# mateomarin/two_towers

Hardware: AMD Instinct MI355X
Metric: training pairs/sec at global batch=8192, 1/2/4/8 GPUs; MRR@10 match (higher is better)
Workload: dtype bf16; 1 GPU; BASELINE configs[2]: EnhancedTwoTowerModel(300, 256), seq_len 64, batch 8192 per GPU, bf16, hard-negative mining k=5 + margin 0.2, dropout 0.1, Adam; global_batch=8192, seq_len=64, hidden=256, embedding_dim=300, parallelism=dp1, loss=hardneg_margin

## Files before the change

### include/tt_hip.h

```cpp
#ifndef TT_HIP_H
#define TT_HIP_H
#include <stdint.h>

#ifdef __cplusplus
extern "C" {
#endif

#define TT_OK 0
#define TT_EINVAL 1000
#define TT_DT_F32 0
#define TT_DT_BF16 1

const char* tt_version(void);
const char* tt_last_error(void);
int tt_set_option(const char* name, int value);
int tt_get_option(const char* name, int* value);

int tt_embed_gather(int dtype, const void* table, long vocab, int ep, const int32_t* ids, long n,
                    void* out, void* stream);

int tt_pack_rows(int dtype, const float* src, long n, int e, int ep, void* out, void* stream);
typedef struct {
  const float* src;
  const float* src2;
  void* dst;
  int rows, cols, dcols;
  long lds, ldd;
  int dst_bf16;
} tt_pack_job;
int tt_pack_multi(const tt_pack_job* jobs, int njobs, void* stream);

int tt_cast(int dtype, const float* x, long n, void* y, void* stream);

int tt_colsum(const float* x, long rows, int cols, long ld, float* out, int accumulate, void* stream);

typedef struct {
  const void* a[4];
  const void* b[4];
  void* c[4];
  const float* bias[4];
  int bshift[4];
  const void* a_hi[4];
  int a_split;
  uint32_t drop_row0;
} tt_gemm_batch;

int tt_gemm(int dtype, int out_dtype, int a_kouter, int b_kouter, int m, int n, int k,
            const tt_gemm_batch* batch, int nbatch, long lda, long ldb, long ldc, float alpha,
            int beta_accum, int relu, int seq_t, uint32_t drop_seed, float drop_p, int splits,
            float* splitk_ws, void* stream);
int tt_gemm_ct(int dtype, int out_dtype, int a_kouter, int b_kouter, int m, int n, int k,
               const tt_gemm_batch* batch, int nbatch, long lda, long ldb, long ldc, float alpha,
               int beta_accum, int relu, int seq_t, uint32_t drop_seed, float drop_p, int splits,
               float* splitk_ws, int c_trans, void* stream);
long tt_gemm_ws_size(int m, int n, int nbatch, int splits);
int tt_gemm_pick_splits(int m, int n, int k, int nbatch);
int tt_gemm_bres_form(int m, int n, int k, int nbatch, long lda, long ldc);
int tt_gemm_tall_form(int dtype, int out_dtype, int a_kouter, int b_kouter, int m, int n, int k, long lda,
                      long ldb, int splits, int extras);

typedef struct {
  const void* g;
  const void* whh;
  const float* bhn;
  void* y;
  void* x1;
  void* save;
  float* hstate;
  int dir;
  uint32_t drop_seed;
  int drop_col0;
  uint32_t drop_row0;
} tt_gru_fwd_rec;

int tt_gru_fwd(int dtype, const tt_gru_fwd_rec* recs, int nrec, int B, int T, int H, long ldg,
               long ldy, float drop_p, void* ws, long ws_bytes, void* stream);
int tt_gru_fwd_launches(int dtype, int T, int H);
long tt_gru_fwd_ws_size(int dtype, int nrec, int B, int T, int H, long ldg, long ldy);
int tt_gru_fwd_launches_for(int dtype, int nrec, int B, int T, int H, long ldg, long ldy);

typedef struct {
  const void* g; const void* whh; const float* bhn;
  void* y;
  void* hfinal;
  void* scratch;
  int dir;
} tt_gru_infer_rec;
int  tt_gru_fwd_infer(int dtype, const tt_gru_infer_rec* recs, int nrec, int B, int T, int H, long ldg,
                      long ldy, long ldf, void* ws, long ws_bytes, void* stream);
long tt_gru_infer_scratch_size(int dtype, int B, int T, int H, int final_only);

typedef struct {
  const void* save;
  const void* y;
  const void* dy;
  const float* dfinal;
  const void* whh;
  void* dgx;
  void* dgh;
  void* dhstate;
  float* dbias_part;
  int dir;
} tt_gru_bwd_rec;

int tt_gru_bwd(int dtype, const tt_gru_bwd_rec* recs, int nrec, int B, int T, int H, long ldy,
               long ldd, long ldf, void* stream);
int tt_gru_bwd_launches(int dtype, int T, int H);
int tt_gru_bwd_carry_on_chip(int dtype, int T, int H);
int tt_gru_bias_rows(int B);

typedef struct {
  const void* w1; const float* b1; const float* ln_g; const float* ln_b;
  const void* w2; const float* b2;
  const void* x;
  void* p1;
  float* mean;
  float* rstd;
  void* u;
  float* out;
} tt_head_fwd_io;

int tt_proj_head_fwd(int dtype, const tt_head_fwd_io* io, int ntower, int B, int h, float ln_eps,
                     void* stream);

typedef struct {
  const void* w1; const float* ln_g; const float* ln_b; const void* w2;
  const void* x; const void* p1; const float* mean; const float* rstd; const void* u;
  const float* dout;
  float* dx;
  float* dw1; float* db1; float* dg; float* dbeta; float* dw2; float* db2;
  void* ws;
} tt_head_bwd_io;

int tt_proj_head_bwd(int dtype, const tt_head_bwd_io* io, int ntower, int B, int h, float ln_eps,
                     void* stream);
long tt_proj_head_bwd_ws_size(int dtype, int B, int h);

typedef struct {
  const void* x;
  const void* w1; const float* b1; const float* ln_g; const float* ln_b;
  void* p1;
  float* mean;
  float* rstd;
  float* out;
} tt_head1_fwd_io;

int tt_proj_head1_fwd(int dtype, const tt_head1_fwd_io* io, long rows, int C, float ln_eps, float drop_p,
                      uint32_t drop_seed, void* stream);

typedef struct {
  const void* x; const void* w1; const float* ln_g; const float* ln_b;
  const void* p1; const float* mean; const float* rstd;
  const float* dout;
  float* dx;
  float* dw1; float* db1; float* dg; float* dbeta;
  void* ws;
} tt_head1_bwd_io;

int tt_proj_head1_bwd(int dtype, const tt_head1_bwd_io* io, long rows, int C, float drop_p, uint32_t drop_seed,
                      void* stream);
long tt_proj_head1_bwd_ws_size(int dtype, long rows, int C);

int tt_l2norm_fwd(int dtype, const float* x, long rows, int cols, float eps, void* y, float* y32,
                  float* norm, void* stream);
int tt_l2norm_bwd(const float* dy, const float* y32, const float* norm, long rows, int cols,
                  float eps, float* dx, int accumulate, void* stream);

int tt_infonce_fwd(int dtype, const void* qn, long bq, const void* dn, long nd, int h,
                   float inv_tau, float offdiag_sub, long label_offset, float* lse,
                   float* row_loss, void* ws, void* stream);
long tt_infonce_fwd_ws_size(long bq, long nd);
int tt_infonce_bwd(int dtype, const void* qn, long bq, const void* dn, long nd, int h,
                   float inv_tau, float offdiag_sub, long label_offset, const float* lse,
                   const float* gscale, float* dqn, float* ddn, void* ws, void* stream);
long tt_infonce_bwd_ws_size(int dtype, long bq, long nd, int h);

int tt_hardneg_topk(int dtype, const void* qn, long bq, const void* dn, long nd, int h,
                    long label_offset, int k, int32_t* idx, float* val, void* ws, void* stream);
long tt_hardneg_ws_size(int dtype, long bq, long nd, int h, int k);

int tt_search_topk(int dtype, const float* qn, long Q, const void* dn, long N, int h, int k,
                   int32_t* idx, float* val, void* ws, void* stream);
long tt_search_ws_size(int dtype, long Q, long N, int h, int k);

int tt_topk_max(void);
int tt_topk_rows(const float* S, long rows, long cols, long ld, long label_offset, int k,
                 int32_t* idx, float* val, void* ws, void* stream);
long tt_topk_rows_ws_size(long rows, long cols, int k);

int tt_margin_fwd(const float* qn, long bq, const float* dn, long nd, int h, long label_offset,
                  const int32_t* idx, int k, float margin, float* row_loss, void* stream);
int tt_margin_bwd(const float* qn, long bq, const float* dn, long nd, int h, long label_offset,
                  const int32_t* idx, int k, float margin, const float* gscale, float* dqn, float* ddn,
                  void* ws, void* stream);
long tt_margin_bwd_ws_size(long bq, long nd, int h, int k);

int tt_sum(const float* x, long n, float scale, float* out, void* stream);

int tt_adam_multi(float* const* params, const float* const* grads, float* const* exp_avg,
                  float* const* exp_avg_sq, const long* sizes, int ntensors, float lr, float beta1,
                  float beta2, float eps, float weight_decay, int step, const int32_t* skip, void* stream);

#ifdef __cplusplus
}
#endif
#endif
```

### two_towers_amd/_lib.py

```python
from __future__ import annotations

import contextlib
import ctypes
import os
from ctypes import POINTER, c_float, c_int, c_long, c_uint32, c_void_p

import torch

_HERE = os.path.dirname(os.path.abspath(__file__))
LIB_PATH = os.environ.get("TT_HIP_LIB", os.path.join(_HERE, "lib", "libtt_hip.so"))

DT_F32 = 0
DT_BF16 = 1
TT_EINVAL = 1000


class TTError(RuntimeError):
    pass


class GruTimeoutError(TTError):
    """A column-split GRU forward launch gave up waiting for one of its member workgroups
    (tt_gru_fwd's status word): that launch's outputs are invalid."""


class GemmBatch(ctypes.Structure):
    _fields_ = [
        ("a", c_void_p * 4),
        ("b", c_void_p * 4),
        ("c", c_void_p * 4),
        ("bias", c_void_p * 4),
        ("bshift", c_int * 4),
        ("a_hi", c_void_p * 4),
        ("a_split", c_int),
        ("drop_row0", c_uint32),
    ]


class PackJob(ctypes.Structure):
    _fields_ = [
        ("src", c_void_p),
        ("src2", c_void_p),
        ("dst", c_void_p),
        ("rows", c_int),
        ("cols", c_int),
        ("dcols", c_int),
        ("lds", c_long),
        ("ldd", c_long),
        ("dst_bf16", c_int),
    ]


class GruFwdRec(ctypes.Structure):
    _fields_ = [
        ("g", c_void_p), ("whh", c_void_p), ("bhn", c_void_p), ("y", c_void_p), ("x1", c_void_p),
        ("save", c_void_p), ("hstate", c_void_p), ("dir", c_int), ("drop_seed", c_uint32),
        ("drop_col0", c_int), ("drop_row0", c_uint32),
    ]


class GruInferRec(ctypes.Structure):
    _fields_ = [
        ("g", c_void_p), ("whh", c_void_p), ("bhn", c_void_p), ("y", c_void_p), ("hfinal", c_void_p),
        ("scratch", c_void_p), ("dir", c_int),
    ]


class GruBwdRec(ctypes.Structure):
    _fields_ = [
        ("save", c_void_p), ("y", c_void_p), ("dy", c_void_p), ("dfinal", c_void_p), ("whh", c_void_p),
        ("dgx", c_void_p), ("dgh", c_void_p), ("dhstate", c_void_p), ("dbias_part", c_void_p),
        ("dir", c_int),
    ]


class HeadFwdIO(ctypes.Structure):
    _fields_ = [
        ("w1", c_void_p), ("b1", c_void_p), ("ln_g", c_void_p), ("ln_b", c_void_p), ("w2", c_void_p),
        ("b2", c_void_p), ("x", c_void_p), ("p1", c_void_p), ("mean", c_void_p), ("rstd", c_void_p),
        ("u", c_void_p), ("out", c_void_p),
    ]


class HeadBwdIO(ctypes.Structure):
    _fields_ = [
        ("w1", c_void_p), ("ln_g", c_void_p), ("ln_b", c_void_p), ("w2", c_void_p), ("x", c_void_p),
        ("p1", c_void_p), ("mean", c_void_p), ("rstd", c_void_p), ("u", c_void_p), ("dout", c_void_p),
        ("dx", c_void_p), ("dw1", c_void_p), ("db1", c_void_p), ("dg", c_void_p), ("dbeta", c_void_p),
        ("dw2", c_void_p), ("db2", c_void_p), ("ws", c_void_p),
    ]


class Head1FwdIO(ctypes.Structure):
    _fields_ = [
        ("x", c_void_p), ("w1", c_void_p), ("b1", c_void_p), ("ln_g", c_void_p), ("ln_b", c_void_p),
        ("p1", c_void_p), ("mean", c_void_p), ("rstd", c_void_p), ("out", c_void_p),
    ]


class Head1BwdIO(ctypes.Structure):
    _fields_ = [
        ("x", c_void_p), ("w1", c_void_p), ("ln_g", c_void_p), ("ln_b", c_void_p), ("p1", c_void_p),
        ("mean", c_void_p), ("rstd", c_void_p), ("dout", c_void_p), ("dx", c_void_p), ("dw1", c_void_p),
        ("db1", c_void_p), ("dg", c_void_p), ("dbeta", c_void_p), ("ws", c_void_p),
    ]


_SIGS = {
    "tt_version": (ctypes.c_char_p, []),
    "tt_last_error": (ctypes.c_char_p, []),
    "tt_set_option": (c_int, [ctypes.c_char_p, c_int]),
    "tt_get_option": (c_int, [ctypes.c_char_p, POINTER(c_int)]),
    "tt_embed_gather": (c_int, [c_int, c_void_p, c_long, c_int, c_void_p, c_long, c_void_p, c_void_p]),
    "tt_pack_rows": (c_int, [c_int, c_void_p, c_long, c_int, c_int, c_void_p, c_void_p]),
    "tt_pack_multi": (c_int, [c_void_p, c_int, c_void_p]),
    "tt_cast": (c_int, [c_int, c_void_p, c_long, c_void_p, c_void_p]),
    "tt_colsum": (c_int, [c_void_p, c_long, c_int, c_long, c_void_p, c_int, c_void_p]),
    "tt_gemm": (c_int, [c_int, c_int, c_int, c_int, c_int, c_int, c_int, POINTER(GemmBatch), c_int, c_long,
                        c_long, c_long, c_float, c_int, c_int, c_int, c_uint32, c_float, c_int, c_void_p,
                        c_void_p]),
    "tt_gemm_ct": (c_int, [c_int, c_int, c_int, c_int, c_int, c_int, c_int, POINTER(GemmBatch), c_int, c_long,
                           c_long, c_long, c_float, c_int, c_int, c_int, c_uint32, c_float, c_int, c_void_p,
                           c_int, c_void_p]),
    "tt_gemm_ws_size": (c_long, [c_int, c_int, c_int, c_int]),
    "tt_gemm_pick_splits": (c_int, [c_int, c_int, c_int, c_int]),
    "tt_gemm_bres_form": (c_int, [c_int, c_int, c_int, c_int, c_long, c_long]),
    "tt_gemm_tall_form": (c_int, [c_int, c_int, c_int, c_int, c_int, c_int, c_int, c_long, c_long, c_int, c_int]),
    "tt_gru_fwd": (c_int, [c_int, POINTER(GruFwdRec), c_int, c_int, c_int, c_int, c_long, c_long, c_float,
                           c_void_p, c_long, c_void_p]),
    "tt_gru_bwd": (c_int, [c_int, POINTER(GruBwdRec), c_int, c_int, c_int, c_int, c_long, c_long, c_long,
                           c_void_p]),
    "tt_gru_bias_rows": (c_int, [c_int]),
    "tt_gru_bwd_launches": (c_int, [c_int, c_int, c_int]),
    "tt_gru_bwd_carry_on_chip": (c_int, [c_int, c_int, c_int]),
    "tt_gru_fwd_launches": (c_int, [c_int, c_int, c_int]),
    "tt_gru_fwd_ws_size": (c_long, [c_int, c_int, c_int, c_int, c_int, c_long, c_long]),
    "tt_gru_fwd_launches_for": (c_int, [c_int, c_int, c_int, c_int, c_int, c_long, c_long]),
    "tt_gru_fwd_infer": (c_int, [c_int, POINTER(GruInferRec), c_int, c_int, c_int, c_int, c_long, c_long, c_long,
                                 c_void_p, c_long, c_void_p]),
    "tt_gru_infer_scratch_size": (c_long, [c_int, c_int, c_int, c_int, c_int]),
    "tt_proj_head_fwd": (c_int, [c_int, POINTER(HeadFwdIO), c_int, c_int, c_int, c_float, c_void_p]),
    "tt_proj_head_bwd": (c_int, [c_int, POINTER(HeadBwdIO), c_int, c_int, c_int, c_float, c_void_p]),
    "tt_proj_head_bwd_ws_size": (c_long, [c_int, c_int, c_int]),
    "tt_proj_head1_fwd": (c_int, [c_int, POINTER(Head1FwdIO), c_long, c_int, c_float, c_float, c_uint32,
                                  c_void_p]),
    "tt_proj_head1_bwd": (c_int, [c_int, POINTER(Head1BwdIO), c_long, c_int, c_float, c_uint32, c_void_p]),
    "tt_proj_head1_bwd_ws_size": (c_long, [c_int, c_long, c_int]),
    "tt_l2norm_fwd": (c_int, [c_int, c_void_p, c_long, c_int, c_float, c_void_p, c_void_p, c_void_p, c_void_p]),
    "tt_l2norm_bwd": (c_int, [c_void_p, c_void_p, c_void_p, c_long, c_int, c_float, c_void_p, c_int, c_void_p]),
    "tt_infonce_fwd": (c_int, [c_int, c_void_p, c_long, c_void_p, c_long, c_int, c_float, c_float, c_long,
                               c_void_p, c_void_p, c_void_p, c_void_p]),
    "tt_infonce_fwd_ws_size": (c_long, [c_long, c_long]),
    "tt_infonce_bwd": (c_int, [c_int, c_void_p, c_long, c_void_p, c_long, c_int, c_float, c_float, c_long,
                               c_void_p, c_void_p, c_void_p, c_void_p, c_void_p, c_void_p]),
    "tt_infonce_bwd_ws_size": (c_long, [c_int, c_long, c_long, c_int]),
    "tt_hardneg_topk": (c_int, [c_int, c_void_p, c_long, c_void_p, c_long, c_int, c_long, c_int, c_void_p,
                                c_void_p, c_void_p, c_void_p]),
    "tt_hardneg_ws_size": (c_long, [c_int, c_long, c_long, c_int, c_int]),
    "tt_search_topk": (c_int, [c_int, c_void_p, c_long, c_void_p, c_long, c_int, c_int, c_void_p, c_void_p,
                               c_void_p, c_void_p]),
    "tt_search_ws_size": (c_long, [c_int, c_long, c_long, c_int, c_int]),
    "tt_topk_max": (c_int, []),
    "tt_topk_rows": (c_int, [c_void_p, c_long, c_long, c_long, c_long, c_int, c_void_p, c_void_p, c_void_p,
                             c_void_p]),
    "tt_topk_rows_ws_size": (c_long, [c_long, c_long, c_int]),
    "tt_margin_fwd": (c_int, [c_void_p, c_long, c_void_p, c_long, c_int, c_long, c_void_p, c_int, c_float,
                              c_void_p, c_void_p]),
    "tt_margin_bwd": (c_int, [c_void_p, c_long, c_void_p, c_long, c_int, c_long, c_void_p, c_int, c_float,
                              c_void_p, c_void_p, c_void_p, c_void_p, c_void_p]),
    "tt_margin_bwd_ws_size": (c_long, [c_long, c_long, c_int, c_int]),
    "tt_sum": (c_int, [c_void_p, c_long, c_float, c_void_p, c_void_p]),
    "tt_adam_multi": (c_int, [POINTER(c_void_p), POINTER(c_void_p), POINTER(c_void_p), POINTER(c_void_p),
                              POINTER(c_long), c_int, c_float, c_float, c_float, c_float, c_float, c_int,
                              c_void_p, c_void_p]),
}

EXPORTED = tuple(_SIGS)

_lib = None
_load_error: str | None = None


def load():
    global _lib, _load_error
    if _lib is not None:
        return _lib
    if _load_error is not None:
        raise TTError(_load_error)
    if not os.path.exists(LIB_PATH):
        _load_error = (f"two_towers_amd: native library not found at {LIB_PATH}; "
                       "build it with `python -c 'import __graft_entry__ as g; g.build()'` (hipcc, gfx950)")
        raise TTError(_load_error)
    lib = ctypes.CDLL(LIB_PATH, mode=ctypes.RTLD_GLOBAL)
    for name, (res, args) in _SIGS.items():
        fn = getattr(lib, name)
        fn.restype = res
        fn.argtypes = args
    _lib = lib
    return lib


def check(rc: int, what: str = ""):
    if rc != 0:
        msg = _lib.tt_last_error().decode(errors="replace") if _lib is not None else ""
        raise TTError(f"{what or 'tt_hip'} failed (rc={rc}): {msg}")


def call(name: str, *args):
    lib = load()
    check(getattr(lib, name)(*args), name)


_topk_max: int | None = None


def topk_max() -> int:
    global _topk_max
    if _topk_max is None:
        _topk_max = int(load().tt_topk_max())
    return _topk_max


def get_option(name: str) -> int:
    v = c_int(0)
    call("tt_get_option", name.encode(), ctypes.byref(v))
    return v.value


def set_option(name: str, value: int) -> int:
    old = get_option(name)
    call("tt_set_option", name.encode(), int(value))
    return old


@contextlib.contextmanager
def option(name: str, value: int):
    torch.cuda.synchronize()
    old = set_option(name, value)
    try:
        yield
    finally:
        torch.cuda.synchronize()
        set_option(name, old)


def ptr(t: torch.Tensor | None) -> int | None:
    if t is None:
        return None
    return t.data_ptr()


def stream_ptr(device: torch.device | None = None) -> int:
    return torch.cuda.current_stream(device).cuda_stream


def require_gpu(*tensors: torch.Tensor):
    load()
    for t in tensors:
        if t is not None and t.device.type != "cuda":
            raise TTError(
                "two_towers_amd runs only on an AMD GPU (HIP, gfx950); got a tensor on "
                f"'{t.device}'. There is deliberately no CPU fallback: move the model and "
                "inputs to the GPU (`.to('cuda')`).")


def dtype_code(dt: torch.dtype) -> int:
    if dt == torch.float32:
        return DT_F32
    if dt == torch.bfloat16:
        return DT_BF16
    raise TTError(f"unsupported compute dtype {dt}; use torch.float32 or torch.bfloat16")
```

### two_towers_amd/csrc/tt_api.h

```cpp
#pragma once
#include <hip/hip_runtime.h>
#include <stdio.h>
#include <string.h>

#include "../../include/tt_hip.h"

namespace tt {
void set_error(const char* fmt, ...);

enum Opt {
  OPT_GRU_STEP,
  OPT_GRU_DEPTH,
  OPT_GRU_BWD_ROWS,
  OPT_GRU_BWD_BIG,
  OPT_GRU_BWD_STREAMS,
  OPT_GEMM_PERSIST,
  OPT_GEMM_A3,
  OPT_GEMM_REGSTAGE,
  OPT_GEMM_STREAM_OUT,
  OPT_HN_GEMM,
  OPT_GRU_BWD_PERSIST,
  OPT_GRU_FWD_STEP_ROWS,
  OPT_INFONCE_FLASH,
  OPT_HN_MAP,
  OPT_GEMM_SKEW,
  OPT_GEMM_PERSIST_MAXK,
  OPT_GRU_FWD_XC,
  OPT_GRU_XC_SKIP,
  OPT_GRU_XC_SPINS,
  OPT_GRU_BWD_SKEW,
  OPT_GRU_FWD_SKEW,
  OPT_GEMM_BRES,
  OPT_GRU_XC_COOP,
  OPT_GEMM_BUF,
  OPT_GEMM_ORDER,
  OPT_GRU_STEP_RING,
  OPT_GRU_FWD_XS,
  OPT_HN_SCAN_GEMM,
  OPT_GEMM_IEPI,
  OPT_BRES_ROWS,
  OPT_HN_SCAN_V,
  OPT_GEMM_W4,
  OPT_BRES_FORM,
  OPT_WGRAD_TALL,
  OPT_N
};
int opt(Opt o);
int tt_hn_scan_gemm(const void* q, long bq, const void* d, long nd, int h, long label_off, float* cm, long nch,
                    hipStream_t st);
}

#define TT_CHECK_ARG(cond, ...)            \
  do {                                     \
    if (!(cond)) {                         \
      tt::set_error(__VA_ARGS__);          \
      return TT_EINVAL;                    \
    }                                      \
  } while (0)

#define TT_CHECK_LAUNCH(what)                                                        \
  do {                                                                               \
    hipError_t e_ = hipGetLastError();                                               \
    if (e_ != hipSuccess) {                                                          \
      tt::set_error("%s: %s", what, hipGetErrorString(e_));                          \
      return (int)e_;                                                                \
    }                                                                                \
  } while (0)

#define TT_CHECK_HIP(expr)                                                           \
  do {                                                                               \
    hipError_t e_ = (expr);                                                          \
    if (e_ != hipSuccess) {                                                          \
      tt::set_error("%s: %s", #expr, hipGetErrorString(e_));                         \
      return (int)e_;                                                                \
    }                                                                                \
  } while (0)

#define TT_PROPAGATE(expr)     \
  do {                         \
    int rc_ = (expr);          \
    if (rc_ != 0) return rc_;  \
  } while (0)

static inline int tt_ceil_div(long a, long b) { return (int)((a + b - 1) / b); }
```

### two_towers_amd/csrc/tt_gemm.hip

```cpp
#include <float.h>
#include <stdarg.h>
#include <stdlib.h>

#include <atomic>
#include <type_traits>

#include "tt_api.h"
#include "tt_gemm_core.h"

namespace tt {
static thread_local char g_err[512];
void set_error(const char* fmt, ...) {
  va_list ap;
  va_start(ap, fmt);
  vsnprintf(g_err, sizeof(g_err), fmt, ap);
  va_end(ap);
}
}

namespace tt {
namespace {
struct OptDef {
  const char* name;
  const char* env;
  int dflt;
};
constexpr OptDef kOpts[OPT_N] = {
    {"gru_step", "TT_GRU_STEP", 0},               {"gru_depth", "TT_GRU_DEPTH", 4},
    {"gru_bwd_rows", "TT_GRU_BWD_ROWS", 0},     {"gru_bwd_big", "TT_GRU_BWD_BIG", 1},
    {"gru_bwd_streams", "TT_GRU_BWD_STREAMS", 2}, {"gemm_persist", "TT_GEMM_PERSIST", 1},
    {"gemm_a3", "TT_GEMM_A3", 1},                 {"gemm_regstage", "TT_GEMM_REGSTAGE", 0},
    {"gemm_stream_out", "TT_GEMM_STREAM_OUT", 1}, {"hn_gemm", "TT_HN_GEMM", 0},
    {"gru_bwd_persist", "TT_GRU_BWD_PERSIST", 1}, {"gru_fwd_step_rows", "TT_GRU_FWD_STEP_ROWS", 0},
    {"infonce_flash", "TT_INFONCE_FLASH", 1},     {"hn_map", "TT_HN_MAP", 2},
    {"gemm_skew", "TT_GEMM_SKEW", 0},             {"gemm_persist_maxk", "TT_GEMM_PERSIST_MAXK", 24},
    {"gru_fwd_xc", "TT_GRU_FWD_XC", 1},           {"gru_xc_skip", "TT_GRU_XC_SKIP", 0},
    {"gru_xc_spins", "TT_GRU_XC_SPINS", 22},      {"gru_bwd_skew", "TT_GRU_BWD_SKEW", 14},
    {"gru_fwd_skew", "TT_GRU_FWD_SKEW", 0},       {"gemm_bres", "TT_GEMM_BRES", 1},
    {"gru_xc_coop", "TT_GRU_XC_COOP", 0},         {"gemm_buf", "TT_GEMM_BUF", 1},
    {"gemm_order", "TT_GEMM_ORDER", 0},           {"gru_step_ring", "TT_GRU_STEP_RING", 4},
    {"gru_fwd_xs", "TT_GRU_FWD_XS", 1},           {"hn_scan_gemm", "TT_HN_SCAN_GEMM", 0},
    {"gemm_iepi", "TT_GEMM_IEPI", 1},             {"bres_rows", "TT_BRES_ROWS", 32},
    {"hn_scan_v", "TT_HN_SCAN_V", 5},             {"gemm_w4", "TT_GEMM_W4", 0},
    {"bres_form", "TT_BRES_FORM", 1},             {"wgrad_tall", "TT_WGRAD_TALL", 1},
};
struct OptTable {
  std::atomic<int> v[OPT_N];
  OptTable() {
    for (int i = 0; i < OPT_N; ++i) {
      const char* e = getenv(kOpts[i].env);
      v[i].store(e && *e ? atoi(e) : kOpts[i].dflt, std::memory_order_relaxed);
    }
  }
};
OptTable& opts() {
  static OptTable t;
  return t;
}
int find_opt(const char* name) {
  for (int i = 0; name && i < OPT_N; ++i)
    if (strcmp(name, kOpts[i].name) == 0) return i;
  return -1;
}
}
int opt(Opt o) { return opts().v[o].load(std::memory_order_relaxed); }
}

extern "C" const char* tt_version(void) { return "tt_hip 0.2.0 gfx950"; }
extern "C" const char* tt_last_error(void) { return tt::g_err; }
extern "C" int tt_set_option(const char* name, int value) {
  const int i = tt::find_opt(name);
  TT_CHECK_ARG(i >= 0, "tt_set_option: unknown option '%s'", name ? name : "(null)");
  tt::opts().v[i].store(value, std::memory_order_relaxed);
  return 0;
}
extern "C" int tt_get_option(const char* name, int* value) {
  const int i = tt::find_opt(name);
  TT_CHECK_ARG(i >= 0 && value, "tt_get_option: unknown option '%s'", name ? name : "(null)");
  *value = tt::opt((tt::Opt)i);
  return 0;
}

namespace {

struct GemmArgs {
  const void* a[4];
  const void* b[4];
  void* c[4];
  const float* bias[4];
  int bshift[4];
  const void* a_hi[4];
  int a_split;
  long lda, ldb, ldc;
  int M, N, K;
  int splits, kt_per_split;
  float alpha;
  int beta, relu, seq_t;
  uint32_t drop_seed, drop_thresh, drop_row0;
  float drop_inv_keep;
  long part_stride;
  int vec_ok;
  int force_regstage;
  int skew;
  int bias_vec_ok;
  int stream_out;
  int walk_g, walk_x;
  int nbatch;
  int c_trans;
  float* cm;
  long nch, label_off;
};

constexpr int BM = 128, BN = 128;

#ifndef TT_TAIL_SKIP
#define TT_TAIL_SKIP 1
#endif
using ttg::xcd_remap;
#ifndef PERSIST_IEPI
#define PERSIST_IEPI 1
#endif
#ifndef PERSIST_BAL
#define PERSIST_BAL 1
#endif
#ifndef TT_EPI_PAIR
#define TT_EPI_PAIR 1
#endif
#ifndef TT_GEMM_BAL
#define TT_GEMM_BAL true
#endif

template <typename T, bool AKO, bool BKO, bool SHIFT, typename TO, int TBM, int TBN, int WGM, int WGN, bool DMA,
          bool A3 = false, bool BUF = false>
__global__ __launch_bounds__(64 * WGM * WGN) void gemm_kernel(GemmArgs g) {
  using ML = std::conditional_t<
      DMA,
      std::conditional_t<TBM == 256 && TBN == 256 && WGM == 2 && WGN == 4,
                         ttg::Loop8<T, AKO, BKO, TT_GEMM_BAL, A3, false, BUF>,
                         ttg::DLoop<T, AKO, BKO, TBM, TBN, WGM, WGN>>,
      ttg::MainLoop<T, AKO, BKO, TBM, TBN>>;
  static_assert(DMA || (TBM == 128 && TBN == 128 && WGM == 2 && WGN == 2), "register path is 128x128");
  constexpr int NT = 64 * WGM * WGN;
  constexpr int LDSB = ML::LDS_BYTES > 64 * (TBN + 4) * 4 ? ML::LDS_BYTES : 64 * (TBN + 4) * 4;
  __shared__ __attribute__((aligned(16))) char lds[LDSB];
  const int ntn = (g.N + TBN - 1) / TBN, ntm = (g.M + TBM - 1) / TBM;
  const int id = xcd_remap(blockIdx.x, gridDim.x);
  const int bs = id / (ntm * ntn), tile = id - bs * (ntm * ntn);
  const int mt = tile / ntn, nt = tile - mt * ntn;
  const int bi = bs / g.splits, s = bs - bi * g.splits;
  const int m0 = mt * TBM, n0 = nt * TBN;
  const T* A = static_cast<const T*>(g.a[bi]);
  const T* B = static_cast<const T*>(g.b[bi]);

  f32x4 acc[ML::TM][ML::TN];
#pragma unroll
  for (int i = 0; i < ML::TM; ++i)
#pragma unroll
    for (int j = 0; j < ML::TN; ++j) acc[i][j] = f32x4{0.f, 0.f, 0.f, 0.f};

  const int nk = (g.K * (int)sizeof(T) + ttg::KTB - 1) / ttg::KTB;
  const int kt0 = s * g.kt_per_split;
  const int kt1 = min(nk, kt0 + g.kt_per_split);

  constexpr bool L8T = DMA && TBM == 256 && TBN == 256 && WGM == 2 && WGN == 4;
  const bool mm = !L8T || !TT_TAIL_SKIP || __builtin_amdgcn_readfirstlane((int)(m0 + (int)(threadIdx.x >> 8) * 128 < g.M));
  auto lrun = [&](const auto& la, const auto& lb) {
    if constexpr (L8T) ML::run(la, lb, g.K, kt0, kt1, lds, acc, mm);
    else ML::run(la, lb, g.K, kt0, kt1, lds, acc);
  };
  auto run = [&](const auto& la) {
    if constexpr (!BKO) {
      lrun(la, ttg::KCPlain<T>{B, g.ldb, n0, g.N});
    } else if constexpr (SHIFT) {
      lrun(la, ttg::KOShift<T>{B, g.ldb, n0, g.N - n0, g.seq_t, g.bshift[bi]});
    } else {
      lrun(la, ttg::KOPlain<T>{B, g.ldb, n0, g.N - n0});
    }
  };
  if constexpr (AKO) {
    ttg::KOPlain<T> la{A, g.lda, m0, g.M - m0};
    if (g.a_split > 0) {
      la.base1 = static_cast<const T*>(g.a_hi[bi]);
      la.csplit = g.a_split;
    }
    run(la);
  } else {
    run(ttg::KCPlain<T>{A, g.lda, m0, g.M});
  }

#ifdef TT_DIAG
  if (g.force_regstage == 9) {
    float sum = 0.f;
#pragma unroll
    for (int i = 0; i < ML::TM; ++i)
#pragma unroll
      for (int j = 0; j < ML::TN; ++j) sum += acc[i][j][0] + acc[i][j][3];
    if (sum == 12345.f) static_cast<float*>(g.c[bi])[0] = 1.f;
// ... 1674 lines not shown
```

### two_towers_amd/csrc/tt_gru.hip

```cpp
#include <algorithm>
#include <cstdlib>
#include <mutex>
#include <type_traits>

#include "tt_api.h"
#include "tt_gemm_core.h"

namespace {

struct FwdRec {
  const void* g; const void* whh; const float* bhn; void* y; void* x1; void* save; float* hs;
  int dir; uint32_t seed; int col0;
  uint32_t row0;
};
struct FwdArgs {
  FwdRec r[4];
  int B, T, H;
  long ldg, ldy;
  int s;
  uint32_t drop_thresh;
  float inv_keep;
#ifdef TT_DIAG
  int dbg;
#endif
};
struct InfArgs : FwdArgs {
  void* hfin[4];
  void* himg[4];
  long ldf;
};
TT_DEV void* inf_hfin(const FwdArgs&, int) { return nullptr; }
TT_DEV void* inf_hfin(const InfArgs& a, int rz) { return a.hfin[rz]; }
TT_DEV long inf_ldf(const FwdArgs&) { return 0; }
TT_DEV long inf_ldf(const InfArgs& a) { return a.ldf; }

struct BwdRec {
  const void* save; const void* y; const void* dy; const float* dfinal; const void* whh;
  void* dgx; void* dgh; void* dh; float* dbias; int dir;
};
struct BwdArgs {
  BwdRec r[4];
  int B, T, H;
  long ldy, ldd, ldf;
  int s;
  int skew;
#ifdef TT_DIAG
  int dbg;
#endif
};


TT_DEV void gru_cell(float xr, float xz, float xn, float lr, float lz, float ln, float bn, float hp, float& y,
                     float& ar, float& az, float& an, float& ghn) {
#pragma clang fp contract(off)
  constexpr float L2E = 0x1.715476p+0f;
  ghn = ln + bn;
  ar = xr + lr;
  az = xz + lz;
  const float rg = __builtin_amdgcn_rcpf(1.0f + __builtin_amdgcn_exp2f(L2E * -ar));
  const float zg = __builtin_amdgcn_rcpf(1.0f + __builtin_amdgcn_exp2f(L2E * -az));
  an = __builtin_fmaf(rg, ghn, xn);
  const float ng = 1.0f - 2.0f * __builtin_amdgcn_rcpf(__builtin_amdgcn_exp2f(L2E * (2.0f * an)) + 1.0f);
  y = __builtin_fmaf(zg, hp, (1.0f - zg) * ng);
}

template <typename T>
struct GateRows {
  static constexpr bool SHIFTED = false, KSPLIT = false;
  const T* w; int H, j0;
  TT_DEV const T* rowptr(int r) const {
    const int half = r / 96, rem = r - half * 96;
    const int g = rem >> 5, j = j0 + half * 32 + (rem & 31);
    return j < H ? w + (long)(g * H + j) * H : nullptr;
  }
  TT_DEV const T* at(int r, int k) const { const T* p = rowptr(r); return p ? p + k : nullptr; }
};

template <typename T, int BMR, int NS = 2, typename A = FwdArgs>
__global__ __launch_bounds__(2 * BMR) void gru_fwd_step(A a) {
  constexpr bool INF = std::is_same_v<A, InfArgs>;
  constexpr int NT = 2 * BMR;
  using ML = ttg::DLoop<T, false, false, BMR, 192, BMR / 64, 2, NS>;
  __shared__ __attribute__((aligned(16))) char lds[ML::LDS_BYTES];
  const int ntj = (a.H + 63) / 64, ntm = (a.B + BMR - 1) / BMR;
  const int id = ttg::xcd_remap(blockIdx.x, gridDim.x);
  const int rz = id / (ntm * ntj), rem = id - rz * ntm * ntj;
  const FwdRec R = a.r[rz];
  const int H = a.H, T_ = a.T, s = a.s;
  const int m0 = (rem / ntj) * BMR, j0 = (rem % ntj) * 64;
  const int t = R.dir ? T_ - 1 - s : s;
  const int tp = R.dir ? t + 1 : t - 1;
  const T* Y = static_cast<const T*>(R.y);

  f32x4 acc[ML::TM][ML::TN];
#pragma unroll
  for (int i = 0; i < ML::TM; ++i)
#pragma unroll
    for (int j = 0; j < ML::TN; ++j) acc[i][j] = f32x4{0.f, 0.f, 0.f, 0.f};
  bool prod = s > 0, epi = true;
#ifdef TT_DIAG
  if (a.dbg & 8) prod = false;
  if (a.dbg & 16) epi = false;
#endif
  const int tid = threadIdx.x;
  const int cur = s & 1, prv = cur ^ 1;
  const T* G = static_cast<const T*>(R.g);
  const float* hs_prv = R.hs + (long)prv * a.B * H;
  if (prod) {
    ttg::KCPlain<T> la{Y + (long)tp * a.ldy, (long)T_ * a.ldy, m0, a.B};
    if constexpr (INF) {
      if (!Y) la = ttg::KCPlain<T>{static_cast<const T*>(a.himg[rz]) + (long)prv * a.B * H, (long)H, m0, a.B};
    }
    GateRows<T> lb{static_cast<const T*>(R.whh), H, j0};
    const int nk = (H * (int)sizeof(T) + ttg::KTB - 1) / ttg::KTB;
    ML::run(la, lb, H, 0, nk, lds, acc);
  }
  if (!epi) {
    if (acc[0][0][0] == 1.2345f) static_cast<T*>(R.y)[0] = T(0);
    return;
  }

  const int wave = threadIdx.x >> 6, lane = threadIdx.x & 63;
  float* L = reinterpret_cast<float*>(lds);
  constexpr int FLD = 68;
  T* Yw = static_cast<T*>(R.y);
  T* X1 = static_cast<T*>(R.x1);
  T* S = static_cast<T*>(R.save);
  float* hs_cur = R.hs + (long)cur * a.B * H;
  const __amdgpu_buffer_rsrc_t srs = tt_rsrc(S + ((long)m0 * T_ + t) * (4L * H));
  const __amdgpu_buffer_rsrc_t xrs = tt_rsrc(X1 ? X1 + ((long)m0 * T_ + t) * a.ldy : Yw);
  for (int hf = 0; hf < BMR / 64; ++hf) {
    if ((wave >> 1) == hf) {
      const int nb = (wave & 1) * 32;
#pragma unroll
      for (int g = 0; g < 3; ++g)
#pragma unroll
        for (int i = 0; i < 4; ++i)
#pragma unroll
          for (int jh = 0; jh < 2; ++jh)
#pragma unroll
            for (int r = 0; r < 4; ++r)
              L[(g * 64 + 16 * i + 4 * (lane >> 4) + r) * FLD + nb + 16 * jh + (lane & 15)] = acc[i][g * 2 + jh][r];
    }
    __syncthreads();
#pragma unroll
    for (int k = 0; k < 512 / NT; ++k) {
      const int rl = (tid >> 3) + (NT / 8) * k, jg = (tid & 7) * 8;
      const int b = m0 + hf * 64 + rl, j = j0 + jg;
      if (b < a.B && j < H) {
        const long row = (long)b * T_ + t;
        float xr[8], xz[8], xn[8], hp[8], bn[8], y[8], sr[8], sz[8], sn[8], sg[8];
        ld8(G + row * a.ldg + j, xr);
        ld8(G + row * a.ldg + H + j, xz);
        ld8(G + row * a.ldg + 2 * H + j, xn);
        ld8(R.bhn + j, bn);
        if (s > 0) ld8(hs_prv + (long)b * H + j, hp);
        else {
#pragma unroll
          for (int e = 0; e < 8; ++e) hp[e] = 0.f;
        }
        const float* Lr = L + (0 * 64 + rl) * FLD + jg;
        const float* Lz = L + (1 * 64 + rl) * FLD + jg;
        const float* Ln = L + (2 * 64 + rl) * FLD + jg;
#pragma unroll
        for (int e = 0; e < 8; ++e)
          gru_cell(xr[e], xz[e], xn[e], Lr[e], Lz[e], Ln[e], bn[e], hp[e], y[e], sr[e], sz[e], sn[e], sg[e]);
        st8(hs_cur + (long)b * H + j, y);
        if constexpr (INF) {
          if (Yw) st8(Yw + row * a.ldy + j, y);
          else st8(static_cast<T*>(a.himg[rz]) + ((long)cur * a.B + b) * H + j, y);
          T* hf = static_cast<T*>(a.hfin[rz]);
          if (hf && s == T_ - 1) st8(hf + (long)b * a.ldf + j, y);
          continue;
        }
        st8(Yw + row * a.ldy + j, y);
        const int so = (int)((((long)(b - m0) * T_) * 4L * H + j) * (long)sizeof(T));
        st8_sc1(srs, so, sr, (T*)nullptr);
        st8_sc1(srs, so + H * (int)sizeof(T), sz, (T*)nullptr);
        st8_sc1(srs, so + 2 * H * (int)sizeof(T), sn, (T*)nullptr);
        st8_sc1(srs, so + 3 * H * (int)sizeof(T), sg, (T*)nullptr);
        if (X1) {
#pragma unroll
          for (int e = 0; e < 8; ++e)
            y[e] *= a.drop_thresh ? tt_dropout_scale(R.seed, R.row0 + (uint32_t)row, (uint32_t)(R.col0 + j + e),
                                                     a.drop_thresh, a.inv_keep)
                                  : 1.f;
          st8_sc1(xrs, (int)((((long)(b - m0) * T_) * a.ldy + j) * (long)sizeof(T)), y, (T*)nullptr);
        }
      }
    }
    __syncthreads();
  }
}

template <typename T, int BMR, int NS = 2>
__global__ __launch_bounds__(256) void gru_bwd_step(BwdArgs a) {
  using ML = ttg::DLoop<T, false, true, BMR, 128, 2, 2, NS>;
  constexpr int LDSB = ML::LDS_BYTES > 64 * 132 * 4 ? ML::LDS_BYTES : 64 * 132 * 4;
// ... 427 lines not shown
  float bacc[4][8];
#pragma unroll
  for (int q = 0; q < 4; ++q)
#pragma unroll
    for (int e = 0; e < 8; ++e) bacc[q][e] = 0.f;
  for (int s = T_ - 1; s >= 0; --s) {
    const int t = R.dir ? T_ - 1 - s : s;
    const int tn = R.dir ? t - 1 : t + 1;
    const int tp = R.dir ? t + 1 : t - 1;
    const bool last = (s == T_ - 1);
    auto column_pass = [&](const int u0) {
    f32x4 acc[4][C::NCB];
#pragma unroll
    for (int i = 0; i < 4; ++i)
#pragma unroll
      for (int j = 0; j < C::NCB; ++j) acc[i][j] = f32x4{0.f, 0.f, 0.f, 0.f};
    if (CREG && !last) {
#pragma unroll
      for (int i = 0; i < 4; ++i)
#pragma unroll
        for (int jc = 0; jc < C::NCB; ++jc) {
          const uint2 w = *reinterpret_cast<const uint2*>(reinterpret_cast<const bf16_t*>(lds) +
                                                          (wr * 64 + 16 * i + (lane & 15)) * C::LDB + wc * (C::HP / 4) +
                                                          16 * jc + 4 * (lane >> 4));
          acc[i][jc] = f32x4{__uint_as_float(w.x << 16), __uint_as_float(w.x & 0xFFFF0000u),
                             __uint_as_float(w.y << 16), __uint_as_float(w.y & 0xFFFF0000u)};
        }
      __syncthreads();
    }
    if (!last && !(dbg & 1)) {
#if TT_BWD_BUF
      const long abytes = (long)(a.B - m0) * ldr * 2;
      const uint32_t anrec = (uint32_t)(abytes > 0xFFFFFFFFL ? 0xFFFFFFFFL : abytes);
      const ttg::tt_rsrc4 rsx = ttg::make_rsrc4(DGX + (long)tn * a.ldd + (long)m0 * ldr, anrec);
      const ttg::tt_rsrc4 rsh = ttg::make_rsrc4(DGH + (long)tn * a.ldd + (long)m0 * ldr - 2 * H, anrec);
      const ttg::tt_rsrc4 rsw = ttg::make_rsrc4(W + u0, 0xFFFFFFFFu);
      uint32_t voff[C::P];
#pragma unroll
      for (int j = 0; j < C::P; ++j)
        voff[j] = prow[j] >= 0 ? (uint32_t)(((long)prow[j] * ldr + pcol[j]) * 2) : (uint32_t)(pcol[j] * 2);
      auto issue = [&](int r) {
        const uint32_t img = lbase + (uint32_t)(r % C::NS) * C::SLOT;
        const int wv = __builtin_amdgcn_readfirstlane(threadIdx.x >> 6);
        const bool hi = r * 32 >= 2 * H;
#pragma unroll
        for (int j = 0; j < C::P; ++j) {
          const int pc = wv + 8 * j;
          if (pc < 8) ttg::dma16_buf(hi ? rsh : rsx, voff[j], (uint32_t)r * 64u, img + (uint32_t)pc * 1024u);
          else ttg::dma16_buf(rsw, voff[j], (uint32_t)r * (uint32_t)(64 * H), img + (uint32_t)pc * 1024u);
        }
      };
#else
      const char* as0[C::P];
      const char* as1[C::P];
#pragma unroll
      for (int j = 0; j < C::P; ++j) {
        const int b = m0 + (prow[j] < 0 ? 0 : prow[j]);
        const bool ok = prow[j] >= 0 && b < a.B;
        as0[j] = ok ? reinterpret_cast<const char*>(DGX + (long)tn * a.ldd + (long)b * ldr + pcol[j]) : zp;
        as1[j] = ok ? reinterpret_cast<const char*>(DGH + (long)tn * a.ldd + (long)b * ldr + pcol[j] - 2 * H) : zp;
      }
      auto issue = [&](int r) {
        const uint32_t img = lbase + (uint32_t)(r % C::NS) * C::SLOT;
        const int wv = __builtin_amdgcn_readfirstlane(threadIdx.x >> 6);
        const bool hi = r * 32 >= 2 * H;
#pragma unroll
        for (int j = 0; j < C::P; ++j) {
          const int pc = wv + 8 * j;
          const char* src;
          if (pc < 8) {
            src = hi ? as1[j] : as0[j];
            if (src != zp) src += (long)r * 64;
          } else {
            src = reinterpret_cast<const char*>(W + (long)r * 32 * H + u0 + pcol[j]);
          }
          ttg::dma16(src, img + (uint32_t)pc * 1024u);
        }
      };
#endif
      issue(0);
      issue(1);
      issue(2);
#if TT_BWD_STAG
      const bool late = wr == 1;
      wait_younger<C::NS - 2, C::P>(NK - 1);
      __builtin_amdgcn_s_barrier();
      if (late) __builtin_amdgcn_s_barrier();
#pragma unroll 1
      for (int r = 0; r < NK; ++r) {
        if (r > 0) __builtin_amdgcn_s_barrier();
        if (r + 3 < NK) issue(r + 3);
        const char* sl = lds + (r % C::NS) * C::SLOT;
        uint4 fa[4], fb[C::NCB];
#pragma unroll
        for (int i = 0; i < 4; ++i) fa[i] = frag_kc64(sl, wr * 64 + 16 * i);
        const char* ib = sl + 8192 + ((wc * (C::HP / 4)) >> 7) * 8192;
        const int cb = (wc * (C::HP / 4)) & 127;
#pragma unroll
        for (int j = 0; j < C::NCB; ++j) fb[j] = ttg::frag<bf16_t, true>(ib, cb + 16 * j, 0);
        __builtin_amdgcn_s_setprio(1);
#pragma unroll
        for (int j = 0; j < C::NCB / 2; ++j)
#pragma unroll
          for (int i = 0; i < 4; ++i) acc[i][j] = ttg::mma<bf16_t>(fb[j], fa[i], acc[i][j]);
        __builtin_amdgcn_s_setprio(0);
        asm volatile("s_waitcnt lgkmcnt(0)" ::: "memory");
        __builtin_amdgcn_sched_barrier(0);
        if (late) wait_younger<C::NS - 2, C::P>(NK - 2 - r);
        __builtin_amdgcn_s_barrier();
        __builtin_amdgcn_s_setprio(1);
#pragma unroll
        for (int j = C::NCB / 2; j < C::NCB; ++j)
#pragma unroll
          for (int i = 0; i < 4; ++i) acc[i][j] = ttg::mma<bf16_t>(fb[j], fa[i], acc[i][j]);
        __builtin_amdgcn_s_setprio(0);
        if (!late) wait_younger<C::NS - 2, C::P>(NK - 2 - r);
      }
      if (!late) __builtin_amdgcn_s_barrier();
#else
#pragma unroll 1
      for (int r = 0; r < NK; ++r) {
        wait_younger<C::NS - 2, C::P>(NK - 1 - r);
        __builtin_amdgcn_s_barrier();
        if (r + 3 < NK) issue(r + 3);
        const char* sl = lds + (r % C::NS) * C::SLOT;
        uint4 fa[4];
#pragma unroll
        for (int i = 0; i < 4; ++i) fa[i] = frag_kc64(sl, wr * 64 + 16 * i);
        const char* ib = sl + 8192 + ((wc * (C::HP / 4)) >> 7) * 8192;
        const int cb = (wc * (C::HP / 4)) & 127;
#pragma unroll
        for (int jp = 0; jp < C::NCB; jp += 2) {
          uint4 fb[2];
#pragma unroll
          for (int j = 0; j < 2; ++j) fb[j] = ttg::frag<bf16_t, true>(ib, cb + 16 * (jp + j), 0);
          __builtin_amdgcn_s_setprio(1);
#pragma unroll
          for (int i = 0; i < 4; ++i)
#pragma unroll
            for (int j = 0; j < 2; ++j)
              acc[i][jp + j] = ttg::mma<bf16_t>(fb[j], fa[i], acc[i][jp + j]);
          __builtin_amdgcn_s_setprio(0);
        }
      }
#endif
      __builtin_amdgcn_s_barrier();
    }
    const long trow = (long)m0 * T_ + t;
    const __amdgpu_buffer_rsrc_t rc =
        tt_rsrc_n(static_cast<const bf16_t*>(R.dh) + (long)((s + 1) & 1) * a.B * H + (long)m0 * H, !last);
    bf16_t* cr_cur = static_cast<bf16_t*>(R.dh) + (long)(s & 1) * a.B * H + (long)m0 * H;
    const __amdgpu_buffer_rsrc_t rd = tt_rsrc_n(DY ? DY + trow * a.ldy : S, DY != nullptr);
    const __amdgpu_buffer_rsrc_t rsv = tt_rsrc_n(S + trow * 4L * H, true);
    const __amdgpu_buffer_rsrc_t ry = tt_rsrc_n(s > 0 ? Y + ((long)m0 * T_ + tp) * a.ldy : S, s > 0);
    const __amdgpu_buffer_rsrc_t grs = tt_rsrc(DGXw + trow * a.ldd);
    uint32_t* L16 = reinterpret_cast<uint32_t*>(lds);
#pragma unroll
    for (int i = 0; i < 4; ++i)
#pragma unroll
      for (int jc = 0; jc < C::NCB; ++jc) {
        const uint32_t w0 = (uint32_t)f2bf(acc[i][jc][0]) | ((uint32_t)f2bf(acc[i][jc][1]) << 16);
        const uint32_t w1 = (uint32_t)f2bf(acc[i][jc][2]) | ((uint32_t)f2bf(acc[i][jc][3]) << 16);
        *reinterpret_cast<uint2*>(reinterpret_cast<bf16_t*>(lds) + (wr * 64 + 16 * i + (lane & 15)) * C::LDB +
                                  wc * (C::HP / 4) + 16 * jc + 4 * (lane >> 4)) = make_uint2(w0, w1);
      }
    __syncthreads();
    float bsum_own[4][8];
    auto& bsum = CREG ? bacc : bsum_own;
    if constexpr (!CREG) {
#pragma unroll
      for (int q = 0; q < 4; ++q)
#pragma unroll
        for (int e = 0; e < 8; ++e) bsum[q][e] = 0.f;
    }
    constexpr int NB = TT_BWD_NB;
    auto load_row = [&](const int k, uint4 (&v)[7]) {
      const int bl = rsub + C::RPI * k;
      const bool ok = k < NIT && m0 + bl < a.B && !(dbg & 2);
      const uint32_t oc = ok ? (uint32_t)(bl * H + u0 + jg) * 2u : 0x80000000u;
      const uint32_t oy = ok ? (uint32_t)(bl * T_ * (int)a.ldy + u0 + jg) * 2u : 0x80000000u;
      const uint32_t os = ok ? (uint32_t)(bl * T_ * 4 * H + u0 + jg) * 2u : 0x80000000u;
      v[0] = CREG ? make_uint4(0, 0, 0, 0) : ld16_buf(rc, oc, 0);
      v[1] = ld16_buf<(TT_BWD_NT & 2) ? 2 : 0>(rd, oy, 0);
#pragma unroll
      for (int q = 0; q < 4; ++q) v[2 + q] = ld16_buf<(TT_BWD_NT & 1) ? 2 : 0>(rsv, os, q * 2 * H);
      v[6] = ld16_buf<(TT_BWD_NT & 2) ? 2 : 0>(ry, oy, 0);
    };
    auto finish_row = [&](const int k, const uint4 (&v)[7]) {
      const int bl = rsub + C::RPI * k;
      const int b = m0 + bl;
      if (b >= a.B) return;
      float cin[8], dy[8], ar[8], az[8], an[8], gh[8], hp[8], gm[8];
      unpack8(v[0], cin);
      unpack8(v[1], dy);
      unpack8(v[2], ar);
      unpack8(v[3], az);
      unpack8(v[4], an);
      unpack8(v[5], gh);
      unpack8(v[6], hp);
      unpack8(*reinterpret_cast<const uint4*>(L16 + ((bl * C::LDB + jg) >> 1)), gm);
      if (last && R.dfinal) {
        const float* pf = R.dfinal + (long)b * a.ldf + u0 + jg;
        tt_u32x4 d0, d1;
        asm volatile("global_load_dwordx4 %0, %2, off\n\tglobal_load_dwordx4 %1, %2, off offset:16\n\ts_waitcnt vmcnt(0)"
                     : "=&v"(d0), "=&v"(d1)
                     : "v"(pf)
                     : "memory");
#pragma unroll
        for (int e = 0; e < 4; ++e) {
          cin[e] = __uint_as_float(d0[e]);
          cin[4 + e] = __uint_as_float(d1[e]);
        }
      }
      float o_r[8], o_z[8], o_n[8], o_hn[8], cout[8];
#pragma unroll
      for (int e = 0; e < 8; ++e) {
        const float dht = gm[e] + cin[e] + dy[e];
        float rg, omr, zg, omz, ng, sech2;
        tt_sigmoid_pair(ar[e], rg, omr);
        tt_sigmoid_pair(az[e], zg, omz);
        tt_tanh_sech2(an[e], ng, sech2);
        const float dnp = dht * omz * sech2;
        const float drp = dnp * gh[e] * rg * omr;
        const float dzp = dht * (hp[e] - ng) * zg * omz;
        o_r[e] = drp; o_z[e] = dzp; o_n[e] = dnp; o_hn[e] = dnp * rg;
        cout[e] = dht * zg;
        bsum[0][e] += drp; bsum[1][e] += dzp; bsum[2][e] += dnp; bsum[3][e] += dnp * rg;
      }
      if constexpr (CREG)
        *reinterpret_cast<uint4*>(L16 + ((bl * C::LDB + jg) >> 1)) = pack8bf(cout);
      if (dbg & 4) {
        if (o_r[0] == 12345.f) L16[0] = __float_as_uint(o_z[1] + o_n[2] + o_hn[3] + cout[4]);
        return;
      }
      if constexpr (!CREG) st8(cr_cur + (long)bl * H + u0 + jg, cout);
      const long row = (long)b * T_ + t;
      bf16_t* xw = DGXw + row * a.ldd + u0 + jg;
      st8_pol<TT_BWD_OUT_NT != 0>(xw, o_r);
      st8_pol<TT_BWD_OUT_NT != 0>(xw + H, o_z);
      st8_sc1(grs, (int)(((long)bl * T_ * a.ldd + u0 + jg + 2 * H) * 2L), o_n, (bf16_t*)nullptr);
      st8_pol<TT_BWD_OUT_NT != 0>(DGHw + row * a.ldd + u0 + jg, o_hn);
    };
    auto batch = [&](const int kb) {
      uint4 vin[NB][7];
#pragma unroll
      for (int kk = 0; kk < NB; ++kk) load_row(kb + kk, vin[kk]);
#pragma unroll
      for (int kk = 0; kk < NB; ++kk) finish_row(kb + kk, vin[kk]);
    };
#if TT_BWD_PIPE
    static_assert(NIT % 2 == 0, "rows in pairs");
    uint4 vr[2][7];
    load_row(0, vr[0]);
#pragma unroll 1
    for (int k = 0; k < NIT; k += 2) {
      load_row(k + 1, vr[1]);
      finish_row(k, vr[0]);
      load_row(k + 2, vr[0]);
      finish_row(k + 1, vr[1]);
    }
#else
#pragma unroll 1
    for (int kb = 0; kb < NIT; kb += NB) batch(kb);
#endif
    if constexpr (!CREG) {
      __syncthreads();
      float* red = L;
#pragma unroll
      for (int q = 0; q < 4; ++q)
#pragma unroll
        for (int e = 0; e < 8; ++e) red[(rsub * 4 + q) * C::HP + jg + e] = bsum[q][e];
      __syncthreads();
      for (int c = tid; c < 4 * C::HP; c += 512) {
        float v = 0.f;
#pragma unroll
        for (int w = 0; w < C::RPI; ++w) v += red[w * 4 * C::HP + c];
        part[(c / C::HP) * H + u0 + c % C::HP] += v;
      }
    }
    asm volatile("s_waitcnt vmcnt(0)" ::: "memory");
    __syncthreads();
    };
    if constexpr (C::NP == 1) {
      column_pass(0);
    } else {
#pragma unroll 1
      for (int pass = 0; pass < C::NP; ++pass) column_pass(pass * C::HP);
    }
  }
  if constexpr (CREG) {
    float* red = reinterpret_cast<float*>(lds);
#pragma unroll 1
    for (int q = 0; q < 4; ++q) {
#pragma unroll
      for (int e = 0; e < 8; ++e) red[rsub * C::HP + jg + e] = bacc[q][e];
      __syncthreads();
      if (tid < C::HP) {
        float v = 0.f;
#pragma unroll
        for (int w = 0; w < C::RPI; ++w) v += red[w * C::HP + tid];
        part[q * H + tid] = v;
      }
      __syncthreads();
    }
  }
}

// ... 280 lines not shown
  TT_STAMP(k_end);
  prf[7] = k_end - k_start;
  if (threadIdx.x == 0 && blockIdx.x < 2048)
    for (int i = 0; i < 8; ++i) g_fwd_prof[blockIdx.x][i] = prf[i];
#endif
}

typedef __attribute__((address_space(1))) unsigned xc_gu32;
#ifndef XC_G_AUX
#define XC_G_AUX 2
#endif
#ifndef XC_OUT_AUX
#define XC_OUT_AUX 2
#endif
#ifndef XC_VALU_PER_MFMA
#define XC_VALU_PER_MFMA 3
#endif
namespace xc {
constexpr int NT = 256;
constexpr int CR = 32;
constexpr int RR = 256;
constexpr int NCH = RR / CR;
constexpr int SSTR = 68;
constexpr int STG = CR * 192 * 4;
constexpr int CSTR = 64;
constexpr unsigned OOB = 0x80000000u;
template <int H>
struct Cfg {
  static constexpr int M = H / 64;
  static constexpr int NKT = H / 32;
  static constexpr int QPW = H / 64;
  static constexpr int SLOT = CR * H * 2;
  static constexpr int ST = RR * SSTR * 4;
  static constexpr int LDS = ST + 2 * SLOT + STG;
};
static_assert(Cfg<512>::LDS <= 163840 && Cfg<256>::LDS <= 163840, "gru_fwd_xc LDS budget");
}

struct XcWs {
  bf16_t* xb;
  unsigned* cnt;
  unsigned* err;
  unsigned* status;
  unsigned spins;
  int skip;
  int xmap;
  int qg;
  int nrec;
  int rpg;
  int nround;
  int fast_ok;
  int skew;
};

TT_DEV void xc_wait(xc_gu32* cnt, unsigned target, const XcWs& ws) {
  xc_gu32* err = (xc_gu32*)(uintptr_t)ws.err;
  for (unsigned spins = 0;; ++spins) {
    if (__hip_atomic_load(cnt, __ATOMIC_RELAXED, __HIP_MEMORY_SCOPE_AGENT) >= target) return;
    if ((spins & 1023u) == 1023u) {
      if (__hip_atomic_load(err, __ATOMIC_RELAXED, __HIP_MEMORY_SCOPE_AGENT) != 0u) return;
      if (spins > ws.spins) {
        __hip_atomic_store(err, 1u, __ATOMIC_RELAXED, __HIP_MEMORY_SCOPE_AGENT);
        __hip_atomic_fetch_or((xc_gu32*)(uintptr_t)ws.status, 1u, __ATOMIC_RELAXED, __HIP_MEMORY_SCOPE_AGENT);
        return;
      }
    }
    __builtin_amdgcn_s_sleep(1);
  }
}

TT_DEV bool xc_group_on_one_xcd(unsigned* cntw, int M, int mem, bool allowed, const XcWs& ws) {
  __shared__ int s_fast;
  if (threadIdx.x == 0) {
    unsigned xcc;
    asm volatile("s_getreg_b32 %0, hwreg(HW_REG_XCC_ID)" : "=s"(xcc));
    xc_gu32* w = (xc_gu32*)(uintptr_t)cntw;
    __hip_atomic_store(w + 8 + mem, (xcc & 15u) + 1u, __ATOMIC_RELAXED, __HIP_MEMORY_SCOPE_AGENT);
    asm volatile("s_waitcnt vmcnt(0)" ::: "memory");
    __hip_atomic_fetch_add(w + 1, 1u, __ATOMIC_RELAXED, __HIP_MEMORY_SCOPE_AGENT);
    xc_wait(w + 1, (unsigned)M, ws);
    unsigned first = __hip_atomic_load(w + 8, __ATOMIC_RELAXED, __HIP_MEMORY_SCOPE_AGENT);
    bool same = allowed && first != 0u;
    for (int m = 1; m < M; ++m) same &= __hip_atomic_load(w + 8 + m, __ATOMIC_RELAXED, __HIP_MEMORY_SCOPE_AGENT) == first;
    s_fast = same ? 1 : 0;
  }
  __syncthreads();
  return s_fast != 0;
}

template <int H>
TT_DEV void xc_h_offsets(uint32_t (&ho)[xc::Cfg<H>::QPW]) {
  const int lane = threadIdx.x & 63, w = threadIdx.x >> 6;
#pragma unroll
  for (int p = 0; p < xc::Cfg<H>::QPW; ++p) {
    const int q = w * xc::Cfg<H>::QPW + p, kt = q >> 1, rb = q & 1;
    ho[p] = (uint32_t)(((rb * 16 + (lane & 15)) * H + kt * 32 + (lane >> 4) * 8) * 2);
  }
}
template <int H>
TT_DEV void xc_load_h(__amdgpu_buffer_rsrc_t rx, const uint32_t (&ho)[xc::Cfg<H>::QPW], int c,
                      tt_u32x4 (&hv)[xc::Cfg<H>::QPW]) {
#pragma unroll
  for (int p = 0; p < xc::Cfg<H>::QPW; ++p)
    hv[p] = __builtin_amdgcn_raw_buffer_load_b128(rx, (int)ho[p], c * xc::CR * H * 2, 16);
}
template <int H>
TT_DEV void xc_put_h(char* slot, const tt_u32x4 (&hv)[xc::Cfg<H>::QPW]) {
  const int lane = threadIdx.x & 63, w = threadIdx.x >> 6;
#pragma unroll
  for (int p = 0; p < xc::Cfg<H>::QPW; ++p)
    *reinterpret_cast<tt_u32x4*>(slot + (w * xc::Cfg<H>::QPW + p) * 1024 + lane * 16) = hv[p];
}
template <int H>
TT_DEV void xc_mfma(const char* slot, const tt_u32x4 (&wa)[3][xc::Cfg<H>::NKT], f32x4 (&acc)[2][3]) {
  constexpr int NKT = xc::Cfg<H>::NKT;
  const int lane = threadIdx.x & 63;
  auto frag = [&](int kt, int rb) {
    return *reinterpret_cast<const tt_u32x4*>(slot + (kt * 2 + rb) * 1024 + lane * 16);
  };
#pragma unroll
  for (int rb = 0; rb < 2; ++rb)
#pragma unroll
    for (int g = 0; g < 3; ++g) acc[rb][g] = f32x4{0.f, 0.f, 0.f, 0.f};
  tt_u32x4 f[3][2];
  f[0][0] = frag(0, 0); f[0][1] = frag(0, 1);
  f[1][0] = frag(1, 0); f[1][1] = frag(1, 1);
#pragma unroll
  for (int kt = 0; kt < NKT; ++kt) {
    if (kt + 2 < NKT) {
      f[(kt + 2) % 3][0] = frag(kt + 2, 0);
      f[(kt + 2) % 3][1] = frag(kt + 2, 1);
    }
#pragma unroll
    for (int rb = 0; rb < 2; ++rb)
#pragma unroll
      for (int g = 0; g < 3; ++g)
        acc[rb][g] = __builtin_amdgcn_mfma_f32_16x16x32_bf16(__builtin_bit_cast(bf16x8v, wa[g][kt]),
                                                             __builtin_bit_cast(bf16x8v, f[kt % 3][rb]), acc[rb][g], 0, 0, 0);
  }
}
TT_DEV void xc_stage(float* stg, const f32x4 (&acc)[2][3]) {
  const int lane = threadIdx.x & 63, w = threadIdx.x >> 6;
#pragma unroll
  for (int rb = 0; rb < 2; ++rb)
#pragma unroll
    for (int g = 0; g < 3; ++g)
      *reinterpret_cast<f32x4*>(stg + stg_off(rb * 16 + (lane & 15), g * 64 + 16 * w + 4 * (lane >> 4))) = acc[rb][g];
}


template <int H, bool DROP, typename A = FwdArgs>
__global__ __launch_bounds__(xc::NT, 1) __attribute__((amdgpu_waves_per_eu(1, 1))) void gru_fwd_xcp(A a, XcWs ws) {
  constexpr bool INF = std::is_same_v<A, InfArgs>;
  static_assert(!(INF && DROP), "no dropout copy in the inference form");
  using C = xc::Cfg<H>;
  constexpr int M = C::M, NKT = C::NKT;
  __shared__ __attribute__((aligned(16))) char lds[C::LDS];
  float* stt = reinterpret_cast<float*>(lds);
  char* slots = lds + C::ST;
  float* stg = reinterpret_cast<float*>(lds + C::ST + 2 * C::SLOT);
  const int tid = threadIdx.x, wave = tid >> 6, lane = tid & 63;
  uint32_t ho[C::QPW];
  xc_h_offsets<H>(ho);
  const int xcd = blockIdx.x & 7, jj = blockIdx.x >> 3;
  const int grp = ws.xmap ? (int)blockIdx.x / M : xcd * ws.qg + jj / M;
  const int mem = ws.xmap ? (int)blockIdx.x % M : jj % M;
  const int rz = grp % ws.nrec, gi = grp / ws.nrec;
  const FwdRec R = a.r[rz];
  const int T_ = a.T, B = a.B;
  const int gb0 = gi * ws.rpg;
  xc_gu32* cw = (xc_gu32*)(uintptr_t)(ws.cnt + grp * xc::CSTR);
  xc_gu32* cntA = cw;
  xc_gu32* cntB = cw + 2;
  const bool publish = !(grp == 0 && mem == ws.skip - 1);
  bf16_t* xbg = ws.xb + (long)grp * 2 * xc::RR * H;
  const __amdgpu_buffer_rsrc_t rx[2] = {tt_rsrc(xbg), tt_rsrc(xbg + xc::RR * H)};
  tt_u32x4 wa[3][NKT];
  {
    const bf16_t* W = static_cast<const bf16_t*>(R.whh);
#pragma unroll
    for (int g = 0; g < 3; ++g)
#pragma unroll
      for (int kt = 0; kt < NKT; ++kt)
        wa[g][kt] = *reinterpret_cast<const tt_u32x4*>(
            W + (long)(g * H + 64 * mem + 16 * wave + (lane & 15)) * H + kt * 32 + (lane >> 4) * 8);
#pragma unroll
    for (int g = 0; g < 3; ++g)
#pragma unroll
      for (int kt = 0; kt < NKT; ++kt) asm volatile("" : "+a"(wa[g][kt]));
  }
  const int cr = tid >> 3, u0 = (tid & 7) * 8, j = 64 * mem + u0;
  float bn[8];
  {
    const float4 b0 = *reinterpret_cast<const float4*>(R.bhn + j);
    const float4 b1 = *reinterpret_cast<const float4*>(R.bhn + j + 4);
    bn[0] = b0.x; bn[1] = b0.y; bn[2] = b0.z; bn[3] = b0.w;
    bn[4] = b1.x; bn[5] = b1.y; bn[6] = b1.z; bn[7] = b1.w;
  }
  const bf16_t* G = static_cast<const bf16_t*>(R.g);
  bf16_t* Yw = static_cast<bf16_t*>(R.y);
  bf16_t* X1 = static_cast<bf16_t*>(R.x1);
  bf16_t* S = static_cast<bf16_t*>(R.save);
  const bool fast = xc_group_on_one_xcd(ws.cnt + grp * xc::CSTR, M, mem, ws.fast_ok != 0, ws);
  if (ws.skew > 0 && (grp & 1))
    for (int i = 0; i < ws.skew; ++i) __builtin_amdgcn_s_sleep(127);
  const int NS = ws.nround * T_;
  struct Step {
    int s, t, rb0, nrow;
  };
  auto step_of = [&](int idx) {
    Step q;
    const int r = idx / T_;
    q.s = idx - r * T_;
    q.t = R.dir ? T_ - 1 - q.s : q.s;
    q.rb0 = gb0 + r * xc::RR;
    q.nrow = min(min(ws.rpg - r * xc::RR, xc::RR), B - q.rb0);
    return q;
  };
  auto g_rsrc = [&](const Step& q) {
    return tt_rsrc_n(G + (long)(q.nrow > 0 ? q.rb0 : 0) * T_ * a.ldg, q.nrow > 0);
  };
  auto load_g = [&](const Step& q, __amdgpu_buffer_rsrc_t rG, int c, tt_u32x4 (&gx)[3]) {
    const uint32_t og = c * xc::CR + cr < q.nrow ? (uint32_t)(((c * xc::CR + cr) * T_ + q.t) * (int)a.ldg + j) * 2u
                                                  : xc::OOB;
#pragma unroll
    for (int g = 0; g < 3; ++g) gx[g] = __builtin_amdgcn_raw_buffer_load_b128(rG, (int)og, g * H * 2, XC_G_AUX);
  };
  tt_u32x4 hv[C::QPW];
  auto load_h = [&](const Step& q, int qidx, int c) {
    if (q.s == 0) {
#pragma unroll
      for (int p = 0; p < C::QPW; ++p) hv[p] = tt_u32x4{0u, 0u, 0u, 0u};
    } else {
      xc_load_h<H>(rx[(qidx - 1) & 1], ho, c, hv);
    }
  };
  float lr[8], lz[8], ln[8], hp[8];
  auto read_gates = [&](int c, bool first) {
    const int rr = c * xc::CR + cr;
#pragma unroll
    for (int h = 0; h < 2; ++h) {
      const float4 v0 = *reinterpret_cast<const float4*>(stg + stg_off(cr, 0 * 64 + u0 + 4 * h));
      const float4 v1 = *reinterpret_cast<const float4*>(stg + stg_off(cr, 1 * 64 + u0 + 4 * h));
      const float4 v2 = *reinterpret_cast<const float4*>(stg + stg_off(cr, 2 * 64 + u0 + 4 * h));
      const float4 p = *reinterpret_cast<const float4*>(stt + rr * xc::SSTR + u0 + 4 * h);
      lr[4 * h] = v0.x; lr[4 * h + 1] = v0.y; lr[4 * h + 2] = v0.z; lr[4 * h + 3] = v0.w;
      lz[4 * h] = v1.x; lz[4 * h + 1] = v1.y; lz[4 * h + 2] = v1.z; lz[4 * h + 3] = v1.w;
      ln[4 * h] = v2.x; ln[4 * h + 1] = v2.y; ln[4 * h + 2] = v2.z; ln[4 * h + 3] = v2.w;
      hp[4 * h] = first ? 0.f : p.x; hp[4 * h + 1] = first ? 0.f : p.y;
      hp[4 * h + 2] = first ? 0.f : p.z; hp[4 * h + 3] = first ? 0.f : p.w;
    }
  };
  f32x4 acc[2][3];
  for (int i = tid; i < 2 * C::SLOT / 16; i += xc::NT)
    reinterpret_cast<float4*>(slots)[i] = make_float4(0.f, 0.f, 0.f, 0.f);
  Step cur = step_of(0);
  __amdgpu_buffer_rsrc_t rGc = g_rsrc(cur);
  tt_u32x4 gq[2][3];
  load_g(cur, rGc, 0, gq[0]);
#pragma unroll
  for (int p = 0; p < C::QPW; ++p) hv[p] = tt_u32x4{0u, 0u, 0u, 0u};
  __syncthreads();
  xc_mfma<H>(slots, wa, acc);
  xc_stage(stg, acc);
  __syncthreads();
  read_gates(0, true);
  for (int idx = 0; idx < NS; ++idx) {
    const bool has_next = idx + 1 < NS;
    const Step nxt = step_of(has_next ? idx + 1 : idx);
    const __amdgpu_buffer_rsrc_t rGn = g_rsrc(nxt);
    const long r0w = (long)(cur.nrow > 0 ? cur.rb0 : 0) * T_;
    const bool on = cur.nrow > 0;
    bf16_t* HF = static_cast<bf16_t*>(inf_hfin(a, rz));
    const __amdgpu_buffer_rsrc_t rY =
        INF ? tt_rsrc_n(Yw ? (const void*)(Yw + r0w * a.ldy) : G, on && Yw != nullptr) : tt_rsrc_n(Yw + r0w * a.ldy, on);
    const __amdgpu_buffer_rsrc_t rX1 =
        INF ? tt_rsrc_n(HF ? (const void*)(HF + (long)(on ? cur.rb0 : 0) * inf_ldf(a)) : G, on && HF != nullptr && cur.s == T_ - 1)
            : tt_rsrc_n(X1 ? X1 + r0w * a.ldy : Yw, on && X1 != nullptr);
    const __amdgpu_buffer_rsrc_t rS = INF ? tt_rsrc_n(G, false) : tt_rsrc_n(S + r0w * 4L * H, on);
    const __amdgpu_buffer_rsrc_t rdst_h = rx[idx & 1];
    const int t = cur.t;
#pragma unroll
    for (int c = 0; c < xc::NCH; ++c) {
      const bool more = c + 1 < xc::NCH || has_next;
      if (c + 1 < xc::NCH) load_g(cur, rGc, c + 1, gq[(c + 1) & 1]);
      else if (has_next) load_g(nxt, rGn, 0, gq[0]);
      {
        const int rr = c * xc::CR + cr;
        const bool ok = rr < cur.nrow;
        float xr[8], xz[8], xn[8], y[8], sr[8], sz[8], sn[8], sg[8], msk[8];
        const uint32_t grow = (uint32_t)(cur.rb0 + rr) * (uint32_t)T_ + (uint32_t)t;
        const tt_u32x4(&gcur)[3] = gq[c & 1];
        unpack8(make_uint4(gcur[0][0], gcur[0][1], gcur[0][2], gcur[0][3]), xr);
        unpack8(make_uint4(gcur[1][0], gcur[1][1], gcur[1][2], gcur[1][3]), xz);
        unpack8(make_uint4(gcur[2][0], gcur[2][1], gcur[2][2], gcur[2][3]), xn);
        if (more) {
          const char* base = slots + ((c + 1) & 1) * C::SLOT + lane * 16;
          auto frag = [&](int kt, int rb) { return *reinterpret_cast<const tt_u32x4*>(base + (kt * 2 + rb) * 1024); };
#pragma unroll
          for (int rb = 0; rb < 2; ++rb)
#pragma unroll
            for (int g = 0; g < 3; ++g) acc[rb][g] = f32x4{0.f, 0.f, 0.f, 0.f};
          tt_u32x4 f[3][2];
          f[0][0] = frag(0, 0); f[0][1] = frag(0, 1);
          f[1][0] = frag(1, 0); f[1][1] = frag(1, 1);
          __builtin_amdgcn_sched_barrier(0);
#pragma unroll
          for (int kt = 0; kt < NKT; ++kt) {
            if (kt + 2 < NKT) {
              f[(kt + 2) % 3][0] = frag(kt + 2, 0);
              f[(kt + 2) % 3][1] = frag(kt + 2, 1);
            }
#pragma unroll
            for (int rb = 0; rb < 2; ++rb)
#pragma unroll
              for (int g = 0; g < 3; ++g)
                acc[rb][g] = __builtin_amdgcn_mfma_f32_16x16x32_bf16(
                    __builtin_bit_cast(bf16x8v, wa[g][kt]), __builtin_bit_cast(bf16x8v, f[kt % 3][rb]), acc[rb][g], 0, 0, 0);
            if constexpr (DROP) {
#pragma unroll
              for (int e = 0; e < 8; ++e)
                if (e * NKT / 8 == kt) {
                  msk[e] = tt_dropout_scale(R.seed, R.row0 + grow, (uint32_t)(R.col0 + j + e), a.drop_thresh, a.inv_keep);
                  asm volatile("" : "+v"(msk[e]));
                }
            }
#pragma unroll
            for (int e = 0; e < 8; ++e)
              if ((e + 1) * NKT / 8 - 1 == kt) {
                asm volatile("" : "+v"(xr[e]), "+v"(xz[e]), "+v"(xn[e]), "+v"(lr[e]), "+v"(lz[e]), "+v"(ln[e]),
                             "+v"(hp[e]));
                gru_cell(xr[e], xz[e], xn[e], lr[e], lz[e], ln[e], bn[e], hp[e], y[e], sr[e], sz[e], sn[e], sg[e]);
                asm volatile("" : "+v"(y[e]), "+v"(sr[e]), "+v"(sz[e]), "+v"(sn[e]), "+v"(sg[e]));
              }
#pragma unroll
            for (int i = 0; i < 6; ++i) {
              __builtin_amdgcn_sched_group_barrier(0x008, 1, 0);
              __builtin_amdgcn_sched_group_barrier(0x002, XC_VALU_PER_MFMA, 0);
            }
            __builtin_amdgcn_sched_barrier(0);
          }
        } else {
#pragma unroll
          for (int e = 0; e < 8; ++e) {
            gru_cell(xr[e], xz[e], xn[e], lr[e], lz[e], ln[e], bn[e], hp[e], y[e], sr[e], sz[e], sn[e], sg[e]);
            if constexpr (DROP)
              msk[e] = tt_dropout_scale(R.seed, R.row0 + grow, (uint32_t)(R.col0 + j + e), a.drop_thresh, a.inv_keep);
          }
        }
        *reinterpret_cast<float4*>(stt + rr * xc::SSTR + u0) = make_float4(y[0], y[1], y[2], y[3]);
        *reinterpret_cast<float4*>(stt + rr * xc::SSTR + u0 + 4) = make_float4(y[4], y[5], y[6], y[7]);
        const uint4 yb = pack8bf(y);
        if (fast) st16_buf(rdst_h, (uint32_t)(rr * H + j) * 2u, 0, yb);
        else st16_buf_sc1(rdst_h, (uint32_t)(rr * H + j) * 2u, 0, yb);
        asm volatile("" ::: "memory");
        const int lrow = rr * T_ + t;
        const uint32_t oy = ok ? (uint32_t)(lrow * (int)a.ldy + j) * 2u : xc::OOB;
        const uint32_t os = ok ? (uint32_t)(lrow * 4 * H + j) * 2u : xc::OOB;
        st16_buf_aux<XC_OUT_AUX>(rY, (int)oy, yb);
        if constexpr (INF) {
          st16_buf_aux<XC_OUT_AUX>(rS, (int)os, yb);
          st16_buf_aux<XC_OUT_AUX>(rS, (int)(os + 2u * H), yb);
          st16_buf_aux<XC_OUT_AUX>(rS, (int)(os + 4u * H), yb);
          st16_buf_aux<XC_OUT_AUX>(rS, (int)(os + 6u * H), yb);
          st16_buf_aux<XC_OUT_AUX>(rX1, (int)(ok ? (uint32_t)(rr * (int)a.ldf + j) * 2u : xc::OOB), yb);
        } else {
          st16_buf_aux<XC_OUT_AUX>(rS, (int)os, pack8bf(sr));
          st16_buf_aux<XC_OUT_AUX>(rS, (int)(os + 2u * H), pack8bf(sz));
          st16_buf_aux<XC_OUT_AUX>(rS, (int)(os + 4u * H), pack8bf(sn));
          st16_buf_aux<XC_OUT_AUX>(rS, (int)(os + 6u * H), pack8bf(sg));
          if constexpr (DROP) {
#pragma unroll
            for (int e = 0; e < 8; ++e) y[e] *= msk[e];
            st16_buf_aux<XC_OUT_AUX>(rX1, (int)oy, pack8bf(y));
          } else {
            st16_buf_aux<XC_OUT_AUX>(rX1, (int)oy, yb);
          }
        }
      }
      if (c == 3 || c == 7) asm volatile("s_nop 0\n\ts_waitcnt vmcnt(6)" ::: "memory");
      if (c + 2 < xc::NCH || has_next) xc_put_h<H>(slots + (c & 1) * C::SLOT, hv);
      if (c + 3 < xc::NCH) load_h(cur, idx, c + 3);
      else if (has_next) load_h(nxt, idx + 1, c + 3 - xc::NCH);
      if (tid == 0) {
        if (c == 0 && idx > 0) xc_wait(cntB, (unsigned)(M * idx), ws);
        if (c == 4 && has_next) xc_wait(cntA, (unsigned)(M * (idx + 1)), ws);
      }
      __syncthreads();
      if (tid == 0 && c == 3 && publish) __hip_atomic_fetch_add(cntA, 1u, __ATOMIC_RELAXED, __HIP_MEMORY_SCOPE_AGENT);
      if (tid == 0 && c == 7 && publish) __hip_atomic_fetch_add(cntB, 1u, __ATOMIC_RELAXED, __HIP_MEMORY_SCOPE_AGENT);
      if (more) {
        xc_stage(stg, acc);
        __syncthreads();
        if (c + 1 < xc::NCH) read_gates(c + 1, cur.s == 0);
        else read_gates(0, nxt.s == 0);
      }
    }
    cur = nxt;
    rGc = rGn;
  }
}

#ifndef XS_VPRIO
#define XS_VPRIO 0
#endif
#ifndef XS_MPUB
#define XS_MPUB 1
#endif
#ifndef XS_MPOLL
#define XS_MPOLL 1
#endif
#ifndef XS_GA
#define XS_GA 1
#endif
namespace xs {
constexpr int NT = 512;
template <int H>
struct Cfg {
  static constexpr int SLOT = xc::Cfg<H>::SLOT;
  static constexpr int LDS = 2 * SLOT + 2 * xc::STG;
};
static_assert(Cfg<512>::LDS <= 163840, "gru_fwd_xs LDS budget");
}

template <int H, bool DROP, typename A = FwdArgs>
__global__ __launch_bounds__(xs::NT, 1) __attribute__((amdgpu_waves_per_eu(2, 2))) void gru_fwd_xs(A a, XcWs ws) {
  constexpr bool INF = std::is_same_v<A, InfArgs>;
  static_assert(!(INF && DROP), "no dropout copy in the inference form");
  using C = xc::Cfg<H>;
  constexpr int M = C::M, NKT = C::NKT, QPW = C::QPW;
#ifdef TT_DIAG
  const int dbg = a.dbg;
#else
  constexpr int dbg = 0;
#endif
  __shared__ __attribute__((aligned(16))) char lds[xs::Cfg<H>::LDS];
  char* slots = lds;
  float* stgb = reinterpret_cast<float*>(lds + 2 * C::SLOT);
  const int tid = threadIdx.x, wave = tid >> 6, lane = tid & 63;
  const bool mw = wave < 4;
  const int vw = wave - 4, vt = tid - 256;
  const int xcd = blockIdx.x & 7, jj = blockIdx.x >> 3;
  const int grp = ws.xmap ? (int)blockIdx.x / M : xcd * ws.qg + jj / M;
  const int mem = ws.xmap ? (int)blockIdx.x % M : jj % M;
  const int rz = grp % ws.nrec, gi = grp / ws.nrec;
  const FwdRec R = a.r[rz];
  const int T_ = a.T, B = a.B;
  const int gb0 = gi * ws.rpg;
  xc_gu32* cw = (xc_gu32*)(uintptr_t)(ws.cnt + grp * xc::CSTR);
  xc_gu32* cntA = cw;
  xc_gu32* cntB = cw + 2;
  const bool publish = !(grp == 0 && mem == ws.skip - 1);
  bf16_t* xbg = ws.xb + (long)grp * 2 * xc::RR * H;
  const __amdgpu_buffer_rsrc_t rx[2] = {tt_rsrc(xbg), tt_rsrc(xbg + xc::RR * H)};
  const bool fast = xc_group_on_one_xcd(ws.cnt + grp * xc::CSTR, M, mem, ws.fast_ok != 0, ws);
  if (ws.skew > 0 && (grp & 1))
    for (int i = 0; i < ws.skew; ++i) __builtin_amdgcn_s_sleep(127);
  const int NS = ws.nround * T_;
  struct Step {
    int s, t, rb0, nrow;
  };
  auto step_of = [&](int idx) {
    Step q;
    const int r = idx / T_;
    q.s = idx - r * T_;
    q.t = R.dir ? T_ - 1 - q.s : q.s;
    q.rb0 = gb0 + r * xc::RR;
    q.nrow = min(min(ws.rpg - r * xc::RR, xc::RR), B - q.rb0);
    return q;
  };
  for (int i = tid; i < 2 * C::SLOT / 16; i += xs::NT) reinterpret_cast<float4*>(slots)[i] = make_float4(0.f, 0.f, 0.f, 0.f);
  __syncthreads();
  if (mw) {
    tt_u32x4 wa[3][NKT];
    {
      const bf16_t* W = static_cast<const bf16_t*>(R.whh);
#pragma unroll
      for (int g = 0; g < 3; ++g)
#pragma unroll
        for (int kt = 0; kt < NKT; ++kt)
          wa[g][kt] = *reinterpret_cast<const tt_u32x4*>(
              W + (long)(g * H + 64 * mem + 16 * wave + (lane & 15)) * H + kt * 32 + (lane >> 4) * 8);
#pragma unroll
      for (int g = 0; g < 3; ++g)
#pragma unroll
        for (int kt = 0; kt < NKT; ++kt) asm volatile("" : "+v"(wa[g][kt]));
    }
    auto chunk = [&](const char* sl, float* gb) {
      f32x4 acc[2][3];
      if (dbg & 8) {
#pragma unroll
        for (int rb = 0; rb < 2; ++rb)
#pragma unroll
          for (int g = 0; g < 3; ++g)
            *reinterpret_cast<f32x4*>(gb + stg_off(rb * 16 + (lane & 15), g * 64 + 16 * wave + 4 * (lane >> 4))) =
                f32x4{0.f, 0.f, 0.f, 0.f};
        return;
      }
      const char* base = sl + lane * 16;
      auto frag = [&](int kt, int rb) { return *reinterpret_cast<const tt_u32x4*>(base + (kt * 2 + rb) * 1024); };
#pragma unroll
      for (int rb = 0; rb < 2; ++rb)
#pragma unroll
        for (int g = 0; g < 3; ++g) acc[rb][g] = f32x4{0.f, 0.f, 0.f, 0.f};
      tt_u32x4 f[3][2];
      f[0][0] = frag(0, 0); f[0][1] = frag(0, 1);
      f[1][0] = frag(1, 0); f[1][1] = frag(1, 1);
#pragma unroll
      for (int kt = 0; kt < NKT; ++kt) {
        if (kt + 2 < NKT) {
          f[(kt + 2) % 3][0] = frag(kt + 2, 0);
          f[(kt + 2) % 3][1] = frag(kt + 2, 1);
        }
#pragma unroll
        for (int rb = 0; rb < 2; ++rb)
#pragma unroll
          for (int g = 0; g < 3; ++g)
            acc[rb][g] = __builtin_amdgcn_mfma_f32_16x16x32_bf16(
                __builtin_bit_cast(bf16x8v, wa[g][kt]), __builtin_bit_cast(bf16x8v, f[kt % 3][rb]), acc[rb][g], 0, 0, 0);
      }
#pragma unroll
      for (int rb = 0; rb < 2; ++rb)
#pragma unroll
        for (int g = 0; g < 3; ++g)
          *reinterpret_cast<f32x4*>(gb + stg_off(rb * 16 + (lane & 15), g * 64 + 16 * wave + 4 * (lane >> 4))) = acc[rb][g];
    };
    chunk(slots, stgb);
    __syncthreads();
    for (int idx = 0; idx < NS; ++idx) {
      const bool has_next = idx + 1 < NS;
#pragma unroll
      for (int c = 0; c < xc::NCH; ++c) {
        if (c + 1 < xc::NCH || has_next) chunk(slots + ((c + 1) & 1) * C::SLOT, stgb + ((c + 1) & 1) * (xc::STG / 4));
#if XS_MPOLL
        if (tid == 0 && !(dbg & 32)) {
          if (c == 0 && idx > 0) xc_wait(cntB, (unsigned)(M * idx), ws);
          if (c == 4 && has_next) xc_wait(cntA, (unsigned)(M * (idx + 1)), ws);
        }
#endif
        __syncthreads();
#if XS_MPUB
        if (tid == 0 && c == 3 && publish) __hip_atomic_fetch_add(cntA, 1u, __ATOMIC_RELAXED, __HIP_MEMORY_SCOPE_AGENT);
        if (tid == 0 && c == 7 && publish) __hip_atomic_fetch_add(cntB, 1u, __ATOMIC_RELAXED, __HIP_MEMORY_SCOPE_AGENT);
#endif
      }
    }
    return;
  }
  uint32_t ho[QPW];
#pragma unroll
  for (int p = 0; p < QPW; ++p) {
    const int q = vw * QPW + p, kt = q >> 1, rb = q & 1;
    ho[p] = (uint32_t)(((rb * 16 + (lane & 15)) * H + kt * 32 + (lane >> 4) * 8) * 2);
  }
  const int cr = vt >> 3, u0 = (vt & 7) * 8, j = 64 * mem + u0;
  float bn[8];
  {
    const float4 b0 = *reinterpret_cast<const float4*>(R.bhn + j);
    const float4 b1 = *reinterpret_cast<const float4*>(R.bhn + j + 4);
    bn[0] = b0.x; bn[1] = b0.y; bn[2] = b0.z; bn[3] = b0.w;
    bn[4] = b1.x; bn[5] = b1.y; bn[6] = b1.z; bn[7] = b1.w;
  }
  const bf16_t* G = static_cast<const bf16_t*>(R.g);
  bf16_t* Yw = static_cast<bf16_t*>(R.y);
  bf16_t* X1 = static_cast<bf16_t*>(R.x1);
  bf16_t* S = static_cast<bf16_t*>(R.save);
  auto g_rsrc = [&](const Step& q) { return tt_rsrc_n(G + (long)(q.nrow > 0 ? q.rb0 : 0) * T_ * a.ldg, q.nrow > 0); };
  auto load_g = [&](const Step& q, __amdgpu_buffer_rsrc_t rG, int c, tt_u32x4 (&gx)[3]) {
    const uint32_t og = c * xc::CR + cr < q.nrow ? (uint32_t)(((c * xc::CR + cr) * T_ + q.t) * (int)a.ldg + j) * 2u
                                                  : xc::OOB;
#pragma unroll
    for (int g = 0; g < 3; ++g)
      gx[g] = (dbg & 2) ? tt_u32x4{0u, 0u, 0u, 0u} : __builtin_amdgcn_raw_buffer_load_b128(rG, (int)og, g * H * 2, XC_G_AUX);
  };
  tt_u32x4 hv[QPW];
  auto load_h = [&](const Step& q, int qidx, int c) {
    if (q.s == 0 || (dbg & 4)) {
#pragma unroll
      for (int p = 0; p < QPW; ++p) hv[p] = tt_u32x4{0u, 0u, 0u, 0u};
    } else {
#pragma unroll
      for (int p = 0; p < QPW; ++p)
        hv[p] = __builtin_amdgcn_raw_buffer_load_b128(rx[(qidx - 1) & 1], (int)ho[p], c * xc::CR * H * 2, 16);
    }
  };
  float st[xc::NCH][8];
  Step cur = step_of(0);
  __amdgpu_buffer_rsrc_t rGc = g_rsrc(cur);
  constexpr int GR = XS_GA < 2 ? 2 : 4;
  static_assert(XS_GA >= 1 && XS_GA < GR && xc::NCH % GR == 0, "gate-input ring");
  tt_u32x4 gq[GR][3];
#pragma unroll
  for (int c = 0; c < XS_GA; ++c) load_g(cur, rGc, c, gq[c]);
#pragma unroll
  for (int p = 0; p < QPW; ++p) hv[p] = tt_u32x4{0u, 0u, 0u, 0u};
  __syncthreads();
  if (XS_VPRIO) __builtin_amdgcn_s_setprio(1);
  for (int idx = 0; idx < NS; ++idx) {
    const bool has_next = idx + 1 < NS;
    const Step nxt = step_of(has_next ? idx + 1 : idx);
    const __amdgpu_buffer_rsrc_t rGn = g_rsrc(nxt);
    const long r0w = (long)(cur.nrow > 0 ? cur.rb0 : 0) * T_;
    const bool on = cur.nrow > 0;
    bf16_t* HF = static_cast<bf16_t*>(inf_hfin(a, rz));
    const __amdgpu_buffer_rsrc_t rY =
        INF ? tt_rsrc_n(Yw ? (const void*)(Yw + r0w * a.ldy) : G, on && Yw != nullptr) : tt_rsrc_n(Yw + r0w * a.ldy, on);
    const __amdgpu_buffer_rsrc_t rX1 =
        INF ? tt_rsrc_n(HF ? (const void*)(HF + (long)(on ? cur.rb0 : 0) * inf_ldf(a)) : G, on && HF != nullptr && cur.s == T_ - 1)
            : tt_rsrc_n(X1 ? X1 + r0w * a.ldy : Yw, on && X1 != nullptr);
    const __amdgpu_buffer_rsrc_t rS = INF ? tt_rsrc_n(G, false) : tt_rsrc_n(S + r0w * 4L * H, on);
    const __amdgpu_buffer_rsrc_t rdst_h = rx[idx & 1];
    const int t = cur.t;
    const bool first = cur.s == 0;
#pragma unroll
    for (int c = 0; c < xc::NCH; ++c) {
      const int gslot = c % GR, gnext = (c + XS_GA) % GR;
      if (c + XS_GA < xc::NCH) load_g(cur, rGc, c + XS_GA, gq[gnext]);
      else if (has_next) load_g(nxt, rGn, c + XS_GA - xc::NCH, gq[gnext]);
      {
        const int rr = c * xc::CR + cr;
        const bool ok = rr < cur.nrow;
        const float* gb = stgb + (c & 1) * (xc::STG / 4);
        float xr[8], xz[8], xn[8], lr[8], lz[8], ln[8], y[8], sr[8], sz[8], sn[8], sg[8];
        const tt_u32x4(&gcur)[3] = gq[gslot];
        unpack8(make_uint4(gcur[0][0], gcur[0][1], gcur[0][2], gcur[0][3]), xr);
        unpack8(make_uint4(gcur[1][0], gcur[1][1], gcur[1][2], gcur[1][3]), xz);
        unpack8(make_uint4(gcur[2][0], gcur[2][1], gcur[2][2], gcur[2][3]), xn);
#pragma unroll
        for (int h = 0; h < 2; ++h) {
          const float4 v0 = *reinterpret_cast<const float4*>(gb + stg_off(cr, 0 * 64 + u0 + 4 * h));
          const float4 v1 = *reinterpret_cast<const float4*>(gb + stg_off(cr, 1 * 64 + u0 + 4 * h));
          const float4 v2 = *reinterpret_cast<const float4*>(gb + stg_off(cr, 2 * 64 + u0 + 4 * h));
          lr[4 * h] = v0.x; lr[4 * h + 1] = v0.y; lr[4 * h + 2] = v0.z; lr[4 * h + 3] = v0.w;
          lz[4 * h] = v1.x; lz[4 * h + 1] = v1.y; lz[4 * h + 2] = v1.z; lz[4 * h + 3] = v1.w;
          ln[4 * h] = v2.x; ln[4 * h + 1] = v2.y; ln[4 * h + 2] = v2.z; ln[4 * h + 3] = v2.w;
        }
        const uint32_t grow = (uint32_t)(cur.rb0 + rr) * (uint32_t)T_ + (uint32_t)t;
#pragma unroll
        for (int e = 0; e < 8; ++e) {
          const float hp = first ? 0.f : st[c][e];
          if (dbg & 16) {
            y[e] = xr[e] + lr[e] + hp; sr[e] = xz[e] + lz[e]; sz[e] = xn[e] + ln[e]; sn[e] = bn[e]; sg[e] = hp;
          } else {
            gru_cell(xr[e], xz[e], xn[e], lr[e], lz[e], ln[e], bn[e], hp, y[e], sr[e], sz[e], sn[e], sg[e]);
          }
          st[c][e] = y[e];
        }
        const uint4 yb = pack8bf(y);
        if (fast) st16_buf(rdst_h, (uint32_t)(rr * H + j) * 2u, 0, yb);
        else st16_buf_sc1(rdst_h, (uint32_t)(rr * H + j) * 2u, 0, yb);
        asm volatile("" ::: "memory");
        const int lrow = rr * T_ + t;
        const bool okd = ok && !(dbg & 1);
        const uint32_t oy = okd ? (uint32_t)(lrow * (int)a.ldy + j) * 2u : xc::OOB;
        const uint32_t os = okd ? (uint32_t)(lrow * 4 * H + j) * 2u : xc::OOB;
        st16_buf_aux<XC_OUT_AUX>(rY, (int)oy, yb);
        if constexpr (INF) {
          st16_buf_aux<XC_OUT_AUX>(rS, (int)os, yb);
          st16_buf_aux<XC_OUT_AUX>(rS, (int)(os + 2u * H), yb);
          st16_buf_aux<XC_OUT_AUX>(rS, (int)(os + 4u * H), yb);
          st16_buf_aux<XC_OUT_AUX>(rS, (int)(os + 6u * H), yb);
          st16_buf_aux<XC_OUT_AUX>(rX1, (int)(okd ? (uint32_t)(rr * (int)a.ldf + j) * 2u : xc::OOB), yb);
        } else {
          st16_buf_aux<XC_OUT_AUX>(rS, (int)os, pack8bf(sr));
          st16_buf_aux<XC_OUT_AUX>(rS, (int)(os + 2u * H), pack8bf(sz));
          st16_buf_aux<XC_OUT_AUX>(rS, (int)(os + 4u * H), pack8bf(sn));
          st16_buf_aux<XC_OUT_AUX>(rS, (int)(os + 6u * H), pack8bf(sg));
          if constexpr (DROP) {
#pragma unroll
            for (int e = 0; e < 8; ++e)
              y[e] *= tt_dropout_scale(R.seed, R.row0 + grow, (uint32_t)(R.col0 + j + e), a.drop_thresh, a.inv_keep);
            st16_buf_aux<XC_OUT_AUX>(rX1, (int)oy, pack8bf(y));
          } else {
            st16_buf_aux<XC_OUT_AUX>(rX1, (int)oy, yb);
          }
        }
      }
      if (c == 3 || c == 7) asm volatile("s_nop 0\n\ts_waitcnt vmcnt(6)" ::: "memory");
      if (c + 2 < xc::NCH || has_next) {
#pragma unroll
        for (int p = 0; p < QPW; ++p)
          *reinterpret_cast<tt_u32x4*>(slots + (c & 1) * C::SLOT + (vw * QPW + p) * 1024 + lane * 16) = hv[p];
      }
      if (c + 3 < xc::NCH) load_h(cur, idx, c + 3);
      else if (has_next) load_h(nxt, idx + 1, c + 3 - xc::NCH);
      if (!XS_MPOLL && vt == 0 && !(dbg & 32)) {
        if (c == 0 && idx > 0) xc_wait(cntB, (unsigned)(M * idx), ws);
        if (c == 4 && has_next) xc_wait(cntA, (unsigned)(M * (idx + 1)), ws);
      }
      __syncthreads();
      if (!XS_MPUB && vt == 0 && c == 3 && publish) __hip_atomic_fetch_add(cntA, 1u, __ATOMIC_RELAXED, __HIP_MEMORY_SCOPE_AGENT);
      if (!XS_MPUB && vt == 0 && c == 7 && publish) __hip_atomic_fetch_add(cntB, 1u, __ATOMIC_RELAXED, __HIP_MEMORY_SCOPE_AGENT);
    }
    cur = nxt;
    rGc = rGn;
  }
}
#ifdef TT_DIAG
}
extern "C" int tt_diag_fwd_prof(unsigned long long* out) {
  return hipMemcpyFromSymbol(out, HIP_SYMBOL(g_fwd_prof), sizeof(g_fwd_prof)) == hipSuccess ? 0 : 1;
}
namespace {
#endif
bool gru_fwd_persistent(int dtype, int H) {
  if (dtype != TT_DT_BF16 || H % 64 != 0 || H > PH_MAX) return false;
  return tt::opt(tt::OPT_GRU_STEP) != 1;
}

}

static int bwd_rows(int B, int H, int nrec) {
  const int o = tt::opt(tt::OPT_GRU_BWD_ROWS);
  if (o == 64 || o == 128) return o;
  return (long)tt_ceil_div(H, 128) * tt_ceil_div(B, 128) * nrec <= 256 ? 64 : 128;
}
extern "C" int tt_gru_bias_rows(int B) { return tt_ceil_div(B, 64); }

extern "C" int tt_gru_fwd_launches(int dtype, int T, int H) { return gru_fwd_persistent(dtype, H) ? 1 : T; }

static bool gru_bwd_persistent(int dtype, int H) {
  const int o = tt::opt(tt::OPT_GRU_BWD_PERSIST);
  return dtype == TT_DT_BF16 && (H == 256 || H == 512 || (H == 1024 && o == 2)) &&
         tt::opt(tt::OPT_GRU_BWD_ROWS) != 64 && o != 0;
}
extern "C" int tt_gru_bwd_launches(int dtype, int T, int H) { return gru_bwd_persistent(dtype, H) ? 1 : T; }
extern "C" int tt_gru_bwd_carry_on_chip(int dtype, int T, int H) {
  (void)T;
  return TT_BWD_CREG != 0 && gru_bwd_persistent(dtype, H) && H <= 512 ? 1 : 0;
}

struct SideStream {
  hipStream_t s = nullptr;
  hipEvent_t fork = nullptr, join = nullptr;
};
static int side_stream(SideStream** out) {
  static SideStream ss[64];
  static std::mutex mu;
  int dev = 0;
  TT_CHECK_HIP(hipGetDevice(&dev));
  TT_CHECK_ARG(dev >= 0 && dev < 64, "tt_gru_bwd: device %d", dev);
  std::lock_guard<std::mutex> lock(mu);
  SideStream& x = ss[dev];
  if (!x.s) {
    SideStream n;
    TT_CHECK_HIP(hipStreamCreateWithFlags(&n.s, hipStreamNonBlocking));
    TT_CHECK_HIP(hipEventCreateWithFlags(&n.fork, hipEventDisableTiming));
    TT_CHECK_HIP(hipEventCreateWithFlags(&n.join, hipEventDisableTiming));
    x = n;
  }
  *out = &x;
  return 0;
}

constexpr int XC_MAX_GROUPS = 512;
constexpr long XC_HDR = 256;
struct XcGeo {
  XcWs w{};
  int grid = 0, ng = 0;
  long cnt_bytes = 0, img_off = 0, bytes = 0;
};

struct XcDev {
  int cus = 0;
  int occ[2][2] = {{0, 0}, {0, 0}};
  int occ_xs[2] = {0, 0};
  int occ_inf[2] = {0, 0};
  int occ_xs_inf = 0;
};
static std::mutex g_xc_mu;
static XcDev g_xc[64];

template <int H, bool DROP>
static const void* xc_kernel() {
  return reinterpret_cast<const void*>(&gru_fwd_xcp<H, DROP>);
}
template <bool DROP>
static const void* xs_kernel() {
  return reinterpret_cast<const void*>(&gru_fwd_xs<512, DROP>);
}
template <int H>
static const void* xc_infer_kernel() {
  return reinterpret_cast<const void*>(&gru_fwd_xcp<H, false, InfArgs>);
}
static const void* xs_infer_kernel() { return reinterpret_cast<const void*>(&gru_fwd_xs<512, false, InfArgs>); }
static bool xs_on(int H) { return H == 512 && tt::opt(tt::OPT_GRU_FWD_XS) != 0; }

static int xc_device(XcDev** out) {
  int dev = 0;
  TT_CHECK_HIP(hipGetDevice(&dev));
  TT_CHECK_ARG(dev >= 0 && dev < 64, "tt_gru_fwd: device %d", dev);
  std::lock_guard<std::mutex> lock(g_xc_mu);
  XcDev& x = g_xc[dev];
  if (!x.cus) {
    int cus = 0;
    TT_CHECK_HIP(hipDeviceGetAttribute(&cus, hipDeviceAttributeMultiprocessorCount, dev));
    const void* k[2][2] = {{xc_kernel<256, false>(), xc_kernel<256, true>()},
                           {xc_kernel<512, false>(), xc_kernel<512, true>()}};
    for (int h = 0; h < 2; ++h)
      for (int d = 0; d < 2; ++d) TT_CHECK_HIP(hipOccupancyMaxActiveBlocksPerMultiprocessor(&x.occ[h][d], k[h][d], xc::NT, 0));
    const void* kx[2] = {xs_kernel<false>(), xs_kernel<true>()};
    for (int d = 0; d < 2; ++d) TT_CHECK_HIP(hipOccupancyMaxActiveBlocksPerMultiprocessor(&x.occ_xs[d], kx[d], xs::NT, 0));
    const void* ki[2] = {xc_infer_kernel<256>(), xc_infer_kernel<512>()};
    for (int h = 0; h < 2; ++h) TT_CHECK_HIP(hipOccupancyMaxActiveBlocksPerMultiprocessor(&x.occ_inf[h], ki[h], xc::NT, 0));
    TT_CHECK_HIP(hipOccupancyMaxActiveBlocksPerMultiprocessor(&x.occ_xs_inf, xs_infer_kernel(), xs::NT, 0));
    x.cus = cus;
  }
  *out = &x;
  return 0;
}

static bool xc_geometry(const XcDev& dev, int dtype, int H, int nrec, int B, int T, long ldg, long ldy, bool drop,
                        XcGeo& g, bool inf = false) {
  const int v = tt::opt(tt::OPT_GRU_FWD_XC);
  if (v == 0 || dtype != TT_DT_BF16 || (H != 512 && H != 256) || tt::opt(tt::OPT_GRU_STEP) == 1) return false;
  const int M = H / 64;
  const int qg = dev.cus / (8 * M);
  const int ng = 8 * qg;
  if (qg < 1 || ng > XC_MAX_GROUPS || ng % nrec != 0) return false;
  const int occ = inf ? (xs_on(H) ? dev.occ_xs_inf : dev.occ_inf[H == 512])
                      : (xs_on(H) ? dev.occ_xs[drop] : dev.occ[H == 512][drop]);
  if (occ < 1 || ng * M > dev.cus * occ) return false;
  const int gpr = ng / nrec;
  if ((v & 3) == 1 && (long)B < (long)gpr * (xc::RR / 2)) return false;
  if ((long)xc::RR * T * std::max({4L * H, ldy, ldg}) * 2 >= (1L << 31)) return false;
  g.w.qg = qg;
  g.w.nrec = nrec;
  g.w.rpg = tt_ceil_div(B, gpr);
  g.w.nround = tt_ceil_div(g.w.rpg, xc::RR);
  g.w.fast_ok = (v & 4) ? 0 : 1;
  g.w.xmap = (v & 16) ? 1 : 0;
  g.w.skip = tt::opt(tt::OPT_GRU_XC_SKIP);
  g.w.skew = tt::opt(tt::OPT_GRU_FWD_SKEW);
  const int sp = std::min(30, std::max(10, tt::opt(tt::OPT_GRU_XC_SPINS)));
  g.w.spins = 1u << sp;
  g.grid = ng * M;
  g.ng = ng;
  g.cnt_bytes = ((long)ng * xc::CSTR * 4 + 256 + 255) / 256 * 256;
  g.img_off = XC_HDR + g.cnt_bytes;
  g.bytes = g.img_off + (long)ng * 2 * xc::RR * H * 2;
  return true;
}

static int xc_plan(int dtype, int nrec, int B, int T, int H, long ldg, long ldy, bool drop, XcGeo& g, bool* ok,
                   bool inf = false) {
  *ok = false;
  if (dtype != TT_DT_BF16 || nrec < 1 || nrec > 4 || B <= 0 || T <= 0 || (H != 256 && H != 512) ||
      tt::opt(tt::OPT_GRU_FWD_XC) == 0)
    return 0;
  XcDev* x = nullptr;
  TT_PROPAGATE(xc_device(&x));
  *ok = xc_geometry(*x, dtype, H, nrec, B, T, ldg, ldy, drop, g, inf);
  return 0;
}

extern "C" long tt_gru_fwd_ws_size(int dtype, int nrec, int B, int T, int H, long ldg, long ldy) {
  XcGeo g;
  bool ok = false;
  if (xc_plan(dtype, nrec, B, T, H, ldg, ldy, true, g, &ok) != 0 || !ok) return 0;
  return g.bytes;
}

template <typename A>
static int gru_fwd_xc_launch(const A& a, int nrec, int B, int T, int H, long ldg, long ldy, void* ws,
                             long ws_bytes, hipStream_t st, bool* used) {
  constexpr bool inf = std::is_same_v<A, InfArgs>;
  *used = false;
  if (!ws) return 0;
  const bool drop = !inf && a.drop_thresh != 0 && a.r[0].x1 != nullptr;
  XcGeo g;
  bool ok = false;
  TT_PROPAGATE(xc_plan(TT_DT_BF16, nrec, B, T, H, ldg, ldy, drop, g, &ok, inf));
  if (!ok || ws_bytes < g.bytes) return 0;
  TT_CHECK_ARG(((uintptr_t)ws & 255) == 0, "tt_gru_fwd: ws must be 256-byte aligned");
  char* base = static_cast<char*>(ws);
  g.w.status = reinterpret_cast<unsigned*>(base);
  g.w.cnt = reinterpret_cast<unsigned*>(base + XC_HDR);
  g.w.err = g.w.cnt + g.ng * xc::CSTR;
  g.w.xb = reinterpret_cast<bf16_t*>(base + g.img_off);
  TT_CHECK_HIP(hipMemsetAsync(base + XC_HDR, 0, g.cnt_bytes, st));
  A ak = a;
  XcWs wk = g.w;
  void* args[] = {&ak, &wk};
  const bool xs = xs_on(H);
  const void* fn = inf ? (xs ? xs_infer_kernel() : H == 512 ? xc_infer_kernel<512>() : xc_infer_kernel<256>())
                   : xs ? (drop ? xs_kernel<true>() : xs_kernel<false>())
                   : H == 512 ? (drop ? xc_kernel<512, true>() : xc_kernel<512, false>())
                              : (drop ? xc_kernel<256, true>() : xc_kernel<256, false>());
  const int nt = xs ? xs::NT : xc::NT;
  const hipError_t e = tt::opt(tt::OPT_GRU_XC_COOP)
                           ? hipLaunchCooperativeKernel(fn, dim3(g.grid), dim3(nt), args, 0, st)
                           : hipLaunchKernel(fn, dim3(g.grid), dim3(nt), args, 0, st);
  if (e == hipErrorCooperativeLaunchTooLarge) {
    (void)hipGetLastError();
    return 0;
  }
  TT_CHECK_HIP(e);
  TT_CHECK_LAUNCH("gru_fwd_xcp");
  *used = true;
  return 0;
}

extern "C" int tt_gru_fwd_launches_for(int dtype, int nrec, int B, int T, int H, long ldg, long ldy) {
  XcGeo g;
  bool ok = false;
  if (xc_plan(dtype, nrec, B, T, H, ldg, ldy, true, g, &ok) == 0 && ok) return 1;
  return tt_gru_fwd_launches(dtype, T, H);
}

template <typename A>
static int launch_fwd_seq(const A& a, int nrec, int B, int H, hipStream_t st) {
  const dim3 grid(tt_ceil_div(B, PR) * nrec);
  int depth = (H / 64) % 4 == 0 ? 4 : (H / 64) % 2 == 0 ? 2 : 1;
  depth = std::min(depth, tt::opt(tt::OPT_GRU_DEPTH));
#define TT_SEQ(D, N) (gru_fwd_seq<D, N, A>)
  if (depth >= 4 && H == 512) hipLaunchKernelGGL(TT_SEQ(4, 8), grid, dim3(PNT), 0, st, a);
  else if (depth >= 4 && H == 256) hipLaunchKernelGGL(TT_SEQ(4, 4), grid, dim3(PNT), 0, st, a);
  else if (depth >= 4) hipLaunchKernelGGL(TT_SEQ(4, 0), grid, dim3(PNT), 0, st, a);
  else if (depth == 2 && H == 512) hipLaunchKernelGGL(TT_SEQ(2, 8), grid, dim3(PNT), 0, st, a);
  else if (depth == 2 && H == 256) hipLaunchKernelGGL(TT_SEQ(2, 4), grid, dim3(PNT), 0, st, a);
  else if (depth == 2) hipLaunchKernelGGL(TT_SEQ(2, 0), grid, dim3(PNT), 0, st, a);
  else if (H == 512) hipLaunchKernelGGL(TT_SEQ(1, 8), grid, dim3(PNT), 0, st, a);
  else if (H == 256) hipLaunchKernelGGL(TT_SEQ(1, 4), grid, dim3(PNT), 0, st, a);
  else hipLaunchKernelGGL(TT_SEQ(1, 0), grid, dim3(PNT), 0, st, a);
#undef TT_SEQ
  TT_CHECK_LAUNCH("gru_fwd_seq");
  return 0;
}

template <typename A>
static int launch_fwd_steps(int dtype, A a, int nrec, int B, int T, int H, long ldg, long ldy, hipStream_t st) {
  const int esz = dtype == TT_DT_BF16 ? 2 : 4;
  int bmr = tt::opt(tt::OPT_GRU_FWD_STEP_ROWS);
  if (bmr != 128 && bmr != 256)
    bmr = (long)tt_ceil_div(H, 64) * tt_ceil_div(B, 256) * nrec >= 512 ? 256 : 128;
  const long span = (long)T * std::max({4L * H, ldy, ldg}) * esz;
  if (bmr == 256 && 256L * span >= (1L << 31)) bmr = 128;
  TT_CHECK_ARG((long)bmr * span < (1L << 31), "tt_gru_fwd: tile byte offsets exceed 2 GiB (B tile %d)", bmr);
  dim3 grid(tt_ceil_div(H, 64) * tt_ceil_div(B, bmr) * nrec);
  XcDev* xd = nullptr;
  TT_PROPAGATE(xc_device(&xd));
  const bool ring = tt::opt(tt::OPT_GRU_STEP_RING) >= 3 && (long)grid.x <= xd->cus;
#define TT_STEP(T, R, NS) (gru_fwd_step<T, R, NS, A>)
  for (int s = 0; s < T; ++s) {
    a.s = s;
    if (dtype == TT_DT_BF16) {
      if (bmr == 256) hipLaunchKernelGGL(TT_STEP(bf16_t, 256, 2), grid, dim3(512), 0, st, a);
      else if (ring) hipLaunchKernelGGL(TT_STEP(bf16_t, 128, 3), grid, dim3(256), 0, st, a);
      else hipLaunchKernelGGL(TT_STEP(bf16_t, 128, 2), grid, dim3(256), 0, st, a);
    } else {
      if (bmr == 256) hipLaunchKernelGGL(TT_STEP(float, 256, 2), grid, dim3(512), 0, st, a);
      else if (ring) hipLaunchKernelGGL(TT_STEP(float, 128, 3), grid, dim3(256), 0, st, a);
      else hipLaunchKernelGGL(TT_STEP(float, 128, 2), grid, dim3(256), 0, st, a);
    }
    TT_CHECK_LAUNCH("gru_fwd_step");
  }
#undef TT_STEP
  return 0;
}

extern "C" int tt_gru_fwd(int dtype, const tt_gru_fwd_rec* recs, int nrec, int B, int T, int H, long ldg,
                          long ldy, float drop_p, void* ws, long ws_bytes, void* stream) {
  TT_CHECK_ARG(dtype == TT_DT_F32 || dtype == TT_DT_BF16, "tt_gru_fwd: bad dtype");
  TT_CHECK_ARG(nrec >= 1 && nrec <= 4, "tt_gru_fwd: nrec %d", nrec);
  TT_CHECK_ARG(B > 0 && T > 0 && H > 0, "tt_gru_fwd: bad shape");
  TT_CHECK_ARG(ws_bytes >= 0 && (ws != nullptr || ws_bytes == 0), "tt_gru_fwd: ws / ws_bytes");
  const int esz = dtype == TT_DT_BF16 ? 2 : 4;
  TT_CHECK_ARG(H % 8 == 0 && (ldy * esz) % 16 == 0, "tt_gru_fwd: H=%d (multiple of 8)/ldy=%ld misaligned", H, ldy);
  TT_CHECK_ARG(drop_p >= 0.f && drop_p < 1.f, "tt_gru_fwd: drop_p");
  TT_CHECK_ARG(tt_ceil_div(B, 128) <= 65535, "tt_gru_fwd: B too large");
  TT_CHECK_ARG(128L * T * std::max({4L * H, ldy, ldg}) * esz < (1L << 31), "tt_gru_fwd: tile byte offsets exceed 2 GiB");
  FwdArgs a{};
  for (int i = 0; i < nrec; ++i) {
    const tt_gru_fwd_rec& r = recs[i];
    TT_CHECK_ARG(r.g && r.whh && r.bhn && r.y && r.save && r.hstate, "tt_gru_fwd: null pointer in rec %d", i);
    a.r[i] = FwdRec{r.g, r.whh, r.bhn, r.y, r.x1, r.save, r.hstate, r.dir, r.drop_seed, r.drop_col0, r.drop_row0};
  }
  a.B = B; a.T = T; a.H = H; a.ldg = ldg; a.ldy = ldy;
  a.drop_thresh = drop_p > 0.f ? (uint32_t)(drop_p * 16777216.0f + 0.5f) : 0u;
  a.inv_keep = drop_p > 0.f ? 1.0f / (1.0f - drop_p) : 1.0f;
#ifdef TT_DIAG
  if (const char* e = getenv("TT_GRU_DBG")) a.dbg = atoi(e);
#endif
  hipStream_t st = (hipStream_t)stream;
  if (dtype == TT_DT_BF16) {
    bool used = false;
    TT_PROPAGATE(gru_fwd_xc_launch(a, nrec, B, T, H, ldg, ldy, ws, ws_bytes, st, &used));
    if (used) return 0;
  }
  if (gru_fwd_persistent(dtype, H)) return launch_fwd_seq(a, nrec, B, H, st);
  return launch_fwd_steps(dtype, a, nrec, B, T, H, ldg, ldy, st);
}

extern "C" long tt_gru_infer_scratch_size(int dtype, int B, int T, int H, int final_only) {
  if ((dtype != TT_DT_F32 && dtype != TT_DT_BF16) || B <= 0 || T <= 0 || H <= 0) return 0;
  if (gru_fwd_persistent(dtype, H)) return 0;
  const long esz = dtype == TT_DT_BF16 ? 2 : 4;
  return 2L * B * H * 4 + (final_only ? 2L * B * H * esz : 0);
}

extern "C" int tt_gru_fwd_infer(int dtype, const tt_gru_infer_rec* recs, int nrec, int B, int T, int H, long ldg,
                                long ldy, long ldf, void* ws, long ws_bytes, void* stream) {
  TT_CHECK_ARG(dtype == TT_DT_F32 || dtype == TT_DT_BF16, "tt_gru_fwd_infer: bad dtype");
  TT_CHECK_ARG(nrec >= 1 && nrec <= 4, "tt_gru_fwd_infer: nrec %d", nrec);
  TT_CHECK_ARG(B > 0 && T > 0 && H > 0, "tt_gru_fwd_infer: bad shape");
  TT_CHECK_ARG(ws_bytes >= 0 && (ws != nullptr || ws_bytes == 0), "tt_gru_fwd_infer: ws / ws_bytes");
  const int esz = dtype == TT_DT_BF16 ? 2 : 4;
  TT_CHECK_ARG(H % 8 == 0 && (ldy * esz) % 16 == 0, "tt_gru_fwd_infer: H=%d (multiple of 8)/ldy=%ld misaligned", H, ldy);
  TT_CHECK_ARG(tt_ceil_div(B, 128) <= 65535, "tt_gru_fwd_infer: B too large");
  TT_CHECK_ARG(128L * T * std::max({4L * H, ldy, ldg}) * esz < (1L << 31),
               "tt_gru_fwd_infer: tile byte offsets exceed 2 GiB");
  const bool has_y = recs[0].y != nullptr, has_f = recs[0].hfinal != nullptr;
  TT_CHECK_ARG(has_y || has_f, "tt_gru_fwd_infer: neither y nor hfinal given");
  TT_CHECK_ARG(!has_f || (ldf >= H && (ldf * esz) % 16 == 0 && 256L * ldf * esz < (1L << 31)),
               "tt_gru_fwd_infer: ldf=%ld misaligned or below H", ldf);
  const bool persistent = gru_fwd_persistent(dtype, H);
  const long state = 2L * B * H * 4;
  InfArgs a{};
  for (int i = 0; i < nrec; ++i) {
    const tt_gru_infer_rec& r = recs[i];
    TT_CHECK_ARG(r.g && r.whh && r.bhn, "tt_gru_fwd_infer: null pointer in rec %d", i);
    TT_CHECK_ARG((r.y != nullptr) == has_y && (r.hfinal != nullptr) == has_f,
                 "tt_gru_fwd_infer: rec %d disagrees with rec 0 on y / hfinal", i);
    TT_CHECK_ARG(persistent || (r.scratch && ((uintptr_t)r.scratch & 15) == 0),
                 "tt_gru_fwd_infer: rec %d needs 16-byte aligned scratch (tt_gru_infer_scratch_size)", i);
    a.r[i] = FwdRec{r.g, r.whh, r.bhn, r.y, nullptr, nullptr, static_cast<float*>(r.scratch), r.dir, 0u, 0, 0u};
    for (int k = nrec; k < 4; ++k) a.hfin[k] = a.himg[k] = nullptr;
    a.hfin[i] = r.hfinal;
    a.himg[i] = r.scratch && !has_y ? static_cast<char*>(r.scratch) + state : nullptr;
  }
  a.B = B; a.T = T; a.H = H; a.ldg = ldg; a.ldy = ldy; a.ldf = ldf;
  a.inv_keep = 1.0f;
  hipStream_t st = (hipStream_t)stream;
  if (dtype == TT_DT_BF16) {
    bool used = false;
    TT_PROPAGATE(gru_fwd_xc_launch(a, nrec, B, T, H, ldg, ldy, ws, ws_bytes, st, &used));
    if (used) return 0;
  }
  if (persistent) return launch_fwd_seq(a, nrec, B, H, st);
  return launch_fwd_steps(dtype, a, nrec, B, T, H, ldg, ldy, st);
}

template <typename T, int BMR>
static void launch_bwd_step(int ring, dim3 grid, hipStream_t st, const BwdArgs& a) {
  if (ring >= 4) hipLaunchKernelGGL((gru_bwd_step<T, BMR, 4>), grid, dim3(256), 0, st, a);
  else if (ring == 3) hipLaunchKernelGGL((gru_bwd_step<T, BMR, 3>), grid, dim3(256), 0, st, a);
  else hipLaunchKernelGGL((gru_bwd_step<T, BMR>), grid, dim3(256), 0, st, a);
}

extern "C" int tt_gru_bwd(int dtype, const tt_gru_bwd_rec* recs, int nrec, int B, int T, int H, long ldy,
                          long ldd, long ldf, void* stream) {
  TT_CHECK_ARG(dtype == TT_DT_F32 || dtype == TT_DT_BF16, "tt_gru_bwd: bad dtype");
  TT_CHECK_ARG(nrec >= 1 && nrec <= 4, "tt_gru_bwd: nrec %d", nrec);
  TT_CHECK_ARG(B > 0 && T > 0 && H > 0, "tt_gru_bwd: bad shape");
  const int esz = dtype == TT_DT_BF16 ? 2 : 4;
  TT_CHECK_ARG(H % 8 == 0 && (ldd * esz) % 16 == 0, "tt_gru_bwd: H=%d (multiple of 8)/ldd=%ld misaligned", H, ldd);
  TT_CHECK_ARG(256L * T * std::max({ldd, ldy, 4L * H}) * esz < (1L << 31), "tt_gru_bwd: tile byte offsets exceed 2 GiB");
  hipStream_t st = (hipStream_t)stream;
  BwdArgs a{};
  for (int i = 0; i < nrec; ++i) {
    const tt_gru_bwd_rec& r = recs[i];
    TT_CHECK_ARG(r.save && r.y && r.whh && r.dgx && r.dgh && r.dhstate && r.dbias_part,
                 "tt_gru_bwd: null pointer in rec %d", i);
    a.r[i] = BwdRec{r.save, r.y, r.dy, r.dfinal, r.whh, r.dgx, r.dgh, r.dhstate, r.dbias_part, r.dir};
    TT_CHECK_HIP(hipMemsetAsync(r.dbias_part, 0, sizeof(float) * 4L * H * tt_gru_bias_rows(B), st));
  }
  a.B = B; a.T = T; a.H = H; a.ldy = ldy; a.ldd = ldd; a.ldf = ldf;
  a.skew = tt::opt(tt::OPT_GRU_BWD_SKEW);
#ifdef TT_DIAG
  if (const char* e = getenv("TT_GRU_DBG")) a.dbg = atoi(e);
#endif
  const int bmr = bwd_rows(B, H, nrec);
  if (gru_bwd_persistent(dtype, H)) {
    TT_CHECK_ARG(128L * T * std::max({ldd, ldy, 4L * H}) * esz < (1L << 31), "tt_gru_bwd: tile offsets exceed 2 GiB");
    const dim3 grid(tt_ceil_div(B, 128) * nrec);
    if (H == 1024) hipLaunchKernelGGL(gru_bwd_rows<1024>, grid, dim3(512), 0, st, a);
    else if (H == 512) hipLaunchKernelGGL(gru_bwd_rows<512>, grid, dim3(512), 0, st, a);
    else hipLaunchKernelGGL(gru_bwd_rows<256>, grid, dim3(512), 0, st, a);
    TT_CHECK_LAUNCH("gru_bwd_rows");
    return 0;
  }
  if (dtype == TT_DT_BF16 && H % 256 == 0 && bmr == 128 && tt::opt(tt::OPT_GRU_BWD_BIG) != 0) {
    const dim3 grid((H / 256) * tt_ceil_div(B, 256) * nrec);
    for (int s = T - 1; s >= 0; --s) {
      a.s = s;
      hipLaunchKernelGGL(gru_bwd_big, grid, dim3(512), 0, st, a);
      TT_CHECK_LAUNCH("gru_bwd_big");
    }
    return 0;
  }
  const int ngrp = (nrec >= 2 && tt::opt(tt::OPT_GRU_BWD_STREAMS) != 1) ? 2 : 1;
  BwdArgs ga[2] = {a, a};
  int gn[2] = {nrec, 0};
  if (ngrp == 2) {
    gn[0] = nrec / 2;
    gn[1] = nrec - gn[0];
    for (int i = 0; i < gn[1]; ++i) ga[1].r[i] = a.r[gn[0] + i];
  }
  hipStream_t gs[2] = {st, st};
  SideStream* side = nullptr;
  if (ngrp == 2) {
    TT_PROPAGATE(side_stream(&side));
    gs[1] = side->s;
    TT_CHECK_HIP(hipEventRecord(side->fork, st));
    TT_CHECK_HIP(hipStreamWaitEvent(side->s, side->fork, 0));
  }
  XcDev* xd = nullptr;
  TT_PROPAGATE(xc_device(&xd));
  long wgs = 0;
  for (int g = 0; g < ngrp; ++g) wgs += (long)tt_ceil_div(H, 128) * tt_ceil_div(B, bmr) * gn[g];
  const int ring = wgs <= xd->cus ? tt::opt(tt::OPT_GRU_STEP_RING) : 2;
  for (int s = T - 1; s >= 0; --s) {
    for (int g = 0; g < ngrp; ++g) {
      ga[g].s = s;
      const dim3 grid(tt_ceil_div(H, 128) * tt_ceil_div(B, bmr) * gn[g]);
      if (dtype == TT_DT_BF16) {
        if (bmr == 64) launch_bwd_step<bf16_t, 64>(ring, grid, gs[g], ga[g]);
        else launch_bwd_step<bf16_t, 128>(ring, grid, gs[g], ga[g]);
      } else {
        if (bmr == 64) launch_bwd_step<float, 64>(ring, grid, gs[g], ga[g]);
        else launch_bwd_step<float, 128>(ring, grid, gs[g], ga[g]);
      }
      TT_CHECK_LAUNCH("gru_bwd_step");
    }
  }
  if (ngrp == 2) {
    TT_CHECK_HIP(hipEventRecord(side->join, side->s));
    TT_CHECK_HIP(hipStreamWaitEvent(st, side->join, 0));
  }
  return 0;
}
```

### two_towers_amd/towers.py

```python
from __future__ import annotations

import ctypes
import os
import threading
from dataclasses import dataclass

import torch
import torch.nn.functional as F

from . import _lib, dist, ops, timing
from ._lib import GruBwdRec, GruFwdRec, GruInferRec, HeadBwdIO, HeadFwdIO, call, dtype_code, stream_ptr

PARAMS_PER_TOWER = 22
LN_EPS = 1e-5
HEAD_DT = torch.float32


def gru_param_names():
    names = []
    for layer in (0, 1):
        for sfx in ("", "_reverse"):
            for w in ("weight_ih", "weight_hh", "bias_ih", "bias_hh"):
                names.append(f"{w}_l{layer}{sfx}")
    return names
# ... 67 lines not shown
                bi, bh = g[f"bias_ih_l{layer}{sfx}"], g[f"bias_hh_l{layer}{sfx}"]
                job(bi.data_ptr(), b.data_ptr() + d * 3 * H * 4, 1, 2 * H, 2 * H, 2 * H, 2 * H, False, bh.data_ptr())
                job(bi.data_ptr() + 2 * H * 4, b.data_ptr() + (d * 3 + 2) * H * 4, 1, H, H, H, H, False)
                wh = _alloc((3 * H, H), torch.bfloat16, dev)
                job(g[f"weight_hh_l{layer}{sfx}"].data_ptr(), wh.data_ptr(), 3 * H, H, H, H, H, True)
                whh.append(wh)
            self.wih.append(w)
            self.bias.append(b)
            self.whh.append(whh)
            self.bhn.append([g[f"bias_hh_l{layer}{s}"][2 * H:] for s in ("", "_reverse")])
        call("tt_pack_multi", jobs, nj, stream_ptr(dev))

    def _pack_torch(self, g, H, E, Ep, dt):
        for layer in (0, 1):
            wf, wr = g[f"weight_ih_l{layer}"], g[f"weight_ih_l{layer}_reverse"]
            w = torch.cat([wf, wr], 0)
            if layer == 0 and Ep != E:
                w = F.pad(w, (0, Ep - E))
            self.wih.append(w.to(dt).contiguous())
            bs = []
            for sfx in ("", "_reverse"):
                bi, bh = g[f"bias_ih_l{layer}{sfx}"], g[f"bias_hh_l{layer}{sfx}"]
                bs.append(torch.cat([bi[: 2 * H] + bh[: 2 * H], bi[2 * H:]]))
            self.bias.append(torch.cat(bs).float().contiguous())
            self.whh.append([g[f"weight_hh_l{layer}{s}"].to(dt).contiguous() for s in ("", "_reverse")])
            self.bhn.append([g[f"bias_hh_l{layer}{s}"][2 * H:].float().contiguous() for s in ("", "_reverse")])


def _packed(p, cfg: TowerCfg, Ep: int, cache_ok: bool) -> _Packed:
    if not cache_ok:
        return _Packed(p, cfg, Ep)
    key = (cfg.dtype, cfg.H, cfg.head, Ep, tuple(t._version for t in p), tuple(t.data_ptr() for t in p))
    hit = getattr(p[0], "_tt_pack", None)
    if hit is not None and hit[0] == key:
        return hit[1]
    pk = _Packed(p, cfg, Ep)
    p[0]._tt_pack = (key, pk)
    return pk


def _alloc(shape, dt, dev):
    return torch.empty(shape, dtype=dt, device=dev)


_status_lock = threading.Lock()
_status_pending: list = []
_step_guard: dict = {}
_guard_reset: set = set()


def step_guard(dev) -> torch.Tensor:
    dev = torch.device(dev)
    with _status_lock:
        g = _step_guard.get(dev)
        if g is None:
            g = _step_guard[dev] = torch.zeros(1, dtype=torch.int32, device=dev)
    return g


def gru_fwd_workspace(nrec, B, T, H, dt, dev):
    nb = _lib.load().tt_gru_fwd_ws_size(dtype_code(dt), nrec, B, T, H, 6 * H, 2 * H)
    if nb <= 0:
        return None
    ws = torch.empty(nb, dtype=torch.uint8, device=dev)
    if ws.data_ptr() % 256:
        raise _lib.TTError("GRU forward workspace is not 256-byte aligned")
    ws[:256].zero_()
    return ws


def reset_guard_if_reported(dev):
    dev = torch.device(dev)
    with _status_lock:
        due = dev in _guard_reset
        _guard_reset.discard(dev)
    if due:
        with torch.cuda.device(dev):
            step_guard(dev).zero_()


def watch_gru_status(ws, arm: bool = True):
    with torch.cuda.device(ws.device):
        st = torch.cuda.current_stream(ws.device)
        word = ws[:4].view(torch.int32)
        if arm:
            step_guard(ws.device).bitwise_or_(word)
        host = torch.zeros(1, dtype=torch.int32, pin_memory=True)
        host.copy_(word, non_blocking=True)
        ev = torch.cuda.Event()
        ev.record(st)
    with _status_lock:
        _status_pending.append((ev, host, torch.device(ws.device)))


def check_gru_status(wait: bool = True):
    with _status_lock:
        pend = list(_status_pending)
        _status_pending.clear()
    bad = 0
    keep = []
    bad_devs = set()
    for ev, host, dev in pend:
        if not wait and not ev.query():
            keep.append((ev, host, dev))
            continue
        ev.synchronize()
        if host.item() != 0:
            bad += 1
            bad_devs.add(dev)
    with _status_lock:
        if keep:
            _status_pending[:0] = keep
        _guard_reset.update(bad_devs)
    if bad:
        raise _lib.GruTimeoutError(
            f"{bad} column-split GRU forward launch(es) timed out waiting for a member workgroup "
            "(not all workgroups were resident); their outputs are invalid and the optimiser step "
            "that followed (two_towers_amd.Adam) left the weights unchanged. Set option gru_fwd_xc=0 "
            "(env TT_GRU_FWD_XC=0) to use the row-owning kernel.")


def _xs_selected() -> bool:
    try:
        return bool(_lib.get_option("gru_fwd_xs"))
    except _lib.TTError:
        return False


def table_cols(table, x):
    return getattr(table, "real_cols", table.shape[1])


def featurize(x: torch.Tensor, table: torch.Tensor | None, Ep: int, dt: torch.dtype) -> torch.Tensor:
    if x.dtype in (torch.int32, torch.int64):
        if table is None:
            raise _lib.TTError("integer token ids need an embedding table (model.set_embedding_table)")
        if table.dtype != dt or table.shape[1] != Ep:
            raise _lib.TTError(f"embedding table must be {dt} with {Ep} columns, got {table.dtype} {tuple(table.shape)}")
        ids = x.reshape(-1).to(torch.int32).contiguous()
        out = _alloc((ids.numel(), Ep), dt, x.device)
        esz = 2 if dt == torch.bfloat16 else 4
        gb = ids.numel() * (4 + 2 * table_cols(table, x) * esz)
        with timing.region("embed_gather", 1, gb, gb):
            ops.embed_gather(table, ids, out)
        return out
    if x.dim() != 3:
        raise ValueError(f"expected [B, T, E] embeddings or [B, T] token ids, got shape {tuple(x.shape)}")
    src = x.float().contiguous()
    out = _alloc((src.shape[0] * src.shape[1], Ep), dt, x.device)
    ops.pack_rows(src, out)
    return out


def _gru_layer_fwd(cfg, xs, K, ldx, packs, layer, B, T, seeds, want_x1, ws):
    n, H, dt, dev = cfg.ntowers, cfg.H, cfg.dtype, xs[0].device
    BT = B * T
    G = [_alloc((BT, 6 * H), dt, dev) for _ in range(n)]
    esz = 2 if dt == torch.bfloat16 else 4
    kr = cfg.E if layer == 0 else K
    with timing.region(f"input_proj_l{layer}", 1, 2.0 * BT * 6 * H * kr * n,
                       float(n * esz * (BT * kr + 6 * H * kr + BT * 6 * H))):
        ops.gemm(xs, [p.wih[layer] for p in packs], G, m=BT, n=6 * H, k=K, lda=ldx, ldb=K, ldc=6 * H,
                 a_kouter=False, b_kouter=False, dtype=dt, out_dtype=dt, bias=[p.bias[layer] for p in packs])
    Y = [_alloc((BT, 2 * H), dt, dev) for _ in range(n)]
    X1 = [_alloc((BT, 2 * H), dt, dev) for _ in range(n)] if want_x1 else None
    S = [[_alloc((BT, 4 * H), dt, dev) for _ in range(2)] for _ in range(n)]
    hs = _alloc((n * 2, 2, B, H), torch.float32, dev)
    recs = (GruFwdRec * (2 * n))()
    for ti in range(n):
        for d in range(2):
            r = recs[ti * 2 + d]
            r.g = G[ti][:, d * 3 * H:].data_ptr()
            r.whh = packs[ti].whh[layer][d].data_ptr()
            r.bhn = packs[ti].bhn[layer][d].data_ptr()
            r.y = Y[ti][:, d * H:].data_ptr()
            r.x1 = X1[ti][:, d * H:].data_ptr() if want_x1 else None
            r.save = S[ti][d].data_ptr()
            r.hstate = hs[ti * 2 + d].data_ptr()
            r.dir = d
            r.drop_seed = seeds[ti] & 0xFFFFFFFF
            r.drop_col0 = d * H
            r.drop_row0 = (cfg.rank * B * T) & 0xFFFFFFFF
    nl = _lib.load().tt_gru_fwd_launches_for(dtype_code(dt), 2 * n, B, T, H, 6 * H, 2 * H) if ws is not None \
        else _lib.load().tt_gru_fwd_launches(dtype_code(dt), T, H)
    per = esz * (8 + (1 if want_x1 else 0)) + (0 if nl == 1 else esz + 8)
    if nl == 1 and ws is not None:
        form = "gru_fwd_xs" if H == 512 and _xs_selected() else "gru_fwd_xcp"
        kname = f"{form}<{H}, {'true' if want_x1 and cfg.drop_p > 0 else 'false'}"
    elif nl == 1:
        kname = "gru_fwd_seq<"
    else:
        kname = "gru_fwd_step<"
    with timing.region("gru_fwd", nl, 2.0 * B * H * 3 * H * 2 * n * (T - 1), float(B * T * H * 2 * n * per),
                       kernel=kname):
        call("tt_gru_fwd", dtype_code(dt), recs, 2 * n, B, T, H, 6 * H, 2 * H, cfg.drop_p if want_x1 else 0.0,
             ws.data_ptr() if ws is not None else None, ws.numel() if ws is not None else 0, stream_ptr(dev))
    del G
    return Y, X1, S


def _gru_layer_infer(cfg, xs, K, ldx, packs, layer, B, T, ws, final_only):
    n, H, dt, dev = cfg.ntowers, cfg.H, cfg.dtype, xs[0].device
    BT = B * T
    lib = _lib.load()
    G = [_alloc((BT, 6 * H), dt, dev) for _ in range(n)]
    esz = 2 if dt == torch.bfloat16 else 4
    kr = cfg.E if layer == 0 else K
    with timing.region(f"input_proj_infer_l{layer}", 1, 2.0 * BT * 6 * H * kr * n,
                       float(n * esz * (BT * kr + 6 * H * kr + BT * 6 * H))):
        ops.gemm(xs, [p.wih[layer] for p in packs], G, m=BT, n=6 * H, k=K, lda=ldx, ldb=K, ldc=6 * H,
                 a_kouter=False, b_kouter=False, dtype=dt, out_dtype=dt, bias=[p.bias[layer] for p in packs])
    out = [_alloc((B, 2 * H) if final_only else (BT, 2 * H), dt, dev) for _ in range(n)]
    nb = lib.tt_gru_infer_scratch_size(dtype_code(dt), B, T, H, int(final_only))
    scr = _alloc((2 * n, nb), torch.uint8, dev) if nb > 0 else None
    recs = (GruInferRec * (2 * n))()
    for ti in range(n):
        for d in range(2):
            r = recs[ti * 2 + d]
            r.g = G[ti][:, d * 3 * H:].data_ptr()
            r.whh = packs[ti].whh[layer][d].data_ptr()
            r.bhn = packs[ti].bhn[layer][d].data_ptr()
            r.y = None if final_only else out[ti][:, d * H:].data_ptr()
            r.hfinal = out[ti][:, d * H:].data_ptr() if final_only else None
            r.scratch = scr[ti * 2 + d].data_ptr() if scr is not None else None
            r.dir = d
    nl = lib.tt_gru_fwd_launches_for(dtype_code(dt), 2 * n, B, T, H, 6 * H, 2 * H) if ws is not None \
        else lib.tt_gru_fwd_launches(dtype_code(dt), T, H)
    per = esz * (3 if final_only else 4) + (0 if nl == 1 else esz * (2 if final_only else 1) + 8)
    if nl == 1 and ws is not None:
        kname = f"{'gru_fwd_xs' if H == 512 and _xs_selected() else 'gru_fwd_xcp'}<{H}, false, (anonymous namespace)::InfArgs>"
    elif nl == 1:
        kname = "gru_fwd_seq<"
    else:
        kname = "gru_fwd_step<"
    with timing.region("gru_infer", nl, 2.0 * B * H * 3 * H * 2 * n * (T - 1), float(B * T * H * 2 * n * per),
                       kernel=kname):
        call("tt_gru_fwd_infer", dtype_code(dt), recs, 2 * n, B, T, H, 6 * H, 2 * H, 2 * H,
             ws.data_ptr() if ws is not None else None, ws.numel() if ws is not None else 0, stream_ptr(dev))
    return out


def towers_infer(cfg: TowerCfg, table, xs, params):
    n = cfg.ntowers
    _lib.require_gpu(*xs, *params)
    check_gru_status(wait=True)
    dt, E, H, h = cfg.dtype, cfg.E, cfg.H, cfg.h
    dev = xs[0].device
    reset_guard_if_reported(dev)
    B, T = xs[0].shape[0], xs[0].shape[1]
    for x in xs:
        if x.shape[0] != B or x.shape[1] != T:
            raise ValueError("query and doc inputs must share [B, T] in one fused call")
    Ep = ops.pad_cols(E, dt)
    npt = cfg.nparams
    with torch.no_grad():
        packs = [_packed(params[i * npt:(i + 1) * npt], cfg, Ep, True) for i in range(n)]
        X0 = [featurize(x, table, Ep, dt) for x in xs]
        ws = gru_fwd_workspace(2 * n, B, T, H, dt, dev)
        Y0 = _gru_layer_infer(cfg, X0, Ep, Ep, packs, 0, B, T, ws, False)
        del X0
        hfin = _gru_layer_infer(cfg, Y0, 2 * H, 2 * H, packs, 1, B, T, ws, True)
        del Y0
        if ws is not None:
            watch_gru_status(ws, arm=False)
        hcat = [f if f.dtype == HEAD_DT else f.to(HEAD_DT) for f in hfin]
        if cfg.head == "none":
            return tuple(hcat)
        outs, keep = [], []
        io = (HeadFwdIO * n)()
        for ti in range(n):
            pk = packs[ti]
            p1 = _alloc((B, 2 * h), HEAD_DT, dev)
            u = _alloc((B, 2 * h), HEAD_DT, dev)
            mean = _alloc((B,), torch.float32, dev)
            rstd = _alloc((B,), torch.float32, dev)
            out = _alloc((B, h), torch.float32, dev)
            q = io[ti]
            q.w1, q.b1, q.ln_g, q.ln_b = pk.w1.data_ptr(), pk.b1.data_ptr(), pk.ln_g.data_ptr(), pk.ln_b.data_ptr()
            q.w2, q.b2 = pk.w2.data_ptr(), pk.b2.data_ptr()
            q.x, q.p1, q.mean, q.rstd, q.u, q.out = (hcat[ti].data_ptr(), p1.data_ptr(), mean.data_ptr(),
                                                     rstd.data_ptr(), u.data_ptr(), out.data_ptr())
            outs.append(out)
            keep += [p1, u, mean, rstd]
        call("tt_proj_head_fwd", dtype_code(HEAD_DT), io, n, B, h, LN_EPS, stream_ptr(dev))
        return tuple(outs)


def _gru_layer_bwd(cfg, layer, B, T, S, Y, dY, dfinal, packs):
    n, H, dt, dev = cfg.ntowers, cfg.H, cfg.dtype, Y[0].device
    BT = B * T
    lib = _lib.load()
    dG = [_alloc((BT, 8 * H), dt, dev) for _ in range(n)]
    dhs = _alloc((n * 2, 2, B, H), dt, dev)
    nbr = lib.tt_gru_bias_rows(B)
    part = _alloc((n * 2, nbr, 4 * H), torch.float32, dev)
    recs = (GruBwdRec * (2 * n))()
    for ti in range(n):
        for d in range(2):
            r = recs[ti * 2 + d]
            r.save = S[ti][d].data_ptr()
            r.y = Y[ti][:, d * H:].data_ptr()
            r.dy = dY[ti][:, d * H:].data_ptr() if dY is not None else None
            r.dfinal = dfinal[ti][:, d * H:].data_ptr() if dfinal is not None else None
            r.whh = packs[ti].whh[layer][d].data_ptr()
            r.dgx = dG[ti][:, d * 3 * H:].data_ptr()
            r.dgh = dG[ti][:, 6 * H + d * H:].data_ptr()
            r.dhstate = dhs[ti * 2 + d].data_ptr()
            r.dbias_part = part[ti * 2 + d].data_ptr()
            r.dir = d
    ldf = dfinal[0].shape[1] if dfinal is not None else 0
    esz = 2 if dt == torch.bfloat16 else 4
    nl = lib.tt_gru_bwd_launches(dtype_code(dt), T, H)
    carry = 0 if lib.tt_gru_bwd_carry_on_chip(dtype_code(dt), T, H) else 2
    per = esz * (12 + carry + (1 if dY is not None else 0))
    kname = (f"gru_bwd_rows<{H}>" if nl == 1 else
             "gru_bwd_big" if dt == torch.bfloat16 and H % 256 == 0 and _lib.get_option("gru_bwd_big") else "gru_bwd_step<")
    with timing.region("gru_bwd", nl, 2.0 * B * 3 * H * H * 2 * n * (T - 1), float(B * T * H * 2 * n * per),
                       kernel=kname):
        call("tt_gru_bwd", dtype_code(dt), recs, 2 * n, B, T, H, 2 * H, 8 * H, ldf, stream_ptr(dev))
    sums = _alloc((n * 2, 4 * H), torch.float32, dev)
    for i in range(2 * n):
        ops.colsum(part[i], nbr, 4 * H, 4 * H, sums[i])
    dbih = [[sums[ti * 2 + d, : 3 * H] for d in range(2)] for ti in range(n)]
    dbhh = [[torch.cat([sums[ti * 2 + d, : 2 * H], sums[ti * 2 + d, 3 * H:]]) for d in range(2)] for ti in range(n)]
    return dG, dbih, dbhh


_WGRAD_T = os.environ.get("TT_WGRAD_T", "1") != "0"
WGRAD_OVERLAP = os.environ.get("TT_WGRAD_OVERLAP", "0") == "1"
_wgrad_streams: dict = {}


def _wgrad_stream(dev) -> torch.cuda.Stream:
    dev = torch.device(dev)
    with _status_lock:
        s = _wgrad_streams.get(dev)
        if s is None:
            s = _wgrad_streams[dev] = torch.cuda.Stream(device=dev)
    return s


def _weight_grads(cfg, B, T, dG, Xin, K, ldx, Y, kr=None):
    n, H, dt, dev = cfg.ntowers, cfg.H, cfg.dtype, dG[0].device
    BT = B * T
    dWih = [[_alloc((3 * H, K), torch.float32, dev) for _ in range(2)] for _ in range(n)]
    dWhh = [[_alloc((3 * H, H), torch.float32, dev) for _ in range(2)] for _ in range(n)]
    a_ih, b_ih, c_ih, a_hh, a_hi, b_hh, c_hh, sh = [], [], [], [], [], [], [], []
    for ti in range(n):
        for d in range(2):
            a_ih.append(dG[ti][:, d * 3 * H:])
            b_ih.append(Xin[ti])
            c_ih.append(dWih[ti][d])
            a_hh.append(dG[ti][:, d * 3 * H:])
            a_hi.append(dG[ti][:, 6 * H + d * H:])
            b_hh.append(Y[ti][:, d * H:])
            c_hh.append(dWhh[ti][d])
            sh.append(-1 if d == 0 else 1)
    esz = 2 if dt == torch.bfloat16 else 4
    kr = K if kr is None else kr
    with timing.region("wgrad_ih", 1, 2.0 * 3 * H * kr * BT * 2 * n,
                       float(n * (esz * BT * (6 * H + kr) + 2 * 3 * H * kr * 4))):
        if _WGRAD_T and dt == torch.bfloat16 and 0 < K % 256 <= 128:
            if ops.gemm_splits(K, 3 * H, BT, len(c_ih), dt) > 1:
                ops.gemm(b_ih, a_ih, c_ih, m=K, n=3 * H, k=BT, lda=ldx, ldb=8 * H, ldc=K, a_kouter=True,
                         b_kouter=True, dtype=dt, out_dtype=torch.float32, c_trans=True)
            else:
                cT = [_alloc((K, 3 * H), torch.float32, dev) for _ in c_ih]
                ops.gemm(b_ih, a_ih, cT, m=K, n=3 * H, k=BT, lda=ldx, ldb=8 * H, ldc=3 * H, a_kouter=True,
                         b_kouter=True, dtype=dt, out_dtype=torch.float32)
                for c, ct in zip(c_ih, cT):
                    c.copy_(ct.t())
        else:
            ops.gemm(a_ih, b_ih, c_ih, m=3 * H, n=K, k=BT, lda=8 * H, ldb=ldx, ldc=K, a_kouter=True,
                     b_kouter=True, dtype=dt, out_dtype=torch.float32)
    with timing.region("wgrad_hh", 1, 2.0 * 3 * H * H * BT * 2 * n,
                       float(n * (esz * BT * (6 * H + 2 * H) + 2 * 3 * H * H * 4))):
        ops.gemm(a_hh, b_hh, c_hh, m=3 * H, n=H, k=BT, lda=8 * H, ldb=2 * H, ldc=H, a_kouter=True, b_kouter=True,
                 dtype=dt, out_dtype=torch.float32, bshift=sh, seq_t=T, a_hi=a_hi, a_split=2 * H)
    return dWih, dWhh


class TowersFn(torch.autograd.Function):

    @staticmethod
    def forward(ctx, cfg: TowerCfg, table, group, cache_ok, *args):
        n = cfg.ntowers
        xs, params = args[:n], args[n:]
        _lib.require_gpu(*xs, *params)
        check_gru_status(wait=True)
        dt, E, H, h = cfg.dtype, cfg.E, cfg.H, cfg.h
        dev = xs[0].device
        reset_guard_if_reported(dev)
        B, T = xs[0].shape[0], xs[0].shape[1]
        for x in xs:
            if x.shape[0] != B or x.shape[1] != T:
                raise ValueError("query and doc inputs must share [B, T] in one fused call")
        Ep = ops.pad_cols(E, dt)
        npt = cfg.nparams
        packs = [_packed(params[i * npt:(i + 1) * npt], cfg, Ep, cache_ok) for i in range(n)]
        X0 = [featurize(x, table, Ep, dt) for x in xs]
        train_drop = cfg.drop_p > 0.0
        seeds = [int(torch.randint(0, 2 ** 31 - 1, (1,)).item()) for _ in range(n)] if train_drop else [0] * n
        ws = gru_fwd_workspace(2 * n, B, T, H, dt, dev)
        Y0, X1, S0 = _gru_layer_fwd(cfg, X0, Ep, Ep, packs, 0, B, T, seeds, train_drop, ws)
        Xl1 = X1 if train_drop else Y0
        Y1, _, S1 = _gru_layer_fwd(cfg, Xl1, 2 * H, 2 * H, packs, 1, B, T, seeds, False, ws)
        if ws is not None:
            watch_gru_status(ws, arm=any(ctx.needs_input_grad))
        hcat = []
        for ti in range(n):
            y = Y1[ti].view(B, T, 2 * H)
            hcat.append(torch.cat([y[:, T - 1, :H], y[:, 0, H:]], 1).to(HEAD_DT).contiguous())
        ctx.cfg = cfg
        ctx.group = group
        ctx.params = params
        ctx.dims = (B, T, Ep)
        ctx.seeds = seeds
        ctx.packs = packs
        if cfg.head == "none":
            ctx.acts = (X0, Y0, X1, S0, Y1, S1, None, None, None, None, None)
            return tuple(hcat)
        outs, p1s, means, rstds, us = [], [], [], [], []
        io = (HeadFwdIO * n)()
        for ti in range(n):
            pk = packs[ti]
            p1 = _alloc((B, 2 * h), HEAD_DT, dev)
            u = _alloc((B, 2 * h), HEAD_DT, dev)
            mean = _alloc((B,), torch.float32, dev)
            rstd = _alloc((B,), torch.float32, dev)
            out = _alloc((B, h), torch.float32, dev)
            q = io[ti]
            q.w1, q.b1, q.ln_g, q.ln_b = pk.w1.data_ptr(), pk.b1.data_ptr(), pk.ln_g.data_ptr(), pk.ln_b.data_ptr()
            q.w2, q.b2 = pk.w2.data_ptr(), pk.b2.data_ptr()
            q.x, q.p1, q.mean, q.rstd, q.u, q.out = (hcat[ti].data_ptr(), p1.data_ptr(), mean.data_ptr(),
                                                     rstd.data_ptr(), u.data_ptr(), out.data_ptr())
            outs.append(out); p1s.append(p1); means.append(mean); rstds.append(rstd); us.append(u)
        call("tt_proj_head_fwd", dtype_code(HEAD_DT), io, n, B, h, LN_EPS, stream_ptr(dev))
        ctx.acts = (X0, Y0, X1, S0, Y1, S1, hcat, p1s, means, rstds, us)
        return tuple(outs)

    @staticmethod
    def backward(ctx, *gouts):
        cfg = ctx.cfg
        check_gru_status(wait=False)
        n, dt, E, H, h = cfg.ntowers, cfg.dtype, cfg.E, cfg.H, cfg.h
        B, T, Ep = ctx.dims
        packs = ctx.packs
        X0, Y0, X1, S0, Y1, S1, hcat, p1s, means, rstds, us = ctx.acts
        dev = Y0[0].device
        lib = _lib.load()
        st = stream_ptr(dev)
        head_grads = [[] for _ in range(n)]
        dhcat = []
        if cfg.head == "none":
            for ti in range(n):
                g = gouts[ti]
                dhcat.append(torch.zeros(B, 2 * H, dtype=torch.float32, device=dev) if g is None
                             else g.float().contiguous())
        ws = None
        if cfg.head == "proj2":
            ws = _alloc((lib.tt_proj_head_bwd_ws_size(dtype_code(HEAD_DT), B, h),), torch.uint8, dev)
        for ti in range(n if cfg.head == "proj2" else 0):
            g = gouts[ti]
            g = torch.zeros(B, h, dtype=torch.float32, device=dev) if g is None else g.float().contiguous()
            pk = packs[ti]
            dx = _alloc((B, 2 * H), torch.float32, dev)
            dw1 = _alloc(pk.w1.shape, torch.float32, dev)
            db1 = _alloc((2 * h,), torch.float32, dev)
            dg = _alloc((2 * h,), torch.float32, dev)
            dbeta = _alloc((2 * h,), torch.float32, dev)
            dw2 = _alloc(pk.w2.shape, torch.float32, dev)
            db2 = _alloc((h,), torch.float32, dev)
            io = HeadBwdIO()
            io.w1, io.ln_g, io.ln_b, io.w2 = pk.w1.data_ptr(), pk.ln_g.data_ptr(), pk.ln_b.data_ptr(), pk.w2.data_ptr()
            io.x, io.p1, io.mean, io.rstd, io.u = (hcat[ti].data_ptr(), p1s[ti].data_ptr(), means[ti].data_ptr(),
                                                   rstds[ti].data_ptr(), us[ti].data_ptr())
            io.dout, io.dx = g.data_ptr(), dx.data_ptr()
            io.dw1, io.db1, io.dg, io.dbeta, io.dw2, io.db2 = (dw1.data_ptr(), db1.data_ptr(), dg.data_ptr(),
                                                               dbeta.data_ptr(), dw2.data_ptr(), db2.data_ptr())
            io.ws = ws.data_ptr()
            call("tt_proj_head_bwd", dtype_code(HEAD_DT), ctypes.byref(io), 1, B, h, LN_EPS, st)
            head_grads[ti] = [dw1, db1, dg, dbeta, dw2, db2]
            dhcat.append(dx)
        dG1, dbih1, dbhh1 = _gru_layer_bwd(cfg, 1, B, T, S1, Y1, None, dhcat, packs)
        Xl1 = X1 if X1 is not None else Y0
        red = dist.OverlapReducer(ctx.group[0]) if ctx.group is not None else None
        gl = [{} for _ in range(n)]

        def layer1_wgrads():
            dWih1, dWhh1 = _weight_grads(cfg, B, T, dG1, Xl1, 2 * H, 2 * H, Y1)
            _layer_grads(gl, 1, E, Ep, dWih1, dWhh1, dbih1, dbhh1)
            if red is not None:
                _reduce_into(red, gl, head_grads)

        main = torch.cuda.current_stream(dev)
        side = _wgrad_stream(dev) if WGRAD_OVERLAP else None
        if side is None:
            layer1_wgrads()
        dY0 = [_alloc((B * T, 2 * H), dt, dev) for _ in range(n)]
        esz = 2 if dt == torch.bfloat16 else 4
        with timing.region("dgrad_l1", 1, 2.0 * B * T * 2 * H * 6 * H * n,
                           float(n * esz * (B * T * 6 * H + B * T * 2 * H))):
            if X1 is None:
                ops.gemm(dG1, [p.wih[1] for p in packs], dY0, m=B * T, n=2 * H, k=6 * H, lda=8 * H, ldb=2 * H,
                         ldc=2 * H, a_kouter=False, b_kouter=True, dtype=dt, out_dtype=dt)
            else:
                for ti in range(n):
                    ops.gemm([dG1[ti]], [packs[ti].wih[1]], [dY0[ti]], m=B * T, n=2 * H, k=6 * H, lda=8 * H,
                             ldb=2 * H, ldc=2 * H, a_kouter=False, b_kouter=True, dtype=dt, out_dtype=dt,
                             drop_seed=ctx.seeds[ti], drop_p=cfg.drop_p, drop_row0=cfg.rank * B * T)
        if side is not None:
            side.wait_stream(main)
            for t in (*dG1, *Xl1, *Y1, *[g for hg in head_grads for g in hg], *[x for b in dbih1 for x in b],
                      *[x for b in dbhh1 for x in b]):
                t.record_stream(side)
            with torch.cuda.stream(side):
                layer1_wgrads()
        del dG1
        dG0, dbih0, dbhh0 = _gru_layer_bwd(cfg, 0, B, T, S0, Y0, dY0, None, packs)
        del dY0
        dWih0, dWhh0 = _weight_grads(cfg, B, T, dG0, X0, Ep, Ep, Y0, kr=E)
        gl0 = [{} for _ in range(n)]
        _layer_grads(gl0, 0, E, Ep, dWih0, dWhh0, dbih0, dbhh0)
        if side is not None:
            main.wait_stream(side)
            for t in [*[v for d in gl for v in d.values()], *[g for hg in head_grads for g in hg]]:
                t.record_stream(main)
        if red is not None:
            _reduce_into(red, gl0, [[] for _ in range(n)])
            red.finish(ctx.params)
        grads = []
        for ti in range(n):
            gl[ti].update(gl0[ti])
            grads.extend(gl[ti][k] for k in GRU_NAMES)
            grads.extend(head_grads[ti])
        ctx.acts = None
        ctx.packs = None
        ctx.params = None
        return (None, None, None, None, *([None] * n), *grads)


def _layer_grads(gl, layer, E, Ep, dWih, dWhh, dbih, dbhh):
    for ti in range(len(gl)):
        for d, sfx in enumerate(("", "_reverse")):
            w = dWih[ti][d]
            if layer == 0 and Ep != E:
                w = w[:, :E].contiguous()
            gl[ti][f"weight_ih_l{layer}{sfx}"] = w
            gl[ti][f"weight_hh_l{layer}{sfx}"] = dWhh[ti][d]
            gl[ti][f"bias_ih_l{layer}{sfx}"] = dbih[ti][d].contiguous()
            gl[ti][f"bias_hh_l{layer}{sfx}"] = dbhh[ti][d]


def _reduce_into(red, gl, head_grads):
    keys = [(ti, k) for ti in range(len(gl)) for k in gl[ti]]
    heads = [(ti, j) for ti in range(len(head_grads)) for j in range(len(head_grads[ti]))]
    views = red.launch([gl[ti][k] for ti, k in keys] + [head_grads[ti][j] for ti, j in heads])
    for (ti, k), v in zip(keys, views):
        gl[ti][k] = v
    for (ti, j), v in zip(heads, views[len(keys):]):
        head_grads[ti][j] = v


def run_towers(cfg: TowerCfg, table, xs, params, reduce_group=None, reduce: bool = False):
    if cfg.H % 8:
        raise ValueError(f"GRU hidden size {cfg.H} must be a multiple of 8 on the HIP path "
                         "(the step epilogues update 8 consecutive units per thread)")
    group = (reduce_group,) if reduce and dist.active(reduce_group) else None
    cache_ok = not (torch.is_grad_enabled() and any(p.requires_grad for p in params))
    if cache_ok and cfg.drop_p == 0.0:
        return towers_infer(cfg, table, xs, params)
    return TowersFn.apply(cfg, table, group, cache_ok, *xs, *params)
```

Measured before the change: 157,600 pairs/s.

## Store GRU outputs shifted by one step (y_prev layout) to simplify backward and wgrad

Adds a forward GRU variant that writes each step's hidden state into the slot of the next timestep, writes the final hidden state to a separate hfinal buffer, and zeroes the first-step row. The backward kernel and the Whh weight-gradient GEMM then read h_{t-1} from the row of the current timestep, so the GEMM no longer needs the seq_t/bshift row-shift indexing. The head input is taken directly from hfinal instead of a slice-and-cat. This adds an extra zeroing kernel and new kernel instantiations, and it relies on the layer-1 consumers accepting the shifted layout. Layer 0 uses it only when dropout is on, since dropout provides a separate X1 copy for the next layer.

```diff
diff --git a/include/tt_hip.h b/include/tt_hip.h
--- a/include/tt_hip.h
+++ b/include/tt_hip.h
@@ -109,6 +109,12 @@
 int tt_gru_bwd_carry_on_chip(int dtype, int T, int H);
 int tt_gru_bias_rows(int B);
 
+int tt_gru_yprev_supported(int dtype, int nrec, int B, int T, int H, long ldg, long ldy);
+int tt_gru_fwd_yprev(int dtype, const tt_gru_fwd_rec* recs, void* const* hfinal, int nrec, int B, int T, int H,
+                     long ldg, long ldy, long ldf, float drop_p, void* ws, long ws_bytes, void* stream);
+int tt_gru_bwd_yprev(int dtype, const tt_gru_bwd_rec* recs, int nrec, int B, int T, int H, long ldy,
+                     long ldd, long ldf, void* stream);
+
 typedef struct {
   const void* w1; const float* b1; const float* ln_g; const float* ln_b;
   const void* w2; const float* b2;
diff --git a/two_towers_amd/_lib.py b/two_towers_amd/_lib.py
--- a/two_towers_amd/_lib.py
+++ b/two_towers_amd/_lib.py
@@ -139,6 +139,11 @@
     "tt_gru_fwd_infer": (c_int, [c_int, POINTER(GruInferRec), c_int, c_int, c_int, c_int, c_long, c_long, c_long,
                                  c_void_p, c_long, c_void_p]),
     "tt_gru_infer_scratch_size": (c_long, [c_int, c_int, c_int, c_int, c_int]),
+    "tt_gru_yprev_supported": (c_int, [c_int, c_int, c_int, c_int, c_int, c_long, c_long]),
+    "tt_gru_fwd_yprev": (c_int, [c_int, POINTER(GruFwdRec), POINTER(c_void_p), c_int, c_int, c_int, c_int, c_long,
+                                 c_long, c_long, c_float, c_void_p, c_long, c_void_p]),
+    "tt_gru_bwd_yprev": (c_int, [c_int, POINTER(GruBwdRec), c_int, c_int, c_int, c_int, c_long, c_long, c_long,
+                                 c_void_p]),
     "tt_proj_head_fwd": (c_int, [c_int, POINTER(HeadFwdIO), c_int, c_int, c_int, c_float, c_void_p]),
     "tt_proj_head_bwd": (c_int, [c_int, POINTER(HeadBwdIO), c_int, c_int, c_int, c_float, c_void_p]),
     "tt_proj_head_bwd_ws_size": (c_long, [c_int, c_int, c_int]),
diff --git a/two_towers_amd/csrc/tt_api.h b/two_towers_amd/csrc/tt_api.h
--- a/two_towers_amd/csrc/tt_api.h
+++ b/two_towers_amd/csrc/tt_api.h
@@ -43,6 +43,7 @@
   OPT_GEMM_W4,
   OPT_BRES_FORM,
   OPT_WGRAD_TALL,
+  OPT_GRU_YPREV,
   OPT_N
 };
 int opt(Opt o);
diff --git a/two_towers_amd/csrc/tt_gemm.hip b/two_towers_amd/csrc/tt_gemm.hip
--- a/two_towers_amd/csrc/tt_gemm.hip
+++ b/two_towers_amd/csrc/tt_gemm.hip
@@ -43,6 +43,7 @@
     {"gemm_iepi", "TT_GEMM_IEPI", 1},             {"bres_rows", "TT_BRES_ROWS", 32},
     {"hn_scan_v", "TT_HN_SCAN_V", 5},             {"gemm_w4", "TT_GEMM_W4", 0},
     {"bres_form", "TT_BRES_FORM", 1},             {"wgrad_tall", "TT_WGRAD_TALL", 1},
+    {"gru_yprev", "TT_GRU_YPREV", 1},
 };
 struct OptTable {
   std::atomic<int> v[OPT_N];
diff --git a/two_towers_amd/csrc/tt_gru.hip b/two_towers_amd/csrc/tt_gru.hip
--- a/two_towers_amd/csrc/tt_gru.hip
+++ b/two_towers_amd/csrc/tt_gru.hip
@@ -29,10 +29,16 @@
   void* himg[4];
   long ldf;
 };
+struct YpArgs : FwdArgs {
+  void* hfin[4];
+  long ldf;
+};
 TT_DEV void* inf_hfin(const FwdArgs&, int) { return nullptr; }
 TT_DEV void* inf_hfin(const InfArgs& a, int rz) { return a.hfin[rz]; }
+TT_DEV void* inf_hfin(const YpArgs& a, int rz) { return a.hfin[rz]; }
 TT_DEV long inf_ldf(const FwdArgs&) { return 0; }
 TT_DEV long inf_ldf(const InfArgs& a) { return a.ldf; }
+TT_DEV long inf_ldf(const YpArgs& a) { return a.ldf; }
 
 struct BwdRec {
   const void* save; const void* y; const void* dy; const float* dfinal; const void* whh;
@@ -44,6 +50,7 @@
   long ldy, ldd, ldf;
   int s;
   int skew;
+  int yprev;
 #ifdef TT_DIAG
   int dbg;
 #endif
@@ -777,7 +784,7 @@
     bf16_t* cr_cur = static_cast<bf16_t*>(R.dh) + (long)(s & 1) * a.B * H + (long)m0 * H;
     const __amdgpu_buffer_rsrc_t rd = tt_rsrc_n(DY ? DY + trow * a.ldy : S, DY != nullptr);
     const __amdgpu_buffer_rsrc_t rsv = tt_rsrc_n(S + trow * 4L * H, true);
-    const __amdgpu_buffer_rsrc_t ry = tt_rsrc_n(s > 0 ? Y + ((long)m0 * T_ + tp) * a.ldy : S, s > 0);
+    const __amdgpu_buffer_rsrc_t ry = tt_rsrc_n(s > 0 ? Y + ((long)m0 * T_ + (a.yprev ? t : tp)) * a.ldy : S, s > 0);
     const __amdgpu_buffer_rsrc_t grs = tt_rsrc(DGXw + trow * a.ldd);
     uint32_t* L16 = reinterpret_cast<uint32_t*>(lds);
 #pragma unroll
@@ -1364,6 +1371,7 @@
 template <int H, bool DROP, typename A = FwdArgs>
 __global__ __launch_bounds__(xc::NT, 1) __attribute__((amdgpu_waves_per_eu(1, 1))) void gru_fwd_xcp(A a, XcWs ws) {
   constexpr bool INF = std::is_same_v<A, InfArgs>;
+  constexpr bool YP = std::is_same_v<A, YpArgs>;
   static_assert(!(INF && DROP), "no dropout copy in the inference form");
   using C = xc::Cfg<H>;
   constexpr int M = C::M, NKT = C::NKT;
@@ -1484,14 +1492,20 @@
     const long r0w = (long)(cur.nrow > 0 ? cur.rb0 : 0) * T_;
     const bool on = cur.nrow > 0;
     bf16_t* HF = static_cast<bf16_t*>(inf_hfin(a, rz));
-    const __amdgpu_buffer_rsrc_t rY =
+    __amdgpu_buffer_rsrc_t rY =
         INF ? tt_rsrc_n(Yw ? (const void*)(Yw + r0w * a.ldy) : G, on && Yw != nullptr) : tt_rsrc_n(Yw + r0w * a.ldy, on);
+    [[maybe_unused]] const bool ylast = YP && cur.s == T_ - 1;
+    if constexpr (YP) {
+      if (ylast) rY = tt_rsrc_n(HF ? (const void*)(HF + (long)(on ? cur.rb0 : 0) * inf_ldf(a)) : G, on && HF != nullptr);
+    }
     const __amdgpu_buffer_rsrc_t rX1 =
         INF ? tt_rsrc_n(HF ? (const void*)(HF + (long)(on ? cur.rb0 : 0) * inf_ldf(a)) : G, on && HF != nullptr && cur.s == T_ - 1)
             : tt_rsrc_n(X1 ? X1 + r0w * a.ldy : Yw, on && X1 != nullptr);
     const __amdgpu_buffer_rsrc_t rS = INF ? tt_rsrc_n(G, false) : tt_rsrc_n(S + r0w * 4L * H, on);
     const __amdgpu_buffer_rsrc_t rdst_h = rx[idx & 1];
     const int t = cur.t;
+    [[maybe_unused]] const int ypr = ylast ? (int)inf_ldf(a) : T_ * (int)a.ldy;
+    [[maybe_unused]] const int ypo = ylast ? 0 : (R.dir ? t - 1 : t + 1) * (int)a.ldy;
 #pragma unroll
     for (int c = 0; c < xc::NCH; ++c) {
       const bool more = c + 1 < xc::NCH || has_next;
@@ -1569,7 +1583,8 @@
         const int lrow = rr * T_ + t;
         const uint32_t oy = ok ? (uint32_t)(lrow * (int)a.ldy + j) * 2u : xc::OOB;
         const uint32_t os = ok ? (uint32_t)(lrow * 4 * H + j) * 2u : xc::OOB;
-        st16_buf_aux<XC_OUT_AUX>(rY, (int)oy, yb);
+        if constexpr (YP) st16_buf_aux<XC_OUT_AUX>(rY, (int)(ok ? (uint32_t)(rr * ypr + ypo + j) * 2u : xc::OOB), yb);
+        else st16_buf_aux<XC_OUT_AUX>(rY, (int)oy, yb);
         if constexpr (INF) {
           st16_buf_aux<XC_OUT_AUX>(rS, (int)os, yb);
           st16_buf_aux<XC_OUT_AUX>(rS, (int)(os + 2u * H), yb);
@@ -1638,6 +1653,7 @@
 template <int H, bool DROP, typename A = FwdArgs>
 __global__ __launch_bounds__(xs::NT, 1) __attribute__((amdgpu_waves_per_eu(2, 2))) void gru_fwd_xs(A a, XcWs ws) {
   constexpr bool INF = std::is_same_v<A, InfArgs>;
+  constexpr bool YP = std::is_same_v<A, YpArgs>;
   static_assert(!(INF && DROP), "no dropout copy in the inference form");
   using C = xc::Cfg<H>;
   constexpr int M = C::M, NKT = C::NKT, QPW = C::QPW;
@@ -1815,14 +1831,20 @@
     const long r0w = (long)(cur.nrow > 0 ? cur.rb0 : 0) * T_;
     const bool on = cur.nrow > 0;
     bf16_t* HF = static_cast<bf16_t*>(inf_hfin(a, rz));
-    const __amdgpu_buffer_rsrc_t rY =
+    __amdgpu_buffer_rsrc_t rY =
         INF ? tt_rsrc_n(Yw ? (const void*)(Yw + r0w * a.ldy) : G, on && Yw != nullptr) : tt_rsrc_n(Yw + r0w * a.ldy, on);
+    [[maybe_unused]] const bool ylast = YP && cur.s == T_ - 1;
+    if constexpr (YP) {
+      if (ylast) rY = tt_rsrc_n(HF ? (const void*)(HF + (long)(on ? cur.rb0 : 0) * inf_ldf(a)) : G, on && HF != nullptr);
+    }
     const __amdgpu_buffer_rsrc_t rX1 =
         INF ? tt_rsrc_n(HF ? (const void*)(HF + (long)(on ? cur.rb0 : 0) * inf_ldf(a)) : G, on && HF != nullptr && cur.s == T_ - 1)
             : tt_rsrc_n(X1 ? X1 + r0w * a.ldy : Yw, on && X1 != nullptr);
     const __amdgpu_buffer_rsrc_t rS = INF ? tt_rsrc_n(G, false) : tt_rsrc_n(S + r0w * 4L * H, on);
     const __amdgpu_buffer_rsrc_t rdst_h = rx[idx & 1];
     const int t = cur.t;
+    [[maybe_unused]] const int ypr = ylast ? (int)inf_ldf(a) : T_ * (int)a.ldy;
+    [[maybe_unused]] const int ypo = ylast ? 0 : (R.dir ? t - 1 : t + 1) * (int)a.ldy;
     const bool first = cur.s == 0;
 #pragma unroll
     for (int c = 0; c < xc::NCH; ++c) {
@@ -1866,7 +1888,8 @@
         const bool okd = ok && !(dbg & 1);
         const uint32_t oy = okd ? (uint32_t)(lrow * (int)a.ldy + j) * 2u : xc::OOB;
         const uint32_t os = okd ? (uint32_t)(lrow * 4 * H + j) * 2u : xc::OOB;
-        st16_buf_aux<XC_OUT_AUX>(rY, (int)oy, yb);
+        if constexpr (YP) st16_buf_aux<XC_OUT_AUX>(rY, (int)(okd ? (uint32_t)(rr * ypr + ypo + j) * 2u : xc::OOB), yb);
+        else st16_buf_aux<XC_OUT_AUX>(rY, (int)oy, yb);
         if constexpr (INF) {
           st16_buf_aux<XC_OUT_AUX>(rS, (int)os, yb);
           st16_buf_aux<XC_OUT_AUX>(rS, (int)(os + 2u * H), yb);
@@ -1979,6 +2002,8 @@
   int occ_xs[2] = {0, 0};
   int occ_inf[2] = {0, 0};
   int occ_xs_inf = 0;
+  int occ_yp[2][2] = {{0, 0}, {0, 0}};
+  int occ_xs_yp[2] = {0, 0};
 };
 static std::mutex g_xc_mu;
 static XcDev g_xc[64];
@@ -1996,6 +2021,14 @@
   return reinterpret_cast<const void*>(&gru_fwd_xcp<H, false, InfArgs>);
 }
 static const void* xs_infer_kernel() { return reinterpret_cast<const void*>(&gru_fwd_xs<512, false, InfArgs>); }
+template <int H, bool DROP>
+static const void* xc_yprev_kernel() {
+  return reinterpret_cast<const void*>(&gru_fwd_xcp<H, DROP, YpArgs>);
+}
+template <bool DROP>
+static const void* xs_yprev_kernel() {
+  return reinterpret_cast<const void*>(&gru_fwd_xs<512, DROP, YpArgs>);
+}
 static bool xs_on(int H) { return H == 512 && tt::opt(tt::OPT_GRU_FWD_XS) != 0; }
 
 static int xc_device(XcDev** out) {
@@ -2016,6 +2049,12 @@
     const void* ki[2] = {xc_infer_kernel<256>(), xc_infer_kernel<512>()};
     for (int h = 0; h < 2; ++h) TT_CHECK_HIP(hipOccupancyMaxActiveBlocksPerMultiprocessor(&x.occ_inf[h], ki[h], xc::NT, 0));
     TT_CHECK_HIP(hipOccupancyMaxActiveBlocksPerMultiprocessor(&x.occ_xs_inf, xs_infer_kernel(), xs::NT, 0));
+    const void* ky[2][2] = {{xc_yprev_kernel<256, false>(), xc_yprev_kernel<256, true>()},
+                            {xc_yprev_kernel<512, false>(), xc_yprev_kernel<512, true>()}};
+    for (int h = 0; h < 2; ++h)
+      for (int d = 0; d < 2; ++d) TT_CHECK_HIP(hipOccupancyMaxActiveBlocksPerMultiprocessor(&x.occ_yp[h][d], ky[h][d], xc::NT, 0));
+    const void* kxy[2] = {xs_yprev_kernel<false>(), xs_yprev_kernel<true>()};
+    for (int d = 0; d < 2; ++d) TT_CHECK_HIP(hipOccupancyMaxActiveBlocksPerMultiprocessor(&x.occ_xs_yp[d], kxy[d], xs::NT, 0));
     x.cus = cus;
   }
   *out = &x;
@@ -2023,15 +2062,16 @@
 }
 
 static bool xc_geometry(const XcDev& dev, int dtype, int H, int nrec, int B, int T, long ldg, long ldy, bool drop,
-                        XcGeo& g, bool inf = false) {
+                        XcGeo& g, bool inf = false, bool yp = false) {
   const int v = tt::opt(tt::OPT_GRU_FWD_XC);
   if (v == 0 || dtype != TT_DT_BF16 || (H != 512 && H != 256) || tt::opt(tt::OPT_GRU_STEP) == 1) return false;
   const int M = H / 64;
   const int qg = dev.cus / (8 * M);
   const int ng = 8 * qg;
   if (qg < 1 || ng > XC_MAX_GROUPS || ng % nrec != 0) return false;
-  const int occ = inf ? (xs_on(H) ? dev.occ_xs_inf : dev.occ_inf[H == 512])
-                      : (xs_on(H) ? dev.occ_xs[drop] : dev.occ[H == 512][drop]);
+  const int occ = inf  ? (xs_on(H) ? dev.occ_xs_inf : dev.occ_inf[H == 512])
+                  : yp ? (xs_on(H) ? dev.occ_xs_yp[drop] : dev.occ_yp[H == 512][drop])
+                       : (xs_on(H) ? dev.occ_xs[drop] : dev.occ[H == 512][drop]);
   if (occ < 1 || ng * M > dev.cus * occ) return false;
   const int gpr = ng / nrec;
   if ((v & 3) == 1 && (long)B < (long)gpr * (xc::RR / 2)) return false;
@@ -2055,14 +2095,14 @@
 }
 
 static int xc_plan(int dtype, int nrec, int B, int T, int H, long ldg, long ldy, bool drop, XcGeo& g, bool* ok,
-                   bool inf = false) {
+                   bool inf = false, bool yp = false) {
   *ok = false;
   if (dtype != TT_DT_BF16 || nrec < 1 || nrec > 4 || B <= 0 || T <= 0 || (H != 256 && H != 512) ||
       tt::opt(tt::OPT_GRU_FWD_XC) == 0)
     return 0;
   XcDev* x = nullptr;
   TT_PROPAGATE(xc_device(&x));
-  *ok = xc_geometry(*x, dtype, H, nrec, B, T, ldg, ldy, drop, g, inf);
+  *ok = xc_geometry(*x, dtype, H, nrec, B, T, ldg, ldy, drop, g, inf, yp);
   return 0;
 }
 
@@ -2076,13 +2116,13 @@
 template <typename A>
 static int gru_fwd_xc_launch(const A& a, int nrec, int B, int T, int H, long ldg, long ldy, void* ws,
                              long ws_bytes, hipStream_t st, bool* used) {
-  constexpr bool inf = std::is_same_v<A, InfArgs>;
+  constexpr bool inf = std::is_same_v<A, InfArgs>, yp = std::is_same_v<A, YpArgs>;
   *used = false;
   if (!ws) return 0;
   const bool drop = !inf && a.drop_thresh != 0 && a.r[0].x1 != nullptr;
   XcGeo g;
   bool ok = false;
-  TT_PROPAGATE(xc_plan(TT_DT_BF16, nrec, B, T, H, ldg, ldy, drop, g, &ok, inf));
+  TT_PROPAGATE(xc_plan(TT_DT_BF16, nrec, B, T, H, ldg, ldy, drop, g, &ok, inf, yp));
   if (!ok || ws_bytes < g.bytes) return 0;
   TT_CHECK_ARG(((uintptr_t)ws & 255) == 0, "tt_gru_fwd: ws must be 256-byte aligned");
   char* base = static_cast<char*>(ws);
@@ -2096,6 +2136,9 @@
   void* args[] = {&ak, &wk};
   const bool xs = xs_on(H);
   const void* fn = inf ? (xs ? xs_infer_kernel() : H == 512 ? xc_infer_kernel<512>() : xc_infer_kernel<256>())
+                   : yp ? (xs ? (drop ? xs_yprev_kernel<true>() : xs_yprev_kernel<false>())
+                           : H == 512 ? (drop ? xc_yprev_kernel<512, true>() : xc_yprev_kernel<512, false>())
+                                      : (drop ? xc_yprev_kernel<256, true>() : xc_yprev_kernel<256, false>()))
                    : xs ? (drop ? xs_kernel<true>() : xs_kernel<false>())
                    : H == 512 ? (drop ? xc_kernel<512, true>() : xc_kernel<512, false>())
                               : (drop ? xc_kernel<256, true>() : xc_kernel<256, false>());
@@ -2202,6 +2245,72 @@
   }
   if (gru_fwd_persistent(dtype, H)) return launch_fwd_seq(a, nrec, B, H, st);
   return launch_fwd_steps(dtype, a, nrec, B, T, H, ldg, ldy, st);
+}
+
+namespace {
+struct YpZeroArgs {
+  void* y[4];
+  int dir[4];
+  int B, T, H;
+  long ldy;
+};
+__global__ __launch_bounds__(256) void gru_yprev_zero_rows(YpZeroArgs a) {
+  const int per = a.H / 8;
+  const long i = (long)blockIdx.x * 256 + threadIdx.x;
+  if (i >= (long)a.B * per) return;
+  const int rz = blockIdx.y;
+  const long b = i / per;
+  const int j = (int)(i - b * per) * 8;
+  const int t = a.dir[rz] ? a.T - 1 : 0;
+  *reinterpret_cast<uint4*>(static_cast<bf16_t*>(a.y[rz]) + (b * a.T + t) * a.ldy + j) = make_uint4(0u, 0u, 0u, 0u);
+}
+}
+
+extern "C" int tt_gru_yprev_supported(int dtype, int nrec, int B, int T, int H, long ldg, long ldy) {
+  if (!gru_bwd_persistent(dtype, H) || H > 512) return 0;
+  XcGeo g;
+  bool ok = false;
+  if (xc_plan(dtype, nrec, B, T, H, ldg, ldy, true, g, &ok, false, true) != 0 || !ok) return 0;
+  return 1;
+}
+
+extern "C" int tt_gru_fwd_yprev(int dtype, const tt_gru_fwd_rec* recs, void* const* hfinal, int nrec, int B, int T,
+                                int H, long ldg, long ldy, long ldf, float drop_p, void* ws, long ws_bytes,
+                                void* stream) {
+  TT_CHECK_ARG(dtype == TT_DT_BF16, "tt_gru_fwd_yprev: bf16 only (tt_gru_yprev_supported)");
+  TT_CHECK_ARG(nrec >= 1 && nrec <= 4, "tt_gru_fwd_yprev: nrec %d", nrec);
+  TT_CHECK_ARG(B > 0 && T > 0 && (H == 256 || H == 512), "tt_gru_fwd_yprev: bad shape (H 256 or 512)");
+  TT_CHECK_ARG(ws != nullptr && ws_bytes > 0, "tt_gru_fwd_yprev: needs the tt_gru_fwd_ws_size workspace");
+  TT_CHECK_ARG((ldy * 2) % 16 == 0 && ldy >= H, "tt_gru_fwd_yprev: ldy=%ld misaligned or below H", ldy);
+  TT_CHECK_ARG(drop_p >= 0.f && drop_p < 1.f, "tt_gru_fwd_yprev: drop_p");
+  TT_CHECK_ARG(128L * T * std::max({4L * H, ldy, ldg}) * 2 < (1L << 31), "tt_gru_fwd_yprev: tile byte offsets exceed 2 GiB");
+  TT_CHECK_ARG(!hfinal || (ldf >= H && (ldf * 2) % 16 == 0 && 256L * ldf * 2 < (1L << 31)),
+               "tt_gru_fwd_yprev: ldf=%ld misaligned or below H", ldf);
+  YpArgs a{};
+  YpZeroArgs z{};
+  for (int i = 0; i < nrec; ++i) {
+    const tt_gru_fwd_rec& r = recs[i];
+    TT_CHECK_ARG(r.g && r.whh && r.bhn && r.y && r.save, "tt_gru_fwd_yprev: null pointer in rec %d", i);
+    TT_CHECK_ARG(((uintptr_t)r.y & 15) == 0, "tt_gru_fwd_yprev: y of rec %d is not 16-byte aligned", i);
+    TT_CHECK_ARG(!hfinal || (hfinal[i] && ((uintptr_t)hfinal[i] & 15) == 0),
+                 "tt_gru_fwd_yprev: hfinal[%d] null or not 16-byte aligned", i);
+    a.r[i] = FwdRec{r.g, r.whh, r.bhn, r.y, r.x1, r.save, r.hstate, r.dir, r.drop_seed, r.drop_col0, r.drop_row0};
+    a.hfin[i] = hfinal ? hfinal[i] : nullptr;
+    z.y[i] = r.y;
+    z.dir[i] = r.dir;
+  }
+  a.B = B; a.T = T; a.H = H; a.ldg = ldg; a.ldy = ldy; a.ldf = hfinal ? ldf : 0;
+  a.drop_thresh = drop_p > 0.f ? (uint32_t)(drop_p * 16777216.0f + 0.5f) : 0u;
+  a.inv_keep = drop_p > 0.f ? 1.0f / (1.0f - drop_p) : 1.0f;
+  z.B = B; z.T = T; z.H = H; z.ldy = ldy;
+  hipStream_t st = (hipStream_t)stream;
+  bool used = false;
+  TT_PROPAGATE(gru_fwd_xc_launch(a, nrec, B, T, H, ldg, ldy, ws, ws_bytes, st, &used));
+  TT_CHECK_ARG(used, "tt_gru_fwd_yprev: the column-split forward does not apply to this call (tt_gru_yprev_supported)");
+  hipLaunchKernelGGL(gru_yprev_zero_rows, dim3((unsigned)tt_ceil_div((long)B * (H / 8), 256), (unsigned)nrec), dim3(256), 0,
+                     st, z);
+  TT_CHECK_LAUNCH("gru_yprev_zero_rows");
+  return 0;
 }
 
 extern "C" long tt_gru_infer_scratch_size(int dtype, int B, int T, int H, int final_only) {
@@ -2260,14 +2369,16 @@
   else hipLaunchKernelGGL((gru_bwd_step<T, BMR>), grid, dim3(256), 0, st, a);
 }
 
-extern "C" int tt_gru_bwd(int dtype, const tt_gru_bwd_rec* recs, int nrec, int B, int T, int H, long ldy,
-                          long ldd, long ldf, void* stream) {
+static int gru_bwd_impl(int dtype, const tt_gru_bwd_rec* recs, int nrec, int B, int T, int H, long ldy, long ldd,
+                        long ldf, void* stream, int yprev) {
   TT_CHECK_ARG(dtype == TT_DT_F32 || dtype == TT_DT_BF16, "tt_gru_bwd: bad dtype");
   TT_CHECK_ARG(nrec >= 1 && nrec <= 4, "tt_gru_bwd: nrec %d", nrec);
   TT_CHECK_ARG(B > 0 && T > 0 && H > 0, "tt_gru_bwd: bad shape");
   const int esz = dtype == TT_DT_BF16 ? 2 : 4;
   TT_CHECK_ARG(H % 8 == 0 && (ldd * esz) % 16 == 0, "tt_gru_bwd: H=%d (multiple of 8)/ldd=%ld misaligned", H, ldd);
   TT_CHECK_ARG(256L * T * std::max({ldd, ldy, 4L * H}) * esz < (1L << 31), "tt_gru_bwd: tile byte offsets exceed 2 GiB");
+  TT_CHECK_ARG(!yprev || (gru_bwd_persistent(dtype, H) && H <= 512),
+               "tt_gru_bwd_yprev: the row-owning backward does not apply to this call (tt_gru_yprev_supported)");
   hipStream_t st = (hipStream_t)stream;
   BwdArgs a{};
   for (int i = 0; i < nrec; ++i) {
@@ -2279,6 +2390,7 @@
   }
   a.B = B; a.T = T; a.H = H; a.ldy = ldy; a.ldd = ldd; a.ldf = ldf;
   a.skew = tt::opt(tt::OPT_GRU_BWD_SKEW);
+  a.yprev = yprev;
 #ifdef TT_DIAG
   if (const char* e = getenv("TT_GRU_DBG")) a.dbg = atoi(e);
 #endif
@@ -2342,3 +2454,13 @@
   }
   return 0;
 }
+
+extern "C" int tt_gru_bwd(int dtype, const tt_gru_bwd_rec* recs, int nrec, int B, int T, int H, long ldy,
+                          long ldd, long ldf, void* stream) {
+  return gru_bwd_impl(dtype, recs, nrec, B, T, H, ldy, ldd, ldf, stream, 0);
+}
+
+extern "C" int tt_gru_bwd_yprev(int dtype, const tt_gru_bwd_rec* recs, int nrec, int B, int T, int H, long ldy,
+                                long ldd, long ldf, void* stream) {
+  return gru_bwd_impl(dtype, recs, nrec, B, T, H, ldy, ldd, ldf, stream, 1);
+}
diff --git a/two_towers_amd/towers.py b/two_towers_amd/towers.py
--- a/two_towers_amd/towers.py
+++ b/two_towers_amd/towers.py
@@ -243,7 +243,14 @@
     return out
 
 
-def _gru_layer_fwd(cfg, xs, K, ldx, packs, layer, B, T, seeds, want_x1, ws):
+def yprev_supported(cfg, B, T) -> bool:
+    H = cfg.H
+    if not _lib.get_option("gru_yprev"):
+        return False
+    return bool(_lib.load().tt_gru_yprev_supported(dtype_code(cfg.dtype), 2 * cfg.ntowers, B, T, H, 6 * H, 2 * H))
+
+
+def _gru_layer_fwd(cfg, xs, K, ldx, packs, layer, B, T, seeds, want_x1, ws, yprev=False, want_final=False):
     n, H, dt, dev = cfg.ntowers, cfg.H, cfg.dtype, xs[0].device
     BT = B * T
     G = [_alloc((BT, 6 * H), dt, dev) for _ in range(n)]
@@ -282,12 +289,20 @@
         kname = "gru_fwd_seq<"
     else:
         kname = "gru_fwd_step<"
+    hfin = [_alloc((B, 2 * H), dt, dev) for _ in range(n)] if yprev and want_final else None
     with timing.region("gru_fwd", nl, 2.0 * B * H * 3 * H * 2 * n * (T - 1), float(B * T * H * 2 * n * per),
                        kernel=kname):
-        call("tt_gru_fwd", dtype_code(dt), recs, 2 * n, B, T, H, 6 * H, 2 * H, cfg.drop_p if want_x1 else 0.0,
-             ws.data_ptr() if ws is not None else None, ws.numel() if ws is not None else 0, stream_ptr(dev))
+        if yprev:
+            fin = None
+            if hfin is not None:
+                fin = (ctypes.c_void_p * (2 * n))(*[hfin[ti][:, d * H:].data_ptr() for ti in range(n) for d in range(2)])
+            call("tt_gru_fwd_yprev", dtype_code(dt), recs, fin, 2 * n, B, T, H, 6 * H, 2 * H, 2 * H,
+                 cfg.drop_p if want_x1 else 0.0, ws.data_ptr(), ws.numel(), stream_ptr(dev))
+        else:
+            call("tt_gru_fwd", dtype_code(dt), recs, 2 * n, B, T, H, 6 * H, 2 * H, cfg.drop_p if want_x1 else 0.0,
+                 ws.data_ptr() if ws is not None else None, ws.numel() if ws is not None else 0, stream_ptr(dev))
     del G
-    return Y, X1, S
+    return Y, X1, S, hfin
 
 
 def _gru_layer_infer(cfg, xs, K, ldx, packs, layer, B, T, ws, final_only):
@@ -377,7 +392,7 @@
         return tuple(outs)
 
 
-def _gru_layer_bwd(cfg, layer, B, T, S, Y, dY, dfinal, packs):
+def _gru_layer_bwd(cfg, layer, B, T, S, Y, dY, dfinal, packs, yprev=False):
     n, H, dt, dev = cfg.ntowers, cfg.H, cfg.dtype, Y[0].device
     BT = B * T
     lib = _lib.load()
@@ -408,7 +423,8 @@
              "gru_bwd_big" if dt == torch.bfloat16 and H % 256 == 0 and _lib.get_option("gru_bwd_big") else "gru_bwd_step<")
     with timing.region("gru_bwd", nl, 2.0 * B * 3 * H * H * 2 * n * (T - 1), float(B * T * H * 2 * n * per),
                        kernel=kname):
-        call("tt_gru_bwd", dtype_code(dt), recs, 2 * n, B, T, H, 2 * H, 8 * H, ldf, stream_ptr(dev))
+        call("tt_gru_bwd_yprev" if yprev else "tt_gru_bwd", dtype_code(dt), recs, 2 * n, B, T, H, 2 * H, 8 * H, ldf,
+             stream_ptr(dev))
     sums = _alloc((n * 2, 4 * H), torch.float32, dev)
     for i in range(2 * n):
         ops.colsum(part[i], nbr, 4 * H, 4 * H, sums[i])
@@ -431,7 +447,7 @@
     return s
 
 
-def _weight_grads(cfg, B, T, dG, Xin, K, ldx, Y, kr=None):
+def _weight_grads(cfg, B, T, dG, Xin, K, ldx, Y, kr=None, yprev=False):
     n, H, dt, dev = cfg.ntowers, cfg.H, cfg.dtype, dG[0].device
     BT = B * T
     dWih = [[_alloc((3 * H, K), torch.float32, dev) for _ in range(2)] for _ in range(n)]
@@ -466,8 +482,12 @@
                      b_kouter=True, dtype=dt, out_dtype=torch.float32)
     with timing.region("wgrad_hh", 1, 2.0 * 3 * H * H * BT * 2 * n,
                        float(n * (esz * BT * (6 * H + 2 * H) + 2 * 3 * H * H * 4))):
-        ops.gemm(a_hh, b_hh, c_hh, m=3 * H, n=H, k=BT, lda=8 * H, ldb=2 * H, ldc=H, a_kouter=True, b_kouter=True,
-                 dtype=dt, out_dtype=torch.float32, bshift=sh, seq_t=T, a_hi=a_hi, a_split=2 * H)
+        if yprev:
+            ops.gemm(a_hh, b_hh, c_hh, m=3 * H, n=H, k=BT, lda=8 * H, ldb=2 * H, ldc=H, a_kouter=True, b_kouter=True,
+                     dtype=dt, out_dtype=torch.float32, a_hi=a_hi, a_split=2 * H)
+        else:
+            ops.gemm(a_hh, b_hh, c_hh, m=3 * H, n=H, k=BT, lda=8 * H, ldb=2 * H, ldc=H, a_kouter=True, b_kouter=True,
+                     dtype=dt, out_dtype=torch.float32, bshift=sh, seq_t=T, a_hi=a_hi, a_split=2 * H)
     return dWih, dWhh
 
 
@@ -493,16 +513,23 @@
         train_drop = cfg.drop_p > 0.0
         seeds = [int(torch.randint(0, 2 ** 31 - 1, (1,)).item()) for _ in range(n)] if train_drop else [0] * n
         ws = gru_fwd_workspace(2 * n, B, T, H, dt, dev)
-        Y0, X1, S0 = _gru_layer_fwd(cfg, X0, Ep, Ep, packs, 0, B, T, seeds, train_drop, ws)
+        yp1 = ws is not None and yprev_supported(cfg, B, T)
+        yp0 = yp1 and train_drop
+        Y0, X1, S0, _ = _gru_layer_fwd(cfg, X0, Ep, Ep, packs, 0, B, T, seeds, train_drop, ws, yprev=yp0)
         Xl1 = X1 if train_drop else Y0
-        Y1, _, S1 = _gru_layer_fwd(cfg, Xl1, 2 * H, 2 * H, packs, 1, B, T, seeds, False, ws)
+        Y1, _, S1, hfin = _gru_layer_fwd(cfg, Xl1, 2 * H, 2 * H, packs, 1, B, T, seeds, False, ws, yprev=yp1,
+                                         want_final=True)
         if ws is not None:
             watch_gru_status(ws, arm=any(ctx.needs_input_grad))
         hcat = []
         for ti in range(n):
+            if hfin is not None:
+                hcat.append(hfin[ti].to(HEAD_DT))
+                continue
             y = Y1[ti].view(B, T, 2 * H)
             hcat.append(torch.cat([y[:, T - 1, :H], y[:, 0, H:]], 1).to(HEAD_DT).contiguous())
         ctx.cfg = cfg
+        ctx.yprev = (yp0, yp1)
         ctx.group = group
         ctx.params = params
         ctx.dims = (B, T, Ep)
@@ -536,6 +563,7 @@
         check_gru_status(wait=False)
         n, dt, E, H, h = cfg.ntowers, cfg.dtype, cfg.E, cfg.H, cfg.h
         B, T, Ep = ctx.dims
+        yp0, yp1 = ctx.yprev
         packs = ctx.packs
         X0, Y0, X1, S0, Y1, S1, hcat, p1s, means, rstds, us = ctx.acts
         dev = Y0[0].device
@@ -573,13 +601,13 @@
             call("tt_proj_head_bwd", dtype_code(HEAD_DT), ctypes.byref(io), 1, B, h, LN_EPS, st)
             head_grads[ti] = [dw1, db1, dg, dbeta, dw2, db2]
             dhcat.append(dx)
-        dG1, dbih1, dbhh1 = _gru_layer_bwd(cfg, 1, B, T, S1, Y1, None, dhcat, packs)
+        dG1, dbih1, dbhh1 = _gru_layer_bwd(cfg, 1, B, T, S1, Y1, None, dhcat, packs, yprev=yp1)
         Xl1 = X1 if X1 is not None else Y0
         red = dist.OverlapReducer(ctx.group[0]) if ctx.group is not None else None
         gl = [{} for _ in range(n)]
 
         def layer1_wgrads():
-            dWih1, dWhh1 = _weight_grads(cfg, B, T, dG1, Xl1, 2 * H, 2 * H, Y1)
+            dWih1, dWhh1 = _weight_grads(cfg, B, T, dG1, Xl1, 2 * H, 2 * H, Y1, yprev=yp1)
             _layer_grads(gl, 1, E, Ep, dWih1, dWhh1, dbih1, dbhh1)
             if red is not None:
                 _reduce_into(red, gl, head_grads)
@@ -608,9 +636,9 @@
             with torch.cuda.stream(side):
                 layer1_wgrads()
         del dG1
-        dG0, dbih0, dbhh0 = _gru_layer_bwd(cfg, 0, B, T, S0, Y0, dY0, None, packs)
+        dG0, dbih0, dbhh0 = _gru_layer_bwd(cfg, 0, B, T, S0, Y0, dY0, None, packs, yprev=yp0)
         del dY0
-        dWih0, dWhh0 = _weight_grads(cfg, B, T, dG0, X0, Ep, Ep, Y0, kr=E)
+        dWih0, dWhh0 = _weight_grads(cfg, B, T, dG0, X0, Ep, Ep, Y0, kr=E, yprev=yp0)
         gl0 = [{} for _ in range(n)]
         _layer_grads(gl0, 0, E, Ep, dWih0, dWhh0, dbih0, dbhh0)
         if side is not None:
```

Result: faster. 159,900 pairs/s (median of 6 runs) (+1.5%).
